# behzadnouri/firedancer

Hardware: AMD Instinct MI355X
Metric: ed25519 verified sigs/sec at 1/8 MI355X vs host AVX-512; p99 batch latency (higher is better)
Workload: dtype u32; 1 GPU; BASELINE configs[1]: 1M single-sig 1232-byte synthetic Solana txns, all valid; txns_per_gpu=1048576, sigs_per_gpu=1048576, parallelism=independent per-GPU shards x1, semantics=avx512, contexts_per_gpu=1

## Files before the change

### firedancer_amd/csrc/fd_ed25519_gpu.hip

```cpp

#include "fd_gpu_sha512.h"
#include "fd_gpu_curve.h"
#include "fd_gpu_txn.h"
#include "fd_gpu_lattice.h"
#include "fd_pin_list.h"
#include "../../include/fd_ed25519_gpu.h"

#include <hip/hip_runtime.h>
#include <atomic>
#include <mutex>
#include <string.h>
#include <stdio.h>
#include <time.h>
#include <stdlib.h>
#include <string>
#include <vector>
#include <deque>
#include <thread>
#include <pthread.h>
#include <sched.h>

#define FD_WG 256
#define FD_ATAB_ENTRIES 9
#define FD_ATAB_STORED  8
// ... 38 lines not shown


FD_DEV void fe_store_packed( uint4 * dst, fe const & a ) {
  u32 w[8]; fe_pack( w, a );
  dst[0] = make_uint4( w[0], w[1], w[2], w[3] );
  dst[1] = make_uint4( w[4], w[5], w[6], w[7] );
}
FD_DEV void fe_from_quads( fe & a, uint4 x, uint4 y ) {
  u32 w[8] = { x.x, x.y, x.z, x.w, y.x, y.y, y.z, y.w };
  fe_unpack( a, w );
}

__device__ __attribute__(( aligned( 16 ) )) unsigned const fd_atab_ident_w[ 32 ] = {
  1u,0u,0u,0u, 0u,0u,0u,0u,  1u,0u,0u,0u, 0u,0u,0u,0u,  1u,0u,0u,0u, 0u,0u,0u,0u,  0u,0u,0u,0u, 0u,0u,0u,0u };

FD_DEV uint4 const * atab_entry( uint4 const * tab, u32 s, int e ) {
  return e ? tab + ((size_t)s * FD_ATAB_STORED + (size_t)( e - 1 )) * 8 : (uint4 const *)fd_atab_ident_w;
}

FD_DEV void atab_store( uint4 * tab, u32 s, int e, ge_cached const & c ) {
  uint4 * b = tab + ((size_t)s * FD_ATAB_STORED + (size_t)( e - 1 )) * 8;
  fe_store_packed( b + 0, c.YpX );
  fe_store_packed( b + 2, c.YmX );
  fe_store_packed( b + 4, c.Z   );
  fe_store_packed( b + 6, c.T2d );
}

struct atab_raw { uint4 q[8]; };

FD_DEV void atab_fetch( atab_raw & r, uint4 const * tab, u32 s, int e ) {
  uint4 const * b = atab_entry( tab, s, e );
#pragma unroll
  for( int i=0; i<8; i++ ) r.q[i] = b[i];
}
FD_DEV void fe_load_planar( fe & r, u32 const * p, size_t n ) {
#pragma unroll
  for( int i=0; i<10; i++ ) r.v[i] = p[(size_t)i*n];
}
FD_DEV void fe_store_planar( u32 * p, size_t n, fe const & a ) {
#pragma unroll
  for( int i=0; i<10; i++ ) p[(size_t)i*n] = a.v[i];
}
FD_DEV void fe_shfl_up( fe & r, fe const & a, int d ) {
#pragma unroll
  for( int i=0; i<10; i++ ) r.v[i] = (u32)__shfl_up( (int)a.v[i], (unsigned)d, 64 );
}
FD_DEV void fe_shfl_down( fe & r, fe const & a, int d ) {
#pragma unroll
  for( int i=0; i<10; i++ ) r.v[i] = (u32)__shfl_down( (int)a.v[i], (unsigned)d, 64 );
}

FD_DEV void atab_unpack( ge_cached & c, atab_raw const & r ) {
  fe_from_quads( c.YpX, r.q[0], r.q[1] );
  fe_from_quads( c.YmX, r.q[2], r.q[3] );
  fe_from_quads( c.Z,   r.q[4], r.q[5] );
  fe_from_quads( c.T2d, r.q[6], r.q[7] );
}

FD_DEV int ks_pos( u32 b, u32 nsig, u32 nf, u32 nh, u32 & col, u32 & j, int & cls ) {
  u32 fb = ( nf + FD_WG - 1u ) / FD_WG, hb = ( nh + FD_WG - 1u ) / FD_WG;
  cls = b < fb ? 2 : b < fb + hb ? 1 : 0;
  j = ( cls==2 ? b : cls==1 ? b - fb : b - fb - hb ) * FD_WG + threadIdx.x;
  col = cls==2 ? j : cls==1 ? nf + j : nsig - 1u - j;
  return j < ( cls==2 ? nf : cls==1 ? nh : nsig - nf - nh );
}
FD_DEV u32 ks_sig( u32 const * __restrict__ order, u32 const * __restrict__ orderh, u32 col, u32 j, int cls ) {
  return ( orderh && cls==1 ) ? orderh[j] : order[col];
}
#define FD_KC_HOTK 0
#define FD_KC_HOT  1
#define FD_KC_COLD 2
#define FD_KC_FBK  3
#define FD_KC_FB   4
#define FD_KC_HIT   6
#define FD_KC_MISS  7
#define FD_KC_BUILD 8
#define FD_KC_HAND0 9
#define FD_KC_HAND  10
#define FD_KC_PTIX  11
#define FD_KC_FFK   12
#define FD_KC_FFS   13
#define FD_KC_PINK  14
#define FD_KC_PINS  15


__global__ void __launch_bounds__( FD_WG )
fd_expand_kernel( fdgpu_txn_desc_t const * __restrict__ desc, u32 txn_cnt, u32 * __restrict__ map, u32 nsig,
                  u32 * __restrict__ zero_word ) {
  u32 t = blockIdx.x * FD_WG + threadIdx.x;
  if( zero_word && t == 0u ) { zero_word[0] = 0u; zero_word[1] = 0u; }
  if( t >= txn_cnt ) return;
  fdgpu_txn_desc_t d = desc[t];
  for( u32 j=0; j<d.sig_cnt; j++ ) {
    u32 s = d.sig_base + j;
    if( s < nsig ) map[s] = t | (j << 24);
  }
}

template<int FM = FD_CARRY_FOLD>
FD_DEV void atab_build( uint4 * __restrict__ tab, u32 s, uint4 const * __restrict__ Axy ) {
  uint4 const * ap = Axy + (size_t)s*4;
  ge_p3 A;
  fe_from_quads( A.X, ap[0], ap[1] );
  fe_from_quads( A.Y, ap[2], ap[3] );
  A.Z = fe_one();
  fe_neg( A.X, A.X ); fe_wcarry( A.X, A.X );
  fe_mul<FM>( A.T, A.X, A.Y );
  ge_cached c1, c;
  ge_p3_to_cached<FM>( c1, A );
  atab_store( tab, s, 1, c1 );
  ge_precomp a1; a1.ypx = c1.YpX; a1.ymx = c1.YmX; a1.xy2d = c1.T2d;
  ge_p3 cur = A;
#pragma unroll 1
  for( int e=2; e<FD_ATAB_ENTRIES; e++ ) {
    ge_p1p1 tt;
    ge_add_precomp<FM>( tt, cur, a1 );
    ge_p1p1_to_p3<FM>( cur, tt );
    ge_p3_to_cached<FM>( c, cur );
    atab_store( tab, s, e, c );
  }
}

FD_DEV int txn_desc_ok( fdgpu_txn_desc_t const & d ) {
  u32 cnt = d.sig_cnt;
  return !( cnt==0u || cnt>16u
            || (u32)d.signature_off + 64u*cnt > (u32)d.payload_sz
            || (u32)d.acct_addr_off + 32u*cnt > (u32)d.payload_sz
            || (u32)d.message_off > (u32)d.payload_sz );
}

template<int FM = FD_CARRY_FOLD>
FD_DEV void decode_one( unsigned char const * __restrict__ payload, fdgpu_txn_desc_t const * __restrict__ desc,
                        u32 const * __restrict__ map, u32 s, u32 is_r, unsigned char * __restrict__ stat,
                        uint4 * __restrict__ Rxy, uint4 * __restrict__ Axy ) {
  u32 m = map[s];
  u32 t = m & 0xffffffu, j = m >> 24;
  fdgpu_txn_desc_t d = desc[t];
  if( !txn_desc_ok( d ) ) { *stat = 0xffu; return; }
  unsigned char const * base = payload + d.payload_off;
  u32 w[8];
  fd_load_words<8>( w, base + ( is_r ? (u32)d.signature_off + 64u*j : (u32)d.acct_addr_off + 32u*j ) );
  ge_p3 P; int rc;
  ge_decode1<FM>( P, rc, w );
  int so = ge_affine_is_small_order( P );
  *stat = (unsigned char)( rc | (so << 2) );
  u32 x[8], y[8];
  fe_pack( x, P.X ); fe_pack( y, P.Y );
  uint4 * o = ( is_r ? Rxy : Axy ) + (size_t)s*4;
  o[0] = make_uint4( x[0], x[1], x[2], x[3] ); o[1] = make_uint4( x[4], x[5], x[6], x[7] );
  o[2] = make_uint4( y[0], y[1], y[2], y[3] ); o[3] = make_uint4( y[4], y[5], y[6], y[7] );
}

__global__ void __launch_bounds__( FD_WG )
fd_decode_kernel( unsigned char const *    __restrict__ payload,
                  fdgpu_txn_desc_t const * __restrict__ desc,
                  u32 const *              __restrict__ map,
                  u32                                   nsig,
                  int                                   both,
                  unsigned char *          __restrict__ pstat,
                  uint4 *                  __restrict__ Rxy,
                  uint4 *                  __restrict__ Axy,
                  uint4 *                  __restrict__ tabA,
                  uint4 *                  __restrict__ tabR,
                  u32 const *              __restrict__ ulist,
                  u32 *                    __restrict__ ucnt,
                  unsigned char *          __restrict__ astat,
                  u32                                   ublk,
                  u32 const *              __restrict__ order,
                  u32 const *              __restrict__ orderh,
                  u32 const *              __restrict__ kscnt,
                  u32 const *              __restrict__ kcnt,
                  u32                                   fb_min,
                  u32 const *              __restrict__ fidx,
                  u32 const *              __restrict__ birth,
                  u32                                   batch,
                  u32 const *              __restrict__ full ) {
  u32 s, is_r;
  unsigned char * st;
  if( ulist ) {
    if( blockIdx.x < ublk ) {
      u32 i = blockIdx.x * FD_WG + threadIdx.x;
      u32 cnt = ucnt[0];
      if( !i ) {
        u32 samp = FD_KD_SBLK( ublk ) * FD_WG; samp = samp < nsig ? samp : nsig;
        ucnt[1] = ucnt[1] ? ucnt[2] > samp - ( samp >> 3 ) : cnt > nsig - ( nsig >> 3 );
        ucnt[2] = 0u;
      }
      if( i >= cnt ) return;
      s = ulist[i]; is_r = 0u; st = astat + s;
      if( fidx && kcnt[s] >= fb_min ) {
        u32 slot = fidx[s];
        if( slot != FD_FB_NONE && full[slot] ) atomicAdd( ucnt + 3 + FD_KC_FFK, 1u );
        if( slot != FD_FB_NONE && birth[slot] != batch ) return;
      }
    } else if( order ) {
      u32 col, j; int cls;
      if( !ks_pos( blockIdx.x - ublk, nsig, kscnt[FD_KC_FB], kscnt[FD_KC_HOT], col, j, cls ) || cls==2 ) return;
      s = ks_sig( order, orderh, col, j, cls ); is_r = 1u;
      st = pstat + 2u*s + 1u;
    } else {
      s = ( blockIdx.x - ublk ) * FD_WG + threadIdx.x; is_r = 1u;
      if( s >= nsig ) return;
      st = pstat + 2u*s + 1u;
    }
  } else {
    u32 p = blockIdx.x * FD_WG + threadIdx.x;
    if( p >= ( both ? 2u*nsig : nsig ) ) return;
    s = both ? p >> 1 : p; is_r = both ? p & 1u : 0u;
    st = pstat + 2u*s + is_r;
  }
  decode_one( payload, desc, map, s, is_r, st, Rxy, Axy );
  if( tabA && ( *st & 3u )==0u ) atab_build( is_r ? tabR : tabA, s, is_r ? Rxy : Axy );
}

template<class W>
FD_DEV int store_digits_B( u32 const Sw[ 8 ], u32 s, size_t n, short * __restrict__ digB, int top, W win ) {
  int carry = 0;
#pragma unroll
  for( int i=0; i<FD_BDIG; i++ ) {
    int bit = FD_BWIN*i;
    int v = (int)((Sw[bit>>5] >> (bit&31)) & ((1u<<FD_BWIN)-1u)) + carry;
    carry = (v + (1<<(FD_BWIN-1))) >> FD_BWIN;
    int db = v - (carry << FD_BWIN);
    digB[(size_t)i*n + s] = (short)db;
    int wb = win( i );
    top = ( db && wb > top ) ? wb : top;
  }
  return top;
}

FD_DEV void store_digits( u32 const k[ 8 ], u32 const Sw[ 8 ], u32 s, size_t n,
                          i8 * __restrict__ digA, short * __restrict__ digB ) {
  int carry = 0;
#pragma unroll
  for( int i=0; i<64; i++ ) {
    int v = (int)((k[i>>3] >> (4*(i&7))) & 15u) + carry;
    carry = (v + 8) >> 4;
    digA[(size_t)i*n + s] = (i8)(v - (carry << 4));
  }
  (void)store_digits_B( Sw, s, n, digB, 0, []( int ) { return 0; } );
}


FD_DEV void sc_mul_5x8( u32 out[ 16 ], u32 const a[ 5 ], u32 const b[ 8 ] ) {
  u32 r[ 16 ];
#pragma unroll
  for( int i=0; i<16; i++ ) r[i] = 0u;
#pragma unroll
  for( int i=0; i<5; i++ ) {
    u64 c = 0;
#pragma unroll
    for( int j=0; j<8; j++ ) { u64 t = (u64)a[i] * (u64)b[j] + (u64)r[i+j] + c; r[i+j] = (u32)t; c = t >> 32; }
    r[i+8] = (u32)c;
  }
#pragma unroll
  for( int i=0; i<16; i++ ) out[i] = r[i];
}

template<int HOT = 0>
FD_DEV int hs_prepare( u32 const k[ 8 ], u32 const Sw[ 8 ], u32 c0[ HOT ? 7 : 5 ], u32 c1m[ 5 ], int & c1neg, u32 sp[ 8 ] ) {
  constexpr int NC = HOT ? 7 : 5;
  int ng = 0, nwin = 0;
  if( HOT ) { if( !fd_lat_skew( c0, c1m, &ng, &nwin, k ) ) return 0; }
  else if( !fd_lat_halfsize( c0, c1m, &ng, k ) ) return 0;
  c1neg = ng;
  u32 c1lo = ng ? 0u - c1m[0] : c1m[0];
  if( ( c0[0] - c1lo * k[0] ) & 7u ) return 0;
  u32 const lw[8] = { 0x5cf5d3edu, 0x5812631au, 0xa2f79cd6u, 0x14def9deu, 0u, 0u, 0u, 0x10000000u };
  u32 prod[ 16 ], x[ 8 ];
  sc_mul_5x8( prod, c1m, k ); sc_reduce( x, prod );
  u32 diff = 0u;
  if( !ng ) {
#pragma unroll
    for( int i=0; i<8; i++ ) diff |= x[i] ^ ( i < NC ? c0[i] : 0u );
  } else {
// ... 241 lines not shown
  fd_load_words<8>( Aw, base + d.acct_addr_off + 32u*j );
  u32 h[16], k[8];
  if( khash ) {
    if( q ) return;
    khash_load( h, khash, s );
  } else {
    fd_sha512_RAM_quad( h, Rw, Aw, base + d.message_off, (u32)d.payload_sz - (u32)d.message_off, q, qbase );
    if( q ) return;
  }
  sc_reduce( k, h );
  u32 c0[5], c1m[5], sp[8]; int c1neg = 0;
  if( !( force_slow && s % force_slow == 0u ) && hs_prepare( k, Sw, c0, c1m, c1neg, sp ) ) {
    hs_store_digits( c0, c1m, c1neg, sp, s, n, digA, digR, digB, htop );
    code_out[s] = FD_ED25519_SUCCESS;
  } else {
    store_digits( k, Sw, s, n, digA, digB );
    code_out[s] = FD_PEND_SLOW;
    slow[ atomicAdd( slow_cnt, 1u ) ] = s;
  }
}

template<int FM = FD_CARRY_FOLD>
FD_DEV void htab_build( uint4 * __restrict__ htab, u32 hi, u32 part, uint4 const * __restrict__ Axy, u32 rep ) {
  uint4 const * ap = Axy + (size_t)rep*4;
  ge_p3 A;
  fe_from_quads( A.X, ap[0], ap[1] );
  fe_from_quads( A.Y, ap[2], ap[3] );
  A.Z = fe_one();
  fe_neg( A.X, A.X ); fe_wcarry( A.X, A.X );
  fe_mul<FM>( A.T, A.X, A.Y );
  int nd = 4*FD_KS_W*( (int)part + 1 );
#pragma unroll 1
  for( int i=0; i<nd; i++ ) ge_p3_dbl<FM>( A, A );
  u32 t = 2u*hi + part;
  ge_cached c1;
  ge_p3_to_cached<FM>( c1, A );
  atab_store( htab, t, 1, c1 );
#pragma unroll 1
  for( int e=2; e<FD_ATAB_ENTRIES; e++ ) {
    ge_p1p1 tt;
    ge_add_cached<FM>( tt, A, c1 );
    ge_p1p1_to_p3<FM>( A, tt );
    uint4 * b = htab + ((size_t)t * FD_ATAB_STORED + (size_t)( e - 1 )) * 8;
    fe u;
    fe_add( u, A.Y, A.X ); fe_store_packed( b + 0, u );
    fe_sub( u, A.Y, A.X ); fe_store_packed( b + 2, u );
    fe_store_packed( b + 4, A.Z );
    fe d2 = fe_d2(); fe_mul<FM>( u, A.T, d2 ); fe_store_packed( b + 6, u );
  }
}


FD_DEV void hashf_one( unsigned char const * __restrict__ payload, fdgpu_txn_desc_t const * __restrict__ desc,
                       u32 const * __restrict__ map, u32 s, size_t n, int semantics, u32 pa,
                       i8 * __restrict__ code_out, i8 * __restrict__ digA, short * __restrict__ digB,
                       uint4 * __restrict__ Rraw, uint4 const * __restrict__ khash, u32 col ) {
  fdgpu_txn_desc_t d; u32 j;
  if( !sig_desc( desc, map, s, d, j ) ) { code_out[s] = FD_ED25519_ERR_SIG; return; }
  unsigned char const * base = payload + d.payload_off;
  u32 Sw[8];
  fd_load_words<8>( Sw, base + d.signature_off + 64u*j + 32u );
  int code = sc_is_canonical( Sw ) ? FD_ED25519_SUCCESS : FD_ED25519_ERR_SIG;
  code = result_code( code, pa, 0u, semantics, 1 );
  code_out[s] = (i8)code;
  if( code != FD_ED25519_SUCCESS && code != FD_PEND_ASMALL ) return;
  u32 Rw[8], Aw[8];
  fd_load_words<8>( Rw, base + d.signature_off + 64u*j );
  Rraw[4*(size_t)s]   = make_uint4( Rw[0], Rw[1], Rw[2], Rw[3] );
  Rraw[4*(size_t)s+1] = make_uint4( Rw[4], Rw[5], Rw[6], Rw[7] );
  if( code != FD_ED25519_SUCCESS ) return;
  fd_load_words<8>( Aw, base + d.acct_addr_off + 32u*j );
  u32 h[16], k[8];
  if( khash ) khash_load( h, khash, s );
  else fd_sha512_RAM( h, Rw, Aw, base + d.message_off, (u32)d.payload_sz - (u32)d.message_off );
  sc_reduce( k, h );
  i8 dk[ 32 ];
  (void)fd_fb_recode( dk, k );
#pragma unroll
  for( int i=0; i<32; i++ ) digA[(size_t)i*n + col] = dk[i];
  (void)store_digits_B( Sw, col, n, digB, 0, []( int ) { return 0; } );
}

template<int FM = FD_CARRY_FOLD>
FD_DEV void fbase_chain( uint4 * __restrict__ fbase, u32 fi, u32 j, ge_p3 & A, int nd ) {
#pragma unroll 1
  for( int i=0; i<nd; i++ ) ge_p3_dbl<FM>( A, A );
  ge_cached c;
  ge_p3_to_cached<FM>( c, A );
  uint4 * b = fbase + ( (size_t)fi * FD_FB_NT + j ) * 8;
  fe_store_packed( b + 0, c.YpX );
  fe_store_packed( b + 2, c.YmX );
  fe_store_packed( b + 4, c.Z   );
  fe_store_packed( b + 6, c.T2d );
}
template<int FM = FD_CARRY_FOLD>
FD_DEV void fbase_build( uint4 * __restrict__ fbase, u32 fi, u32 j, uint4 const * __restrict__ Axy, u32 rep ) {
  uint4 const * ap = Axy + (size_t)rep*4;
  ge_p3 A;
  fe_from_quads( A.X, ap[0], ap[1] );
  fe_from_quads( A.Y, ap[2], ap[3] );
  A.Z = fe_one();
  fe_neg( A.X, A.X ); fe_wcarry( A.X, A.X );
  fe_mul<FM>( A.T, A.X, A.Y );
  fbase_chain<FM>( fbase, fi, j, A, 8*(int)j );
}

__device__ __attribute__(( aligned( 16 ) )) unsigned const fd_ptab_ident_w[ 24 ] = {
  1u,0u,0u,0u, 0u,0u,0u,0u,  1u,0u,0u,0u, 0u,0u,0u,0u,  0u,0u,0u,0u, 0u,0u,0u,0u };

FD_DEV size_t ftab_at( u32 fi, u32 j, u32 e ) {
  return ( ( (size_t)fi * FD_FB_NT + j ) * FD_FB_E + ( e - 1u ) ) * 6;
}

template<int I>
FD_DEV void ftab_pass1( ge_p3 & Q, ge_cached const & pc, uint4 * __restrict__ ent, fe (&pf)[ 8 ] ) {
  ge_p1p1 tt;
  ge_add_cached( tt, Q, pc ); ge_p1p1_to_p3( Q, tt );
  fe_store_packed( ent + 6*I + 0, Q.X );
  fe_store_packed( ent + 6*I + 2, Q.Y );
  fe_store_packed( ent + 6*I + 4, Q.Z );
  if constexpr( I > 0 ) fe_mul( pf[I], pf[I-1], Q.Z ); else pf[0] = Q.Z;
  if constexpr( I < 7 ) ftab_pass1<I+1>( Q, pc, ent, pf );
}
template<int I>
FD_DEV void ftab_pass2( fe & inv, uint4 * __restrict__ ent, fe const (&pf)[ 8 ] ) {
  fe X, Y, Z, zi, x, y, u;
  fe_from_quads( X, ent[6*I+0], ent[6*I+1] );
  fe_from_quads( Y, ent[6*I+2], ent[6*I+3] );
  if constexpr( I > 0 ) {
    fe_from_quads( Z, ent[6*I+4], ent[6*I+5] );
    fe_mul( zi, inv, pf[I-1] ); fe_mul( inv, inv, Z );
  } else zi = inv;
  fe_mul( x, X, zi ); fe_mul( y, Y, zi );
  fe_add( u, y, x ); fe_store_packed( ent + 6*I + 0, u );
  fe_sub( u, y, x ); fe_store_packed( ent + 6*I + 2, u );
  fe d2 = fe_d2();
  fe_mul( u, x, y ); fe_mul( u, u, d2 ); fe_store_packed( ent + 6*I + 4, u );
  if constexpr( I > 0 ) ftab_pass2<I-1>( inv, ent, pf );
}

__global__ void __launch_bounds__( FD_WG, 2 )
fd_ftab_kernel( u32 const * __restrict__ kscnt, u32 const * __restrict__ flist,
                unsigned char const * __restrict__ astat, uint4 const * __restrict__ fbase, uint4 * __restrict__ ftab,
                u32 cg, u32 const * __restrict__ plist, u32 pmax ) {
  u32 nk = kscnt[FD_KC_BUILD] * cg;
  u32 np = kscnt[FD_KC_PTIX]; np = np < pmax ? np : pmax;
  u32 bi = blockIdx.x * 2u + ( threadIdx.x >> 7 );
  if( blockIdx.x * 2u >= nk + 3u*np ) return;
  if( bi >= nk + 3u*np ) return;
  u32 fi, grp;
  if( bi < nk ) {
    if( astat[ flist[ 2u*( bi / cg ) + 1u ] ] & 7u ) return;
    fi = flist[ 2u*( bi / cg ) ]; grp = bi % cg;
  } else { fi = plist[ ( bi - nk ) / 3u ]; grp = ( bi - nk ) % 3u + 1u; }
  u32 t = 4u*( ( threadIdx.x >> 4 ) & 7u ) + grp, g = threadIdx.x & 15u;
  int lane = (int)( threadIdx.x & 63u );
  ge_cached pc;
  {
    atab_raw r; uint4 const * b = fbase + ( (size_t)fi * FD_FB_NT + t ) * 8;
#pragma unroll
    for( int i=0; i<8; i++ ) r.q[i] = b[i];
    atab_unpack( pc, r );
  }
  ge_p3 Q; ge_p3_identity( Q );
  ge_p1p1 tt;
#pragma unroll 1
  for( int b=3; b>=0; b-- ) {
    ge_p3_dbl( Q, Q );
    ge_add_cached( tt, Q, pc );
    ge_p3 Qa; ge_p1p1_to_p3( Qa, tt );
    int bit = (int)( ( g >> b ) & 1u );
    fe_sel( Q.X, bit, Qa.X, Q.X ); fe_sel( Q.Y, bit, Qa.Y, Q.Y ); fe_sel( Q.Z, bit, Qa.Z, Q.Z ); fe_sel( Q.T, bit, Qa.T, Q.T );
  }
#pragma unroll 1
  for( int b=0; b<3; b++ ) ge_p3_dbl( Q, Q );
  fe pf[ 8 ];
  uint4 * ent = ftab + ftab_at( fi, t, 8u*g + 1u );
  ftab_pass1<0>( Q, pc, ent, pf );
  fe one = fe_one(), pre = pf[7], suf = pf[7], u;
#pragma unroll 1
  for( int d=1; d<64; d<<=1 ) {
    fe_shfl_up( u, pre, d );   fe_sel( u, lane >= d, u, one );     fe_mul( pre, pre, u );
    fe_shfl_down( u, suf, d ); fe_sel( u, lane + d < 64, u, one ); fe_mul( suf, suf, u );
  }
  fe o, e, tot, inv;
  fe_shfl_up( o, pre, 1 );   fe_sel( o, lane > 0, o, one );
  fe_shfl_down( e, suf, 1 ); fe_sel( e, lane < 63, e, one );
  fe_mul( o, o, e );
#pragma unroll
  for( int i=0; i<10; i++ ) tot.v[i] = (u32)__shfl( (int)pre.v[i], 63, 64 );
  fe_invert( inv, tot );
  fe_mul( inv, inv, o );
  ftab_pass2<7>( inv, ent, pf );
}

template<int KS>
__global__ void __launch_bounds__( FD_WG )
fd_hashh_kernel( unsigned char const *    __restrict__ payload,
                 fdgpu_txn_desc_t const * __restrict__ desc,
                 u32 const *              __restrict__ map,
                 u32                                   nsig,
                 int                                   semantics,
                 unsigned char *          __restrict__ pstat,
                 i8 *                     __restrict__ code_out,
                 i8 *                     __restrict__ digA,
                 i8 *                     __restrict__ digR,
                 short *                  __restrict__ digB,
                 u32 *                    __restrict__ slow,
                 u32 *                    __restrict__ slow_cnt,
                 uint4 const *            __restrict__ khash,
                 u32                                   force_slow,
                 unsigned char *          __restrict__ htop,
                 u32 const *              __restrict__ arep,
                 unsigned char const *    __restrict__ astat,
                 u32 *                    __restrict__ order,
                 u32 const *              __restrict__ kscnt,
                 u32 const *              __restrict__ hlist,
                 uint4 const *            __restrict__ Axy,
                 uint4 *                  __restrict__ htab,
                 u32                                   hblk,
                 u32 const *              __restrict__ orderh,
                 u32 const *              __restrict__ flist,
                 uint4 *                  __restrict__ fbase,
                 u32                                   fblk,
                 unsigned char *          __restrict__ sstat,
                 uint4 *                  __restrict__ Rraw,
                 u32                                   lpk ) {
  if( KS ) {
    if( blockIdx.x < hblk ) {
      u32 i = blockIdx.x * FD_WG + threadIdx.x;
      if( ( i >> 1 ) >= kscnt[FD_KC_HOTK] ) return;
      u32 rep = hlist[ i >> 1 ];
      if( astat[rep] & 7u ) return;
      htab_build( htab, i >> 1, i & 1u, Axy, rep );
      return;
    }
    if( blockIdx.x < hblk + fblk ) {
      u32 i = ( blockIdx.x - hblk ) * FD_WG + threadIdx.x;
      u32 k = i / lpk, q = i % lpk;
      if( k >= kscnt[FD_KC_BUILD] ) return;
      u32 slot = flist[ 2u*k ], rep = flist[ 2u*k + 1u ];
      if( !q ) sstat[slot] = astat[rep];
      if( astat[rep] & 7u ) return;
      fbase_build( fbase, slot, q * ( (u32)FD_FB_NT / lpk ), Axy, rep );
      return;
    }
    u32 col, j; int cls;
    if( !ks_pos( blockIdx.x - hblk - fblk, nsig, orderh ? kscnt[FD_KC_FB] : 0u, kscnt[FD_KC_HOT], col, j, cls ) ) return;
    u32 s = ks_sig( order, orderh, col, j, cls );
    if( cls==2 ) {
      hashf_one( payload, desc, map, s, nsig, semantics, astat[ arep[s] ], code_out, digA, digB, Rraw, khash, col );
      return;
    }
    if( orderh && cls==1 ) order[col] = s;
    hashh_one<1>( payload, desc, map, s, nsig, semantics, 1, pstat, code_out, digA, digR, digB, slow, slow_cnt,
                  khash, force_slow, htop, arep, astat, col, cls==1 );
    return;
  }
  u32 s = blockIdx.x * FD_WG + threadIdx.x;
  if( s >= nsig ) return;
// ... 251 lines not shown
  uint4 ra[ 6 ], rb[ 6 ];
#pragma unroll 1
  for( int r=3; r>=0; r-- ) {
    int na = fd_fb_old_adds( r );
    int d = dA[ (size_t)fd_fb_old_digit( r, 0 )*n ];
    ptab_fetch( ra, d ? ftab + ftab_at( fi, (u32)fd_fb_old_table( 0 ), (u32)fd_fb_entry( d ) ) : (uint4 const *)fd_ptab_ident_w );
#pragma unroll 1
    for( int i=0; i<na; i++ ) {
      int dn = 0;
      if( i + 1 < na ) {
        int i1 = i + 1;
        if( !fd_fb_old_is_base( i1 ) ) {
          dn = dA[ (size_t)fd_fb_old_digit( r, i1 )*n ];
          ptab_fetch( rb, dn ? ftab + ftab_at( fi, (u32)fd_fb_old_table( i1 ), (u32)fd_fb_entry( dn ) ) : (uint4 const *)fd_ptab_ident_w );
        } else {
          dn = dB[ (size_t)fd_fb_old_digit( r, i1 )*n ];
          ptab_fetch( rb, btabf + ( (size_t)fd_fb_old_table( i1 ) * FD_BTAB_ENTRIES + (size_t)fd_fb_entry( dn ) ) * 6 );
        }
      }
      ge_precomp q;
      fe_from_quads( q.ypx,  ra[0], ra[1] );
      fe_from_quads( q.ymx,  ra[2], ra[3] );
      fe_from_quads( q.xy2d, ra[4], ra[5] );
      ge_precomp_cneg( q, d < 0 );
      ge_p1p1 t;
      ge_add_precomp<FM>( t, P, q ); ge_p1p1_to_p3<FM>( P, t );
#pragma unroll
      for( int v=0; v<6; v++ ) ra[v] = rb[v];
      d = dn;
    }
    if( r ) {
      ge_p2 P2; P2.X = P.X; P2.Y = P.Y; P2.Z = P.Z;
      ge_p1p1 t;
#pragma unroll 1
      for( int b=0; b<7; b++ ) { ge_dbl<FM>( t, P2 ); ge_p1p1_to_p2<FM>( P2, t ); }
      ge_dbl<FM>( t, P2 ); ge_p1p1_to_p3<FM>( P, t );
    }
  }
  fe_store_planar( Pbuf + col, n, P.X );
  fe_store_planar( Pbuf + 10*n + col, n, P.Y );
  fe_store_planar( Pbuf + 20*n + col, n, P.Z );
}

FD_DEV void full_fetch( uint4 r[ 6 ], int & d, int i, size_t n, u32 fi, uint4 const * __restrict__ ftab,
                        uint4 const * __restrict__ btabf, i8 const * __restrict__ dA, short const * __restrict__ dB ) {
  if( !fd_fb_full_is_base( i ) ) {
    d = dA[ (size_t)fd_fb_full_digit( i )*n ];
    ptab_fetch( r, d ? ftab + ftab_at( fi, (u32)fd_fb_full_table( i ), (u32)fd_fb_entry( d ) ) : (uint4 const *)fd_ptab_ident_w );
  } else {
    d = dB[ (size_t)fd_fb_full_digit( i )*n ];
    ptab_fetch( r, btabf + ( (size_t)fd_fb_full_table( i ) * FD_BTAB_ENTRIES + (size_t)fd_fb_entry( d ) ) * 6 );
  }
}
template<int FM>
FD_DEV void full_add( ge_p3 & P, uint4 const r[ 6 ], int d ) {
  ge_precomp q;
  fe_from_quads( q.ypx,  r[0], r[1] );
  fe_from_quads( q.ymx,  r[2], r[3] );
  fe_from_quads( q.xy2d, r[4], r[5] );
  ge_precomp_cneg( q, d < 0 );
  ge_p1p1 t;
  ge_add_precomp<FM>( t, P, q ); ge_p1p1_to_p3<FM>( P, t );
}
template<int FM>
FD_DEV void dsmf_full( u32 col, size_t n, u32 fi, uint4 const * __restrict__ ftab, uint4 const * __restrict__ btabf,
                       i8 const * __restrict__ digA, short const * __restrict__ digB, u32 * __restrict__ Pbuf ) {
  ge_p3 P; ge_p3_identity( P );
  i8 const * dA = digA + col; short const * dB = digB + col;
  uint4 ra[ 6 ], rb[ 6 ];
  int da, db;
  full_fetch( ra, da, 0, n, fi, ftab, btabf, dA, dB );
#pragma unroll 1
  for( int i=0; i<FD_FB_FULL_ADDS; i+=2 ) {
    full_fetch( rb, db, i + 1, n, fi, ftab, btabf, dA, dB );
    full_add<FM>( P, ra, da );
    if( i + 2 < FD_FB_FULL_ADDS ) full_fetch( ra, da, i + 2, n, fi, ftab, btabf, dA, dB );
    full_add<FM>( P, rb, db );
  }
  fe_store_planar( Pbuf + col, n, P.X );
  fe_store_planar( Pbuf + 10*n + col, n, P.Y );
  fe_store_planar( Pbuf + 20*n + col, n, P.Z );
}

template<int FM, int KS = 0>
__global__ void __launch_bounds__( FD_WG, FM ? FD_DSMH_MINW : 1 )
fd_dsmh_kernel( u32                      nsig,
                uint4 const * __restrict__ tabA,
                uint4 const * __restrict__ tabR,
                i8 const *    __restrict__ digA,
                i8 const *    __restrict__ digR,
                short const * __restrict__ digB,
                uint4 const * __restrict__ btab,
                uint4 const * __restrict__ btab2,
                i8 *          __restrict__ code,
                uint4 const * __restrict__ Rxy,
                u32 const *   __restrict__ slow,
                u32 const *   __restrict__ slow_cnt,
                u32                        nslowblk,
                unsigned char const * __restrict__ pstat,
                unsigned char const * __restrict__ htop,
                int                        rc,
                int                        semantics,
                u32 const *   __restrict__ arep,
                u32 const *   __restrict__ order,
                u32 const *   __restrict__ kscnt,
                u32 const *   __restrict__ hidx,
                uint4 const * __restrict__ htab,
                uint4 const * __restrict__ btabh,
                u32 const *   __restrict__ fidx,
                uint4 const * __restrict__ ftab,
                uint4 const * __restrict__ btabf,
                u32 *         __restrict__ Pbuf,
                u32 const *   __restrict__ full,
                u32 *         __restrict__ ffcnt ) {
  size_t n = nsig;
  if( blockIdx.x < nslowblk ) {
    u32 i = blockIdx.x * FD_WG + threadIdx.x;
    if( i < *slow_cnt ) {
      u32 cs = slow[i], ss = KS ? order[cs] : cs;
      dsm_one<FM>( ss, n, tabA, Rxy, digA, digB, btab, code, (u32 *)0, 0, arep ? arep[ss] : ss, cs );
    }
    return;
  }
  u32 s, col; int in, hot = 0;
  if( KS ) {
    u32 j; int cls;
    in = ks_pos( blockIdx.x - nslowblk, nsig, fidx ? kscnt[FD_KC_FB] : 0u, kscnt[FD_KC_HOT], col, j, cls );
    s = in ? order[col] : 0u;
    if( cls==2 ) {
      int walk = in && code[s] == FD_ED25519_SUCCESS;
      u32 fi = walk ? fidx[ arep[s] ] : 0u;
      unsigned long long wm = __ballot( walk );
      int allfull = __all( walk ? full[fi] != 0u : 1 );
      if( !walk ) return;
      if( allfull ) {
        if( (int)( threadIdx.x & 63u ) == __ffsll( (long long)wm ) - 1 ) atomicAdd( ffcnt, (u32)__popcll( wm ) );
        dsmf_full<FM>( col, n, fi, ftab, btabf, (i8 const *)digA, digB, Pbuf );
      }
      else dsmf_one<FM>( col, n, fi, ftab, btabf, (i8 const *)digA, digB, Pbuf );
      return;
    }
    hot = cls==1;
  }
  else { s = col = ( blockIdx.x - nslowblk ) * FD_WG + threadIdx.x; in = s < nsig; }
  int c = in ? (int)code[s] : FD_ED25519_ERR_SIG;
  if( rc && in ) c = result_code( c, pstat[2*s], pstat[2*s+1], semantics, 0 );
  int pend = c == FD_ED25519_SUCCESS && !( pstat[2*s] & FD_PSTAT_SLOW );
  int wtop = hs_wave_top( pend, htop, col );
  if( !pend ) { if( rc && in && c != FD_PEND_SLOW ) code[s] = (i8)c; return; }
  u32 sa = arep ? arep[s] : s;
  if( KS && hot ) {
    int ok = dsmh_hot<FM>( s, col, n, wtop, sa, hidx[sa], tabA, tabR, htab, digA, digR, digB, btab, btabh );
    code[s] = ok ? FD_ED25519_SUCCESS : FD_ED25519_ERR_MSG;
    return;
  }
  ge_p3 P; ge_p3_identity( P );
  ge_p2 P2;
  atab_raw ra, rr;
  int da = digA[ (size_t)wtop*n + col ], dr = digR[ (size_t)wtop*n + col ];
#pragma unroll 1
  for( int w=wtop; w>=0; w-- ) {
    atab_fetch( ra, tabA, sa, da < 0 ? -da : da );
    ge_p1p1 t;
    if( w != wtop ) {
#pragma unroll 1
      for( int r=0; r<3; r++ ) { ge_dbl<FM>( t, P2 ); ge_p1p1_to_p2<FM>( P2, t ); }
      ge_dbl<FM>( t, P2 ); ge_p1p1_to_p3<FM>( P, t );
    }
    atab_fetch( rr, tabR, s, dr < 0 ? -dr : dr );
    {
      ge_cached q; atab_unpack( q, ra ); ge_cached_cneg( q, da < 0 );
      ge_add_cached<FM>( t, P, q ); ge_p1p1_to_p3<FM>( P, t );
    }
    int bw = !(w & 1) && w < 32;
    int db = bw ? digB[ (size_t)( (w>>2) + ( (w & 2) ? 8 : 0 ) )*n + col ] : 0;
    {
      ge_cached q; atab_unpack( q, rr ); ge_cached_cneg( q, dr < 0 );
      ge_add_cached<FM>( t, P, q );
    }
    if( bw ) {
      uint4 braw[6];
      uint4 const * bp = ( (w & 2) ? btab2 : btab ) + (size_t)( db < 0 ? -db : db )*6;
#pragma unroll
      for( int i=0; i<6; i++ ) braw[i] = bp[i];
      ge_precomp bq;
      ge_p1p1_to_p3<FM>( P, t );
      fe_from_quads( bq.ypx,  braw[0], braw[1] );
      fe_from_quads( bq.ymx,  braw[2], braw[3] );
      fe_from_quads( bq.xy2d, braw[4], braw[5] );
      ge_precomp_cneg( bq, db < 0 );
      ge_add_precomp<FM>( t, P, bq );
    }
    ge_p1p1_to_p2<FM>( P2, t );
    if( w > 0 ) { da = digA[ (size_t)(w-1)*n + col ]; dr = digR[ (size_t)(w-1)*n + col ]; }
  }
  int ok = fe_is_zero( P2.X ) & fe_eq( P2.Y, P2.Z );
  code[s] = ok ? FD_ED25519_SUCCESS : FD_ED25519_ERR_MSG;
}

#define FD_DPP_MOV( d, a, PERM ) "v_mov_b32_dpp %" #d ", %" #a " " PERM " row_mask:0xf bank_mask:0xf\n\t"
#define FD_DEF_FE_DPP( name, PERM )                                                        \
FD_DEV void name( fe & r, fe const & a ) {                                                 \
  asm volatile( "s_nop 1\n\t"                                                              \
                FD_DPP_MOV( 0, 10, PERM ) FD_DPP_MOV( 1, 11, PERM ) FD_DPP_MOV( 2, 12, PERM ) \
                FD_DPP_MOV( 3, 13, PERM ) FD_DPP_MOV( 4, 14, PERM ) FD_DPP_MOV( 5, 15, PERM ) \
                FD_DPP_MOV( 6, 16, PERM ) FD_DPP_MOV( 7, 17, PERM ) FD_DPP_MOV( 8, 18, PERM ) \
                FD_DPP_MOV( 9, 19, PERM )                                                  \
                : "=&v"( r.v[0] ), "=&v"( r.v[1] ), "=&v"( r.v[2] ), "=&v"( r.v[3] ), "=&v"( r.v[4] ), \
                  "=&v"( r.v[5] ), "=&v"( r.v[6] ), "=&v"( r.v[7] ), "=&v"( r.v[8] ), "=&v"( r.v[9] ) \
                : "v"( a.v[0] ), "v"( a.v[1] ), "v"( a.v[2] ), "v"( a.v[3] ), "v"( a.v[4] ),  \
                  "v"( a.v[5] ), "v"( a.v[6] ), "v"( a.v[7] ), "v"( a.v[8] ), "v"( a.v[9] ) ); \
}
#define FD_DEF_U32_DPP( name, PERM )                                                       \
FD_DEV u32 name( u32 x ) {                                                                 \
  u32 r;                                                                                   \
  asm volatile( "s_nop 1\n\t" FD_DPP_MOV( 0, 1, PERM ) : "=&v"( r ) : "v"( x ) );          \
  return r;                                                                                \
}
FD_DEF_U32_DPP( fd_pair_xchg, "quad_perm:[1,0,3,2]" )
FD_DEF_FE_DPP( fe_xchg,   "quad_perm:[1,0,3,2]" )
// ... 715 lines not shown
FD_DEV u64 fd_xxh_round( u64 acc, u64 in ) { acc += in * FD_XXP2; acc = fd_rotl64( acc, 31 ); return acc * FD_XXP1; }
FD_DEV u64 fd_xxh64_64( u64 seed, unsigned char const * p ) {
  u32 w[16];
  fd_load_words<16>( w, p );
  u64 v[4] = { seed + FD_XXP1 + FD_XXP2, seed + FD_XXP2, seed, seed - FD_XXP1 };
#pragma unroll
  for( int blk=0; blk<2; blk++ )
#pragma unroll
    for( int i=0; i<4; i++ ) v[i] = fd_xxh_round( v[i], ((u64)w[8*blk + 2*i + 1] << 32) | (u64)w[8*blk + 2*i] );
  u64 h = fd_rotl64( v[0], 1 ) + fd_rotl64( v[1], 7 ) + fd_rotl64( v[2], 12 ) + fd_rotl64( v[3], 18 );
#pragma unroll
  for( int i=0; i<4; i++ ) { h ^= fd_xxh_round( 0UL, v[i] ); h = h * FD_XXP1 + FD_XXP4; }
  h += 64UL;
  h ^= h >> 33; h *= FD_XXP2; h ^= h >> 29; h *= FD_XXP3; h ^= h >> 32;
  return h;
}

#define FD_KD_PROBES 16u
FD_DEV u64 fd_key_hash( u32 const w[ 8 ], u32 seed32 ) {
  u64 seed = (u64)seed32 * FD_XXP3;
  u64 v0 = fd_xxh_round( seed + FD_XXP1 + FD_XXP2, ((u64)w[1] << 32) | (u64)w[0] );
  u64 v1 = fd_xxh_round( seed + FD_XXP2,           ((u64)w[3] << 32) | (u64)w[2] );
  u64 v2 = fd_xxh_round( seed,                     ((u64)w[5] << 32) | (u64)w[4] );
  u64 v3 = fd_xxh_round( seed - FD_XXP1,           ((u64)w[7] << 32) | (u64)w[6] );
  u64 h = fd_rotl64( v0, 1 ) + fd_rotl64( v1, 7 ) + fd_rotl64( v2, 12 ) + fd_rotl64( v3, 18 );
  h ^= h >> 33; h *= FD_XXP2; h ^= h >> 29; h *= FD_XXP3; h ^= h >> 32;
  return h;
}

struct fd_kcache {
  u32 *           key;
  u32 *           state;
  u32 *           birth;
  unsigned char * stat;
  u32 *           idx;
  u32             imask, iprobes;
  u32             fcap;
  u32             batch;
  u32 *           full;
  u32 *           plist;
  u32             pmax;
  u32             fnow;
  u32             npin;
};

template<int KS>
__global__ void __launch_bounds__( FD_WG )
fd_keydedup_kernel( unsigned char const *    __restrict__ payload,
                    fdgpu_txn_desc_t const * __restrict__ desc,
                    u32 const *              __restrict__ map,
                    u32                                   nsig,
                    u32 *                    __restrict__ ktab,
                    u32                                   kmask,
                    u32                                   seed32,
                    u32                                   probes,
                    u32 *                    __restrict__ arep,
                    u32 *                    __restrict__ ulist,
                    u32 *                    __restrict__ ucnt,
                    unsigned char *          __restrict__ pstat,
                    u32                                   sblk,
                    u32 *                    __restrict__ kcnt,
                    u32                                   hot_min,
                    u32                                   iblk,
                    fd_kcache                             kc ) {
  __shared__ u32 wcnt[ FD_WG / 64 + 1 ];
  if( KS && blockIdx.x < iblk ) {
    u32 slot = blockIdx.x * FD_WG + threadIdx.x;
    if( slot < kc.npin ) { kc.state[slot] = kc.batch; kc.birth[slot] = 0u; kc.full[slot] = 1u; }
    if( slot >= kc.fcap || !kc.state[slot] ) return;
    u32 w[8];
#pragma unroll
    for( int k=0; k<8; k++ ) w[k] = kc.key[ 8u*slot + k ];
    u32 h = (u32)( fd_key_hash( w, seed32 ) >> 32 );
    for( u32 i=0; i<kc.iprobes; i++ )
      if( !atomicCAS( kc.idx + ( ( h + i ) & kc.imask ), 0u, slot + 1u ) ) break;
    return;
  }
  u32 bx = KS ? blockIdx.x - iblk : blockIdx.x;
  u32 s = bx * FD_WG + threadIdx.x;
  if( KS && !s ) {
    u32 * c = ucnt + 3;
    for( int k=0; k<5; k++ ) c[k] = 0u;
    for( int k=FD_KC_HIT; k<=FD_KC_BUILD; k++ ) c[k] = 0u;
    for( int k=FD_KC_PTIX; k<=FD_KC_PINS; k++ ) c[k] = 0u;
    if( iblk ) { u32 h = c[FD_KC_HAND] % kc.fcap; c[FD_KC_HAND] = h; c[FD_KC_HAND0] = h; }
  }
  int bypass = ucnt[1] != 0u;
  int peek = !bypass;
  int own = s < nsig;
  u32 rep = s;
  if( s < nsig ) {
    pstat[2u*s] = 0u;
    u32 m = map[s];
    fdgpu_txn_desc_t d = desc[m & 0xffffffu];
    if( ( !bypass || bx < sblk ) && txn_desc_ok( d ) ) {
      u32 w[8];
      fd_load_words<8>( w, payload + d.payload_off + (u32)d.acct_addr_off + 32u*( m >> 24 ) );
      u64 h = fd_key_hash( w, seed32 );
      for( u32 i=0; i<probes; i++ ) {
        u32 * slot = ktab + ( ( (u32)h + i ) & kmask );
        u32 v = peek ? __hip_atomic_load( slot, __ATOMIC_RELAXED, __HIP_MEMORY_SCOPE_WORKGROUP ) : 0u;
        if( !v ) {
          v = atomicCAS( slot, 0u, s + 1u );
          if( !v ) break;
        }
        u32 c = v - 1u;
        if( c >= nsig ) continue;
        u32 mc = map[c];
        fdgpu_txn_desc_t dc = desc[mc & 0xffffffu];
        u32 wc[8];
        fd_load_words<8>( wc, payload + dc.payload_off + (u32)dc.acct_addr_off + 32u*( mc >> 24 ) );
        u32 diff = 0u;
#pragma unroll
        for( int k=0; k<8; k++ ) diff |= w[k] ^ wc[k];
        if( !diff ) { rep = c; own = 0; break; }
      }
      if( KS && !bypass ) {
        u32 * kc = kcnt + rep;
        if( __hip_atomic_load( kc, __ATOMIC_RELAXED, __HIP_MEMORY_SCOPE_WORKGROUP ) < hot_min ) atomicAdd( kc, 1u );
      }
    }
    arep[s] = rep;
  }
  unsigned long long mk = __ballot( own );
  u32 lane = threadIdx.x & 63u, wv = threadIdx.x >> 6;
  if( !lane ) wcnt[wv] = (u32)__popcll( mk );
  __syncthreads();
  u32 nsamp = sblk * FD_WG < nsig ? sblk * FD_WG : nsig;
  if( !threadIdx.x ) {
    u32 tot = 0u;
    for( u32 k=0; k<FD_WG/64; k++ ) { u32 c = wcnt[k]; wcnt[k] = tot; tot += c; }
    u32 base = 0u;
    if( !bypass ) {
      if( tot ) base = atomicAdd( ucnt, tot );
      if( tot && bx < sblk ) atomicAdd( ucnt + 2, tot );
    } else if( bx < sblk ) {
      if( tot ) { base = ( nsig - nsamp ) + atomicAdd( ucnt + 2, tot ); atomicAdd( ucnt, tot ); }
      if( !bx && nsig > nsamp ) atomicAdd( ucnt, nsig - nsamp );
    }
    wcnt[ FD_WG/64 ] = base;
  }
  __syncthreads();
  if( own ) {
    if( bypass && bx >= sblk ) ulist[ s - nsamp ] = s;
    else ulist[ wcnt[ FD_WG/64 ] + wcnt[wv] + (u32)__popcll( mk & ( ( 1ULL << lane ) - 1ULL ) ) ] = s;
  }
}

__global__ void __launch_bounds__( FD_WG )
fd_keysplit_kernel( u32 nsig, u32 const * __restrict__ arep, u32 const * __restrict__ kcnt, u32 hot_min,
                    u32 * __restrict__ hidx, u32 * __restrict__ hlist, u32 * __restrict__ order, u32 * __restrict__ cnt,
                    u32 hcap, u32 const * __restrict__ fidx, u32 * __restrict__ orderh, u32 fb_min,
                    u32 npin ) {
  __shared__ u32 wc[ 5 ][ FD_WG / 64 ], base[ 5 ];
  u32 s = blockIdx.x * FD_WG + threadIdx.x;
  int in = s < nsig;
  u32 rep = in ? arep[s] : 0u;
  u32 kc = in ? kcnt[rep] : 0u;
  u32 fi = in && fidx && kc >= fb_min ? fidx[rep] : FD_FB_NONE;
  int fb  = fi != FD_FB_NONE;
  int hot = !fb && kc >= hot_min;
  int f[ 5 ] = { hot && rep == s, hot, in && !hot && !fb, fb, fb && fi < npin };
  u32 lane = threadIdx.x & 63u, wv = threadIdx.x >> 6, rank[ 4 ];
#pragma unroll
  for( int k=0; k<5; k++ ) {
    unsigned long long mk = __ballot( f[k] );
    if( !lane ) wc[k][wv] = (u32)__popcll( mk );
    if( k < 4 ) rank[k] = (u32)__popcll( mk & ( ( 1ULL << lane ) - 1ULL ) );
  }
  __syncthreads();
  if( threadIdx.x < 5u ) {
    u32 k = threadIdx.x, tot = 0u;
    for( u32 w=0; w<FD_WG/64; w++ ) { u32 c = wc[k][w]; wc[k][w] = tot; tot += c; }
    base[k] = tot ? atomicAdd( cnt + ( k < 3u ? k : k == 3u ? (u32)FD_KC_FB : (u32)FD_KC_PINS ), tot ) : 0u;
  }
  __syncthreads();
  if( f[0] ) { u32 i = base[0] + wc[0][wv] + rank[0]; if( i < hcap ) { hidx[s] = i; hlist[i] = s; } }
  if( f[1] ) ( fidx ? orderh : order )[ base[1] + wc[1][wv] + rank[1] ] = s;
  if( f[2] ) order[ nsig - 1u - ( base[2] + wc[2][wv] + rank[2] ) ] = s;
  if( f[3] ) order[ base[3] + wc[3][wv] + rank[3] ] = s;
}

__global__ void __launch_bounds__( FD_WG )
fd_keyclass_kernel( u32 const * __restrict__ ulist, u32 const * __restrict__ ucnt, u32 const * __restrict__ kcnt,
                    u32 fb_min, u32 * __restrict__ fidx, u32 * __restrict__ mlist, u32 * __restrict__ cnt,
                    unsigned char const * __restrict__ payload, fdgpu_txn_desc_t const * __restrict__ desc,
                    u32 const * __restrict__ map, u32 seed32, unsigned char * __restrict__ astat, fd_kcache kc ) {
  u32 i = blockIdx.x * FD_WG + threadIdx.x;
  int sampled = ucnt[1] != 0u;
  if( ( sampled && !kc.npin ) || i >= ucnt[0] ) return;
  u32 s = ulist[i];
  int bound = !sampled && kcnt[s] >= fb_min;
  if( !bound && !kc.npin ) return;
  u32 m = map[s];
  fdgpu_txn_desc_t d = desc[m & 0xffffffu];
  if( kc.npin && !txn_desc_ok( d ) ) { fidx[s] = FD_FB_NONE; return; }
  u32 w[8];
  fd_load_words<8>( w, payload + d.payload_off + (u32)d.acct_addr_off + 32u*( m >> 24 ) );
  u32 h = (u32)( fd_key_hash( w, seed32 ) >> 32 );
  u32 slot = FD_FB_NONE;
  for( u32 p=0; p<kc.iprobes; p++ ) {
    u32 v = kc.idx[ ( h + p ) & kc.imask ];
    if( !v ) break;
    u32 sl = v - 1u;
    if( sl >= kc.fcap ) continue;
    u32 diff = 0u;
#pragma unroll
    for( int k=0; k<8; k++ ) diff |= w[k] ^ kc.key[ 8u*sl + k ];
    if( diff ) continue;
    if( sl < kc.npin ) {
      fidx[s] = sl;
      astat[s] = kc.stat[sl];
      atomicAdd( cnt + FD_KC_FBK, 1u ); atomicAdd( cnt + FD_KC_PINK, 1u );
      return;
    }
    slot = sl;
    if( !kc.npin ) break;
  }
  if( bound && slot != FD_FB_NONE ) {
    kc.state[slot] = kc.batch;
    fidx[s] = slot;
    u32 stt = kc.stat[slot];
    astat[s] = (unsigned char)stt;
    atomicAdd( cnt + FD_KC_FBK, 1u ); atomicAdd( cnt + FD_KC_HIT, 1u );
    if( kc.pmax && !( stt & 7u ) && !kc.full[slot] && !atomicCAS( kc.full + slot, 0u, kc.batch ) ) {
      u32 tk = atomicAdd( cnt + FD_KC_PTIX, 1u );
      if( tk < kc.pmax ) kc.plist[tk] = slot; else kc.full[slot] = 0u;
    }
    return;
  }
  fidx[s] = FD_FB_NONE;
  if( bound ) mlist[ atomicAdd( cnt + FD_KC_MISS, 1u ) ] = s;
}

__global__ void __launch_bounds__( FD_WG )
fd_keyclaim_kernel( u32 const * __restrict__ mlist, u32 * __restrict__ cnt, u32 * __restrict__ fidx,
                    u32 * __restrict__ flist, unsigned char const * __restrict__ payload,
                    fdgpu_txn_desc_t const * __restrict__ desc, u32 const * __restrict__ map, fd_kcache kc,
                    u32 cblk, uint4 * __restrict__ fbase ) {
  if( blockIdx.x >= cblk ) {
    u32 i = ( blockIdx.x - cblk ) * FD_WG + threadIdx.x;
    u32 np = cnt[FD_KC_PTIX]; np = np < kc.pmax ? np : kc.pmax;
    u32 p = i / 24u, q = i % 24u;
    if( p >= np ) return;
    u32 slot = kc.plist[p], t = q / 3u, r = q % 3u + 1u;
    uint4 const * e = fbase + ( (size_t)slot * FD_FB_NT + 4u*t ) * 8;
    fe ypx, ymx; ge_p3 A;
    fe_from_quads( ypx, e[0], e[1] ); fe_from_quads( ymx, e[2], e[3] ); fe_from_quads( A.Z, e[4], e[5] );
    fe_sub( A.X, ypx, ymx ); fe_wcarry( A.X, A.X );
    fe_add( A.Y, ypx, ymx ); fe_wcarry( A.Y, A.Y );
    fe_add( A.Z, A.Z, A.Z ); fe_wcarry( A.Z, A.Z ); A.T = fe_zero();
    fbase_chain( fbase, slot, 4u*t + r, A, 8*(int)r );
    return;
  }
  u32 i = blockIdx.x * FD_WG + threadIdx.x;
  if( i >= cnt[FD_KC_MISS] || i >= kc.fcap ) return;
  u32 s = mlist[i], hand0 = cnt[FD_KC_HAND0];
  for(;;) {
    u32 hv = atomicAdd( cnt + FD_KC_HAND, 1u );
    if( hv - hand0 >= kc.fcap ) return;
    u32 slot = hv % kc.fcap;
    if( kc.state[slot] == kc.batch ) continue;
    u32 m = map[s];
    fdgpu_txn_desc_t d = desc[m & 0xffffffu];
    u32 w[8];
    fd_load_words<8>( w, payload + d.payload_off + (u32)d.acct_addr_off + 32u*( m >> 24 ) );
#pragma unroll
    for( int k=0; k<8; k++ ) kc.key[ 8u*slot + k ] = w[k];
    kc.state[slot] = kc.batch; kc.birth[slot] = kc.batch;
    kc.full[slot] = kc.fnow ? kc.batch : 0u;
    fidx[s] = slot;
    u32 b = atomicAdd( cnt + FD_KC_BUILD, 1u );
    flist[2u*b] = slot; flist[2u*b+1u] = s;
    atomicAdd( cnt + FD_KC_FBK, 1u );
    return;
  }
}

__global__ void __launch_bounds__( FD_WG )
fd_keypin_kernel( u32 m, u32 const * __restrict__ key, unsigned char * __restrict__ sstat, uint4 * __restrict__ fbase,
                  u32 * __restrict__ flist, u32 * __restrict__ pcnt ) {
  u32 i = blockIdx.x * FD_WG + threadIdx.x;
  if( !i ) { pcnt[FD_KC_BUILD] = m; pcnt[FD_KC_PTIX] = 0u; }
  u32 slot = i / (u32)FD_FB_NT, j = i % (u32)FD_FB_NT;
  if( slot >= m ) return;
  u32 w[8];
#pragma unroll
  for( int k=0; k<8; k++ ) w[k] = key[ 8u*slot + k ];
  ge_p3 P; int rc;
  ge_decode1( P, rc, w );
  u32 st = (u32)rc | ( (u32)ge_affine_is_small_order( P ) << 2 );
  if( !j ) { sstat[slot] = (unsigned char)st; flist[2u*slot] = slot; flist[2u*slot+1u] = slot; }
  if( st & 7u ) return;
  u32 x[8], y[8];
  fe_pack( x, P.X ); fe_pack( y, P.Y );
  ge_p3 A;
  fe_unpack( A.X, x ); fe_unpack( A.Y, y );
  A.Z = fe_one();
  fe_neg( A.X, A.X ); fe_wcarry( A.X, A.X );
  fe_mul( A.T, A.X, A.Y );
  fbase_chain( fbase, slot, j, A, 8*(int)j );
}

struct fd_seeds { u64 seed[ 16 ]; u32 nseed; };

__global__ void __launch_bounds__( FD_WG )
fd_parse_kernel( unsigned char const *    __restrict__ payload,
                 fdgpu_txn_raw_t const *  __restrict__ raw,
                 u32                                    txn_cnt,
                 fdgpu_txn_desc_t *       __restrict__ desc_out,
                 unsigned char *          __restrict__ pflag,
                 unsigned char *          __restrict__ img,
                 u32                                    img_stride,
                 unsigned short *         __restrict__ fp_out,
                 fd_seeds                               dseeds,
                 u64 *                    __restrict__ dtag_out,
                 unsigned char const *    __restrict__ ovr,
                 u32 *                    __restrict__ map,
                 u32                                    nsig,
                 u32 *                    __restrict__ zero_word,
                 unsigned long *          __restrict__ stamp ) {
  u32 t = blockIdx.x * FD_WG + threadIdx.x;
  if( t == 0u ) {
    if( stamp ) __hip_atomic_store( stamp, __builtin_amdgcn_s_memrealtime(), __ATOMIC_RELAXED, __HIP_MEMORY_SCOPE_SYSTEM );
    if( zero_word ) { zero_word[0] = 0u; zero_word[1] = 0u; }
  }
  if( t >= txn_cnt ) return;
  fdgpu_txn_raw_t r = raw[t];
  if( ovr && ovr[t] ) {
    if( fp_out ) fp_out[t] = 0;
    if( dtag_out ) dtag_out[t] = 0UL;
    if( !desc_out ) return;
    fdgpu_txn_desc_t d;
    d.payload_off = r.payload_off; d.sig_base = r.sig_base; d.payload_sz = 0; d.message_off = 0; d.acct_addr_off = 0;
    d.signature_off = 0; d.sig_cnt = r.sig_lanes;
    desc_out[t] = d;
    pflag[t] = 2u;
    if( map ) for( u32 j=0; j<d.sig_cnt; j++ ) { u32 s = d.sig_base + j; if( s < nsig ) map[s] = t | (j << 24); }
    return;
  }
  fd_txn_hdr h;
  u32 fp = fd_txn_parse_dev( payload + r.payload_off, (u32)r.payload_sz,
                             img ? img + (size_t)t*img_stride : (unsigned char *)0, h );
  if( fp_out ) fp_out[t] = (unsigned short)fp;
  if( dtag_out ) {
    u64 seed = dseeds.nseed ? dseeds.seed[ r._pad[1] & 15u ] : dseeds.seed[0];
    dtag_out[t] = fp ? fd_xxh64_64( seed, payload + r.payload_off + h.sig_off ) : 0UL;
  }
  if( !desc_out ) return;
  fdgpu_txn_desc_t d;
  d.payload_off = r.payload_off; d.sig_base = r.sig_base;
  u32 lanes = h.sig_cnt <= 16u ? h.sig_cnt : 0u;
  int ok = fp != 0u && lanes == (u32)r.sig_lanes;
  if( ok ) {
    d.payload_sz = r.payload_sz; d.message_off = (unsigned short)h.msg_off; d.acct_addr_off = (unsigned short)h.acct_off;
    d.signature_off = (unsigned char)h.sig_off; d.sig_cnt = (unsigned char)lanes;
  } else {
    d.payload_sz = 0; d.message_off = 0; d.acct_addr_off = 0; d.signature_off = 0; d.sig_cnt = r.sig_lanes;
  }
  desc_out[t] = d;
  pflag[t] = ok ? 0u : 1u;
  if( map ) for( u32 j=0; j<d.sig_cnt; j++ ) { u32 s = d.sig_base + j; if( s < nsig ) map[s] = t | (j << 24); }
}

__global__ void __launch_bounds__( FD_WG )
fd_sha512_batch_kernel( unsigned char const * __restrict__ data, unsigned long const * __restrict__ off,
                        unsigned int const * __restrict__ sz, u32 cnt, uint4 * __restrict__ hash ) {
  u32 t = blockIdx.x * FD_WG + threadIdx.x;
  if( t >= cnt ) return;
  u32 h[16];
  fd_sha512_bytes( h, data + off[t], sz[t] );
  uint4 * o = hash + (size_t)t*4;
#pragma unroll
  for( int i=0; i<4; i++ ) o[i] = make_uint4( h[4*i], h[4*i+1], h[4*i+2], h[4*i+3] );
}

__global__ void __launch_bounds__( 256 ) fd_btab_kernel( uint4 * out, int dbl ) {
  int e = blockIdx.x * blockDim.x + threadIdx.x;
  if( e >= FD_BTAB_ENTRIES ) return;
  ge_p3 B; B.X = fe_Bx(); B.Y = fe_By(); B.Z = fe_one(); fe_mul( B.T, B.X, B.Y );
#pragma unroll 1
  for( int i=0; i<dbl; i++ ) ge_p3_dbl( B, B );
  ge_p3 acc; ge_p3_identity( acc );
#pragma unroll 1
// ... 142 lines not shown
#define FD_NGT   64

struct fdgpu_ed25519_ctx {
  int device, semantics, timing;
  std::vector<void *> dev_mem, pin_mem;
  unsigned long max_txn, max_sig, max_payload;
  hipStream_t stream;
  hipStream_t cstream;
  hipEvent_t  pipe_ev[ FD_PIPE_MAX ];
  u32 *   d_map;
  i8 *    d_code;
  unsigned char * d_pstat;
  uint4 * d_tab;
  uint4 * d_Rxy;
  uint4 * d_Axy;
  i8 *    d_digA;
  short * d_digB;
  uint4 * d_btab;
  fdgpu_txn_desc_t * d_rdesc;
  unsigned char *    d_pflag;
  int dsm_lanes;
  int poll_pf;
  int gather_rpb;
  int gather_cu_spread;
  int gather_nowb;
  unsigned long small_max;
  int last_path;
  int           excl_mode;
  unsigned long lat_cus;
  int           quad_sha;
  unsigned      excl_lds[ 8 ];
  unsigned long nofold_max;
  u32 *   d_P;
  u32 *   d_O;
  u32 *   d_blk;
  u32 *   d_slow;
  int     half;
  u32     half_force_slow;
  uint4 * d_tabR;
  i8 *    d_digR;
  unsigned char * d_htop;
  uint4 * d_btab2;
  uint4 * d_khash;
  int     key_dedup;
  u32 *   d_ktab;
  u32     kd_slots, kd_probes;
  int     kd_tiny;
  u32     kd_seed;
  u32 *   d_arep;
  u32 *   d_ulist;
  unsigned char * d_astat;
  int     key_split;
  u32     hot_min;
  u32     hot_cap;
  u32 *   d_kcnt;
  u32 *   d_hidx;
  u32 *   d_hlist;
  u32 *   d_order;
  uint4 * d_htab;
  uint4 * d_btabh;
  int     key_fixed;
  u32     fb_min;
  u32     fb_cap;
  u32 *   d_fidx;
  u32 *   d_flist;
  int     kc_mode;
  int     kc_dirty;
  u32     kc_batch;
  u32     kc_iwords, kc_iprobes;
  u32 *   d_kidx;
  u32 *   d_skey;
  u32 *   d_sstate;
  u32 *   d_sbirth;
  u32 *   d_sfull;
  int     kfull_mode;
  u32     pmax;
  u32 *   d_plist;
  u32     npin;
  unsigned char * d_sstat;
  u32 *   d_mlist;
  u32 *   d_orderh;
  uint4 * d_fbase;
  uint4 * d_ftab;
  uint4 * d_btabf;
  u32 *   d_fslow;
  hipEvent_t ev[5];
  hipEvent_t ring[ FD_NRING ][ 5 ];
  unsigned long ring_cnt;
  fd_slot slot[ FD_NSLOT ];
  int cur;
  int fault;
  int dbg_fail_issue;
  int dedup;
  unsigned long dedup_seed;
  unsigned long dedup_seeds[ 16 ];
  int           dedup_nseed;
  int rec_fp_off;
  hipStream_t gstream;
  hipEvent_t  gev;
  unsigned long * d_gcnt;
  unsigned long   g_launched;
  unsigned        gather_cus;
  unsigned long * h_gtime;
  unsigned long * d_gtime;
  struct { unsigned long target, t_launch, t_issue; } gt[ FD_NGT ];
  unsigned long   gt_head, gt_tail;
  double          gclk_off_ns;
  int             gclk_ok;
  unsigned long   gs_n, gs_start_sum, gs_start_max, gs_run_sum, gs_run_max;
  unsigned long   gs_issue_sum, gs_issue_max, gs_issue_slow;
  long            last_gt;
  unsigned long * h_stamp;
  unsigned long * d_stamp;
  unsigned long   ph[ 9 ];
  unsigned long n_batches, n_txns;
  unsigned long launch_ns;
  unsigned long volatile * h_flag;
  unsigned long sync_token;
  unsigned long * d_flag;
  unsigned long lat_hist[ FDGPU_LAT_BUCKETS ];
  std::deque<int> inflight;
  struct fdgpu_launcher * launcher;
  char lerr[ 192 ];
};

template< class T > static hipError_t
ctx_dev_alloc( fdgpu_ed25519_ctx_t * ctx, T ** p, size_t sz ) {
  hipError_t e = hipMalloc( (void **)p, sz );
  if( e == hipSuccess ) ctx->dev_mem.push_back( (void *)*p );
  return e;
}
template< class T, class U = T > static hipError_t
ctx_pin_alloc( fdgpu_ed25519_ctx_t * ctx, T ** p, size_t sz, U ** dev = NULL ) {
  hipError_t e = hipHostMalloc( (void **)p, sz, hipHostMallocDefault );
  if( e != hipSuccess ) return e;
  ctx->pin_mem.push_back( (void *)*p );
  return dev ? hipHostGetDevicePointer( (void **)dev, (void *)*p, 0 ) : hipSuccess;
}

#define FD_SYNC_SPIN_NS 20000000UL
static int stream_wait( fdgpu_ed25519_ctx_t * ctx, hipStream_t st, int pageable ) {
  if( !pageable ) {
    unsigned long tok = ++ctx->sync_token;
    hipLaunchKernelGGL( fd_done_kernel, dim3(1), dim3(1), 0, st, ctx->d_flag + FD_NSLOT, tok, (unsigned long *)NULL );
    if( hipGetLastError() == hipSuccess ) {
      unsigned long t0 = fd_now_ns();
      while( fd_now_ns() - t0 < FD_SYNC_SPIN_NS ) {
        if( ctx->h_flag[ FD_NSLOT ] == tok ) {
          std::atomic_thread_fence( std::memory_order_acquire );
          return 0;
        }
#if defined(__x86_64__)
        __builtin_ia32_pause();
#endif
      }
    }
  }
  hipError_t e = hipStreamSynchronize( st );
  if( e != hipSuccess ) { set_err( "hipStreamSynchronize", e ); return -2; }
  return 0;
}

extern "C" unsigned long
fdgpu_ed25519_set_small_batch_max( fdgpu_ed25519_ctx_t * ctx, unsigned long small_max ) {
  if( !ctx ) return 0UL;
  unsigned long old = ctx->small_max;
// ... 7 lines not shown
fdgpu_ed25519_set_cu_exclusive( fdgpu_ed25519_ctx_t * ctx, int on ) {
  if( !ctx || on < 0 || on > 4 ) return -1;
  void const * f[ 8 ] = { (void const *)fd_prep_kernel<0,1>, (void const *)fd_prep_kernel<0,0>, (void const *)fd_dsm8_kernel<0>,
                          (void const *)fd_dsm4_kernel<0,1>, (void const *)fd_dsm4_kernel<0,0>,
                          (void const *)fd_dsm2_kernel<0,1>, (void const *)fd_dsm2_kernel<0,0>,
                          (void const *)fd_prep_kernel<0,1,1> };
  unsigned v[ 8 ] = { 0u, 0u, 0u, 0u, 0u, 0u, 0u, 0u };
  if( on ) {
    HIPCHK( hipSetDevice( ctx->device ), -2 );
    int lds = 0;
    HIPCHK( hipDeviceGetAttribute( &lds, hipDeviceAttributeMaxSharedMemoryPerMultiprocessor, ctx->device ), -2 );
    if( lds < 3 * 1024 ) { fd_err = "fdgpu_ed25519_set_cu_exclusive: no LDS size"; return -1; }
    unsigned half = ( (unsigned)lds / 2u + 4096u ) & ~1023u;
    unsigned third = ( (unsigned)lds / 3u + 2048u ) & ~1023u;
    unsigned want = on == 2 ? third : half;
    std::lock_guard<std::mutex> lk( g_excl_mu );
    for( int i=0; i<8; i++ ) {
      hipFuncAttributes a;
      HIPCHK( hipFuncGetAttributes( &a, f[i] ), -2 );
      unsigned st = (unsigned)a.sharedSizeBytes;
      int walk = i >= 2 && i <= 6;
      if( ( on == 3 && !walk ) || ( on == 4 && walk ) ) continue;
      v[i] = st < want ? want - st : 0u;
      unsigned top = st < half ? half - st : 0u;
      if( v[i] && g_excl_max[i] < top ) {
        HIPCHK( hipFuncSetAttribute( f[i], hipFuncAttributeMaxDynamicSharedMemorySize, (int)top ), -2 );
        g_excl_max[i] = top;
      }
    }
  }
  for( int i=0; i<8; i++ ) ctx->excl_lds[i] = v[i];
  ctx->excl_mode = on;
  return 0;
}

extern "C" int
fdgpu_ed25519_get_cu_exclusive( fdgpu_ed25519_ctx_t const * ctx ) { return ctx ? ctx->excl_mode : 0; }

extern "C" int
fdgpu_ed25519_set_lat_share( fdgpu_ed25519_ctx_t * ctx, unsigned parts ) {
  if( !ctx ) return -1;
  if( !parts ) { ctx->lat_cus = 0UL; return 0; }
  int ncu = 0;
  HIPCHK( hipSetDevice( ctx->device ), -2 );
  HIPCHK( hipDeviceGetAttribute( &ncu, hipDeviceAttributeMultiprocessorCount, ctx->device ), -2 );
  unsigned long free_cus = (unsigned long)ncu > ctx->gather_cus ? (unsigned long)ncu - ctx->gather_cus : 1UL;
  ctx->lat_cus = free_cus / parts ? free_cus / parts : 1UL;
  return 0;
}

extern "C" char const * fdgpu_last_error( void ) { return fd_err.c_str(); }

static int async_busy( fdgpu_ed25519_ctx_t const * ctx ) {
  if( !ctx->inflight.empty() ) return 1;
  for( int i=0; i<FD_NSLOT; i++ ) if( ctx->slot[i].txn_cnt ) return 1;
  return 0;
}

static int pick_path( fdgpu_ed25519_ctx_t const * ctx, unsigned long nsig ) {
  if( !nsig ) return FDGPU_PATH_NONE;
  if( nsig <= ctx->small_max ) {
    int lanes = ctx->dsm_lanes ? ctx->dsm_lanes : ( nsig <= FD_DSM8_MAX && ctx->half ? 8 : nsig <= FD_DSM4_MAX ? 4 :
                                                    nsig <= FD_DSM2_MAX ? 2 : 1 );
    if( lanes == 8 && !ctx->half ) lanes = 4;
    int excl_walk = ctx->excl_mode == 1 || ctx->excl_mode == 2 || ctx->excl_mode == 3;
    if( !ctx->dsm_lanes && ctx->lat_cus && excl_walk ) {
      unsigned long budget = ctx->lat_cus * ( ctx->excl_mode == 2 ? 2UL : 1UL );
      unsigned long wg = ( nsig + FD_WG - 1UL ) / FD_WG;
      while( lanes > 1 && (unsigned long)lanes * wg > budget ) lanes >>= 1;
    }
    return lanes;
  }
  return ctx->half ? FDGPU_PATH_THROUGHPUT : FDGPU_PATH_THROUGHPUT_FULL;
}

enum {
  FD_SW_SLOW     = 0,
  FD_SW_KEYS     = 1,
  FD_SW_DISTINCT = 2,
  FD_SW_SAMPLE   = 3,
  FD_SW_HOT      = 4,
  FD_SW_FBSLOW   = 9,
  FD_SW_KCACHE   = 10,
  FD_SW_CNT      = 20 };
static u32 * slow_word( fdgpu_ed25519_ctx_t const * ctx, int w ) { return ctx->d_slow + ctx->max_sig + w; }

struct fd_batch {
  unsigned char const *    d_payload;
  fdgpu_txn_desc_t const * d_desc;
  u32                      nsig;
  unsigned                 sg;
  i8 *                     code;
  hipStream_t              st;
  hipEvent_t *             ev;
};

static int launch_latency( fdgpu_ed25519_ctx_t * ctx, fd_batch const & b, int lanes ) {
  u32 nsig = b.nsig; unsigned sg = b.sg; i8 * code = b.code; hipStream_t st = b.st;
  int hs = ctx->half;
  int qs = hs && ctx->quad_sha >= 0 && nsig <= FD_QSHA_MAX;
  int d2 = lanes > 1;
  u32 * slow_cnt = slow_word( ctx, FD_SW_SLOW );
  hipLaunchKernelGGL( ( qs ? fd_prep_kernel<0,1,1> : hs ? fd_prep_kernel<0,1> : fd_prep_kernel<0,0> ),
                      dim3( ( qs ? 6 : 3 )*sg ), dim3(FD_WG), ctx->excl_lds[ qs ? 7 : hs ? 0 : 1 ], st, b.d_payload, b.d_desc,
                      ctx->d_map, nsig, (u32)sg, ctx->semantics, ctx->d_pstat, ctx->d_Rxy, ctx->d_Axy, code, ctx->d_digA,
                      ctx->d_digB, hs || d2 ? ctx->d_tab : (uint4 *)NULL, (uint4 const *)ctx->d_khash,
                      hs ? ctx->d_tabR : (uint4 *)NULL, hs ? ctx->d_digR : (i8 *)NULL, hs ? ctx->d_slow : (u32 *)NULL,
                      hs ? slow_cnt : (u32 *)NULL, hs ? ctx->half_force_slow : 0u, hs ? ctx->d_htop : (unsigned char *)NULL );
  if( !hs && !d2 )
    hipLaunchKernelGGL( fd_table_kernel, dim3(sg), dim3(FD_WG), 0, st, nsig, ctx->semantics, ctx->d_pstat, code,
                        ctx->d_Axy, ctx->d_tab );
  if( ctx->timing ) hipEventRecord( b.ev[1], st );
  if( lanes==8 )
    hipLaunchKernelGGL( fd_dsm8_kernel<0>, dim3(8*sg), dim3(FD_WG), ctx->excl_lds[2], st, nsig, ctx->d_tab, ctx->d_tabR,
                        ctx->d_digA, ctx->d_digR, ctx->d_digB, ctx->d_btab, ctx->d_btab2, code, ctx->semantics, ctx->d_pstat,
                        ctx->d_htop, ctx->d_Rxy, ctx->d_slow, slow_cnt );
  else if( lanes==4 || lanes==2 )
    hipLaunchKernelGGL( ( lanes==4 ? ( hs ? fd_dsm4_kernel<0,1> : fd_dsm4_kernel<0,0> )
                                   : ( hs ? fd_dsm2_kernel<0,1> : fd_dsm2_kernel<0,0> ) ),
                        dim3(lanes*sg), dim3(FD_WG), ctx->excl_lds[ ( lanes==4 ? 3 : 5 ) + !hs ], st, nsig, ctx->d_tab,
                        ctx->d_Rxy, ctx->d_digA, ctx->d_digB, ctx->d_btab, code, ctx->semantics, ctx->d_pstat,
                        ctx->d_tabR, ctx->d_digR, ctx->d_btab2, ctx->d_htop, ctx->d_slow, slow_cnt );
  else if( hs )
    hipLaunchKernelGGL( fd_dsmh_kernel<0>, dim3(sg), dim3(FD_WG), 0, st, nsig, ctx->d_tab, ctx->d_tabR, ctx->d_digA,
                        ctx->d_digR, ctx->d_digB, ctx->d_btab, ctx->d_btab2, code, ctx->d_Rxy, ctx->d_slow, slow_cnt, 0u,
                        ctx->d_pstat, ctx->d_htop, 1, ctx->semantics, (u32 const *)NULL, (u32 const *)NULL,
                        (u32 const *)NULL, (u32 const *)NULL, (uint4 const *)NULL, (uint4 const *)NULL,
                        (u32 const *)NULL, (uint4 const *)NULL, (uint4 const *)NULL, (u32 *)NULL, (u32 const *)NULL,
                        (u32 *)NULL );
  else
    hipLaunchKernelGGL( ( nsig <= ctx->nofold_max ? fd_dsm_kernel<0> : fd_dsm_kernel<1> ), dim3(sg), dim3(FD_WG), 0, st,
                        nsig, ctx->d_tab, ctx->d_Rxy, ctx->d_digA, ctx->d_digB, ctx->d_btab, code, ctx->d_P, 0 );
  if( ctx->timing ) hipEventRecord( b.ev[2], st );
  if( hs && lanes <= 1 )
    hipLaunchKernelGGL( fd_dsm_slowl_kernel<0>, dim3(sg), dim3(FD_WG), 0, st, nsig, ctx->d_tab, ctx->d_Rxy, ctx->d_digA,
                        ctx->d_digB, ctx->d_btab, code, ctx->d_slow, slow_cnt, ctx->semantics, ctx->d_pstat );
  return 0;
}

static int launch_half( fdgpu_ed25519_ctx_t * ctx, fd_batch const & b ) {
  u32 nsig = b.nsig; unsigned sg = b.sg; i8 * code = b.code; hipStream_t st = b.st;
  int kd = ctx->key_dedup, ks = ctx->key_split, kf = ctx->key_fixed;
  u32 * slow_cnt = slow_word( ctx, FD_SW_SLOW ), * ucnt = slow_word( ctx, FD_SW_KEYS );
  u32 const * arep = kd ? ctx->d_arep : NULL, * order = ks ? ctx->d_order : NULL, * hidx = ks ? ctx->d_hidx : NULL;
  u32 const * kscnt = ks ? slow_word( ctx, FD_SW_HOT ) : NULL;
  unsigned long fkeys = kf ? nsig / ctx->fb_min : 0UL; if( fkeys > ctx->fb_cap ) fkeys = ctx->fb_cap;
  fd_kcache kc = {}; unsigned iblk = 0u;
  u32 npin = kf ? ctx->npin : 0u, fbm = npin ? 0u : ctx->fb_min;
  if( kd ) {
    u32 slots = 64u;
    if( !ctx->kd_tiny ) while( slots < ctx->kd_slots && slots < 2u*nsig ) slots <<= 1;
    if( kf ) {
      kc.key = ctx->d_skey; kc.state = ctx->d_sstate; kc.birth = ctx->d_sbirth; kc.stat = ctx->d_sstat; kc.idx = ctx->d_kidx;
      kc.imask = ctx->kc_iwords - 1u; kc.iprobes = ctx->kc_iprobes; kc.fcap = ctx->fb_cap;
      if( !++ctx->kc_batch ) { ctx->kc_batch = 1u; ctx->kc_dirty = 1; }
      kc.batch = ctx->kc_batch;
      kc.full = ctx->d_sfull; kc.plist = ctx->d_plist; kc.pmax = ctx->pmax; kc.fnow = ctx->kfull_mode == 2;
      kc.npin = ctx->npin;
      int clear = ctx->kc_mode == 1 || ctx->kc_dirty;
      ctx->kc_dirty = 2;
      if( clear ) HIPCHK( hipMemsetAsync( ctx->d_sstate, 0, ( ctx->fb_cap ? ctx->fb_cap : 1UL ) * 3 * sizeof(u32), st ), -3 );
      iblk = ( ctx->fb_cap + FD_WG - 1u ) / FD_WG;
    }
    HIPCHK( hipMemsetAsync( kf ? ctx->d_kidx : ctx->d_ktab, 0, ( (size_t)slots + ( kf ? ctx->kc_iwords : 0u ) ) * sizeof(u32), st ), -3 );
    if( ks ) HIPCHK( hipMemsetAsync( ctx->d_kcnt, 0, (size_t)nsig * sizeof(u32), st ), -3 );
    u32 seed = ++ctx->kd_seed;
    hipLaunchKernelGGL( ( ks ? fd_keydedup_kernel<1> : fd_keydedup_kernel<0> ), dim3(iblk + sg), dim3(FD_WG), 0, st, b.d_payload,
                        b.d_desc, ctx->d_map, nsig, ctx->d_ktab, slots - 1u, seed, ctx->kd_probes, ctx->d_arep,
                        ctx->d_ulist, ucnt, ctx->d_pstat, FD_KD_SBLK( sg ), ks ? ctx->d_kcnt : (u32 *)NULL,
                        kf && ctx->fb_min > ctx->hot_min ? ctx->fb_min : ks ? ctx->hot_min : 0u, (u32)iblk, kc );
    if( kf ) {
      hipLaunchKernelGGL( fd_keyclass_kernel, dim3(sg), dim3(FD_WG), 0, st, (u32 const *)ctx->d_ulist, (u32 const *)ucnt,
                          (u32 const *)ctx->d_kcnt, ctx->fb_min, ctx->d_fidx, ctx->d_mlist, slow_word( ctx, FD_SW_HOT ),
                          b.d_payload, b.d_desc, (u32 const *)ctx->d_map, seed, ctx->d_astat, kc );
      if( fkeys ) {
        unsigned cblk = (unsigned)( ( fkeys + FD_WG - 1UL ) / FD_WG ), pbk = (unsigned)( ( 24UL * ctx->pmax + FD_WG - 1 ) / FD_WG );
        hipLaunchKernelGGL( fd_keyclaim_kernel, dim3( cblk + pbk ), dim3(FD_WG), 0, st,
                            (u32 const *)ctx->d_mlist, slow_word( ctx, FD_SW_HOT ), ctx->d_fidx, ctx->d_flist, b.d_payload,
                            b.d_desc, (u32 const *)ctx->d_map, kc, (u32)cblk, ctx->d_fbase );
      }
    }
    if( ks )
      hipLaunchKernelGGL( fd_keysplit_kernel, dim3(sg), dim3(FD_WG), 0, st, nsig, (u32 const *)ctx->d_arep,
                          (u32 const *)ctx->d_kcnt, ctx->hot_min, ctx->d_hidx, ctx->d_hlist, ctx->d_order,
                          slow_word( ctx, FD_SW_HOT ), ctx->hot_cap, (u32 const *)( kf ? ctx->d_fidx : NULL ),
                          kf ? ctx->d_orderh : (u32 *)NULL, kf ? fbm : 0u, npin );
  }
  hipLaunchKernelGGL( fd_decode_kernel, dim3( kf ? 2*sg + 2 : kd ? 2*sg : (unsigned)( ( 2UL*nsig + FD_WG - 1 ) / FD_WG ) ),
                      dim3(FD_WG), 0, st,
                      b.d_payload, b.d_desc, ctx->d_map, nsig, 1, ctx->d_pstat, ctx->d_Rxy, ctx->d_Axy, ctx->d_tab, ctx->d_tabR,
                      kd ? (u32 const *)ctx->d_ulist : NULL, kd ? ucnt : (u32 *)NULL,
                      kd ? ctx->d_astat : (unsigned char *)NULL, kd ? (u32)sg : 0u, kf ? order : (u32 const *)NULL,
                      (u32 const *)( kf ? ctx->d_orderh : NULL ), kf ? kscnt : (u32 const *)NULL,
                      (u32 const *)( kf ? ctx->d_kcnt : NULL ), kf ? fbm : 0u, (u32 const *)( kf ? ctx->d_fidx : NULL ),
                      (u32 const *)( kf ? ctx->d_sbirth : NULL ), kc.batch, (u32 const *)( kf ? ctx->d_sfull : NULL ) );
  if( ctx->timing ) hipEventRecord( b.ev[4], st );
  unsigned hb = ks ? (unsigned)( ( 2UL * ( nsig / ctx->hot_min ) + FD_WG - 1 ) / FD_WG ) : 0u;
  unsigned lpk = kf && ctx->kfull_mode == 2 ? 32u : 8u, cg = lpk / 8u;
  unsigned long pkeys = fkeys ? ctx->pmax : 0UL;
  unsigned fbk = (unsigned)( ( lpk * fkeys + FD_WG - 1 ) / FD_WG );
  hipLaunchKernelGGL( ( ks ? fd_hashh_kernel<1> : fd_hashh_kernel<0> ), dim3( ks ? hb + fbk + sg + ( kf ? 2 : 1 ) : sg ),
                      dim3(FD_WG), 0, st,
                      b.d_payload, b.d_desc, ctx->d_map, nsig, ctx->semantics, ctx->d_pstat, code, ctx->d_digA, ctx->d_digR,
                      ctx->d_digB, ctx->d_slow, slow_cnt, (uint4 const *)ctx->d_khash, ctx->half_force_slow, ctx->d_htop,
                      arep, (unsigned char const *)( kd ? ctx->d_astat : NULL ), ks ? ctx->d_order : (u32 *)NULL, kscnt,
                      (u32 const *)( ks ? ctx->d_hlist : NULL ), (uint4 const *)( ks ? ctx->d_Axy : NULL ),
                      ks ? ctx->d_htab : (uint4 *)NULL, (u32)hb, (u32 const *)( kf ? ctx->d_orderh : NULL ),
                      (u32 const *)( kf ? ctx->d_flist : NULL ), kf ? ctx->d_fbase : (uint4 *)NULL, (u32)fbk,
                      kf ? ctx->d_sstat : (unsigned char *)NULL, kf ? ctx->d_Rxy : (uint4 *)NULL, (u32)lpk );
  if( fkeys )
    hipLaunchKernelGGL( fd_ftab_kernel, dim3( (unsigned)( ( cg * fkeys + 3UL * pkeys + 1UL ) / 2UL ) ), dim3(FD_WG), 0, st, kscnt,
                        (u32 const *)ctx->d_flist, (unsigned char const *)ctx->d_astat, (uint4 const *)ctx->d_fbase,
                        ctx->d_ftab, (u32)cg, (u32 const *)ctx->d_plist, ctx->pmax );
  if( ctx->timing ) hipEventRecord( b.ev[1], st );
  unsigned nsb = ( sg + 63u ) / 64u;
  int fold = nsig > ctx->nofold_max;
  hipLaunchKernelGGL( ( fold ? ( ks ? fd_dsmh_kernel<1,1> : fd_dsmh_kernel<1,0> )
                             : ( ks ? fd_dsmh_kernel<0,1> : fd_dsmh_kernel<0,0> ) ),
                      dim3( nsb + sg + ( kf ? 2u : ks ? 1u : 0u ) ), dim3(FD_WG), 0, st, nsig, ctx->d_tab, ctx->d_tabR, ctx->d_digA,
                      ctx->d_digR, ctx->d_digB, ctx->d_btab, ctx->d_btab2, code, ctx->d_Rxy, ctx->d_slow, slow_cnt, nsb,
                      ctx->d_pstat, ctx->d_htop, 0, ctx->semantics, arep, order, kscnt, hidx,
                      (uint4 const *)( ks ? ctx->d_htab : NULL ), (uint4 const *)( ks ? ctx->d_btabh : NULL ),
                      (u32 const *)( kf ? ctx->d_fidx : NULL ), (uint4 const *)( kf ? ctx->d_ftab : NULL ),
                      (uint4 const *)( kf ? ctx->d_btabf : NULL ), kf ? ctx->d_P : (u32 *)NULL,
                      (u32 const *)( kf ? ctx->d_sfull : NULL ), kf ? slow_word( ctx, FD_SW_HOT ) + FD_KC_FFS : (u32 *)NULL );
  if( ctx->timing ) hipEventRecord( b.ev[2], st );
  if( fkeys || npin ) {
    u32 const * fcnt = kscnt + FD_KC_FB; u32 * fslow_cnt = slow_word( ctx, FD_SW_FBSLOW );
    hipLaunchKernelGGL( fd_rprod_kernel, dim3(sg), dim3(FD_WG), 0, st, nsig, code, ctx->d_P, ctx->d_O, ctx->d_blk, fslow_cnt,
                        order, fcnt );
    hipLaunchKernelGGL( fd_rinv_kernel, dim3((sg + FD_WG - 1)/FD_WG), dim3(FD_WG), 0, st, sg, ctx->d_blk, fcnt );
    hipLaunchKernelGGL( fd_rcheck_kernel, dim3(sg), dim3(FD_WG), 0, st, nsig, code, ctx->d_Rxy, ctx->d_P, ctx->d_O, ctx->d_blk,
                        ctx->d_fslow, fslow_cnt, order, fcnt, 4u, FD_PEND_FBREQ );
    hipLaunchKernelGGL( fd_rslow_kernel, dim3(sg), dim3(FD_WG), 0, st, nsig, ctx->semantics, code, ctx->d_Rxy, ctx->d_P,
                        ctx->d_fslow, fslow_cnt, order, 4u );
  }
  hipLaunchKernelGGL( ( fold ? fd_dsm_slow_kernel<1> : fd_dsm_slow_kernel<0> ), dim3(sg), dim3(FD_WG), 0, st, nsig,
                      ctx->d_tab, ctx->d_Rxy, ctx->d_digA, ctx->d_digB, ctx->d_btab, code, ctx->d_slow, slow_cnt,
                      nsb * FD_WG, arep, order );
  return 0;
}

static int launch_full( fdgpu_ed25519_ctx_t * ctx, fd_batch const & b ) {
  u32 nsig = b.nsig; unsigned sg = b.sg; i8 * code = b.code; hipStream_t st = b.st;
  u32 * slow_cnt = slow_word( ctx, FD_SW_SLOW );
  hipLaunchKernelGGL( fd_decode_kernel, dim3(sg), dim3(FD_WG), 0, st, b.d_payload, b.d_desc, ctx->d_map, nsig, 0,
                      ctx->d_pstat, ctx->d_Rxy, ctx->d_Axy, (uint4 *)NULL, (uint4 *)NULL, (u32 const *)NULL,
                      (u32 *)NULL, (unsigned char *)NULL, 0u, (u32 const *)NULL, (u32 const *)NULL, (u32 const *)NULL,
                      (u32 const *)NULL, 0u, (u32 const *)NULL, (u32 const *)NULL, 0u, (u32 const *)NULL );
  hipLaunchKernelGGL( fd_hash_kernel, dim3(sg), dim3(FD_WG), 0, st, b.d_payload, b.d_desc, ctx->d_map, nsig,
                      ctx->semantics, 1, ctx->d_pstat, code, ctx->d_digA, ctx->d_digB, ctx->d_Rxy,
                      (uint4 const *)ctx->d_khash );
  hipLaunchKernelGGL( fd_table_kernel, dim3(sg), dim3(FD_WG), 0, st, nsig, ctx->semantics,
                      (unsigned char const *)NULL, code, ctx->d_Axy, ctx->d_tab );
  if( ctx->timing ) hipEventRecord( b.ev[1], st );
  hipLaunchKernelGGL( ( nsig <= ctx->nofold_max ? fd_dsm_kernel<0> : fd_dsm_kernel<1> ), dim3(sg), dim3(FD_WG), 0, st,
                      nsig, ctx->d_tab, ctx->d_Rxy, ctx->d_digA, ctx->d_digB, ctx->d_btab, code, ctx->d_P, 1 );
  if( ctx->timing ) hipEventRecord( b.ev[2], st );
  hipLaunchKernelGGL( fd_rprod_kernel, dim3(sg), dim3(FD_WG), 0, st, nsig, code, ctx->d_P, ctx->d_O, ctx->d_blk, slow_cnt,
                      (u32 const *)NULL, (u32 const *)NULL );
  hipLaunchKernelGGL( fd_rinv_kernel, dim3((sg + FD_WG - 1)/FD_WG), dim3(FD_WG), 0, st, sg, ctx->d_blk, (u32 const *)NULL );
  hipLaunchKernelGGL( fd_rcheck_kernel, dim3(sg), dim3(FD_WG), 0, st, nsig, code, ctx->d_Rxy, ctx->d_P, ctx->d_O, ctx->d_blk,
                      ctx->d_slow, slow_cnt, (u32 const *)NULL, (u32 const *)NULL, 2u, FD_PEND_REQ );
  hipLaunchKernelGGL( fd_rslow_kernel, dim3(sg), dim3(FD_WG), 0, st, nsig, ctx->semantics, code, ctx->d_Rxy, ctx->d_P,
                      ctx->d_slow, slow_cnt, (u32 const *)NULL, 2u );
  return 0;
}

static int launch_batch( fdgpu_ed25519_ctx_t * ctx, unsigned char const * d_payload, fdgpu_txn_desc_t const * d_desc,
                         unsigned long txn_cnt, unsigned long sig_cnt, i8 * d_txn_out, i8 * d_sig_out, hipStream_t st,
                         unsigned char const * d_pflag = NULL, int flags = 0 ) {
  if( !txn_cnt ) return 0;
  fd_batch b = { d_payload, d_desc, (u32)sig_cnt, (unsigned)( (sig_cnt + FD_WG - 1) / FD_WG ),
                 d_sig_out ? d_sig_out : ctx->d_code, st, ctx->ev };
  if( ctx->timing ) { b.ev = ctx->ring[ ctx->ring_cnt % FD_NRING ]; ctx->ring_cnt++; }
  unsigned tg = (unsigned)( (txn_cnt + FD_WG - 1) / FD_WG );
  ctx->last_path = pick_path( ctx, b.nsig );
  if( b.nsig ) {
    if( !( flags & 1 ) )
      hipLaunchKernelGGL( fd_expand_kernel, dim3(tg), dim3(FD_WG), 0, st, d_desc, (u32)txn_cnt, ctx->d_map, b.nsig,
                          slow_word( ctx, FD_SW_SLOW ) );
    if( ctx->timing ) hipEventRecord( b.ev[0], st );
    int err = b.nsig <= ctx->small_max ? launch_latency( ctx, b, ctx->last_path )
            : ctx->half                ? launch_half( ctx, b ) : launch_full( ctx, b );
    if( err ) return err;
  }
  if( !( flags & 2 ) )
    hipLaunchKernelGGL( fd_reduce_kernel, dim3(tg), dim3(FD_WG), 0, st, d_desc, (u32)txn_cnt, b.nsig, b.code, d_pflag, d_txn_out );
  if( ctx->timing ) hipEventRecord( b.ev[3], st );
  HIPCHK( hipGetLastError(), -3 );
  if( ctx->kc_dirty == 2 ) ctx->kc_dirty = 0;
  return 0;
}

static std::mutex g_dbg_mu;
static fdgpu_debug_opts_t g_dbg = { -1, 0u, -1L, 0, -1L, 0, 0, 0, 0, 0, 0, 0, 0, 0, 0, 0 };
static void debug_opts_get( fdgpu_debug_opts_t * o ) { std::lock_guard<std::mutex> lk( g_dbg_mu ); *o = g_dbg; }

extern "C" void
fdgpu_debug_set_opts( fdgpu_debug_opts_t const * opts ) {
  std::lock_guard<std::mutex> lk( g_dbg_mu );
  if( opts ) g_dbg = *opts;
  else       g_dbg = fdgpu_debug_opts_t{ -1, 0u, -1L, 0, -1L, 0, 0, 0, 0, 0, 0, 0, 0, 0, 0, 0 };
}

static int
slot_bufs( fdgpu_ed25519_ctx_t * ctx, int i ) {
  fd_slot & sl = ctx->slot[i];
  if( sl.h_payload ) return 0;
  unsigned long mp = ctx->max_payload, mt = ctx->max_txn;
  HIPCHK( hipSetDevice( ctx->device ), -1 );
  HIPCHK( ctx_pin_alloc( ctx, &sl.h_payload, mp + FD_ARENA_SLACK ), -1 );
  HIPCHK( ctx_pin_alloc( ctx, &sl.h_desc, mt * sizeof(fdgpu_txn_desc_t), &sl.hd_desc ), -1 );
  HIPCHK( ctx_pin_alloc( ctx, &sl.h_txn_out, mt, &sl.hd_txn_out ), -1 );
  HIPCHK( ctx_pin_alloc( ctx, &sl.h_tags, mt * sizeof(unsigned long) ), -1 );
  HIPCHK( ctx_dev_alloc( ctx, &sl.d_payload, mp + FD_ARENA_SLACK + FD_IMG_TAIL ), -1 );
  HIPCHK( ctx_dev_alloc( ctx, &sl.d_desc, mt * sizeof(fdgpu_txn_desc_t) ), -1 );
  HIPCHK( ctx_dev_alloc( ctx, &sl.d_txn_out, mt ), -1 );
  memset( sl.h_payload, 0, FD_ARENA_SLACK );
  return 0;
}

__global__ void fd_clock_kernel( unsigned long * out ) {
  __hip_atomic_store( out, __builtin_amdgcn_s_memrealtime(), __ATOMIC_RELAXED, __HIP_MEMORY_SCOPE_SYSTEM );
}

static void gclk_calibrate( fdgpu_ed25519_ctx_t * ctx ) {
  unsigned long volatile * w = (unsigned long volatile *)( ctx->h_stamp + 2*FD_NSLOT );
  double best = 1e30;
  for( int k=0; k<3; k++ ) {
    w[0] = 0UL;
    unsigned long t0 = fd_now_ns();
    hipLaunchKernelGGL( fd_clock_kernel, dim3(1), dim3(1), 0, ctx->stream, ctx->d_stamp + 2*FD_NSLOT );
    if( hipStreamSynchronize( ctx->stream ) != hipSuccess || !w[0] ) return;
    unsigned long t1 = fd_now_ns();
    if( (double)( t1 - t0 ) < best ) { best = (double)( t1 - t0 ); ctx->gclk_off_ns = (double)w[0] * 10.0 - 0.5 * ( (double)t0 + (double)t1 ); }
  }
  ctx->gclk_ok = 1;
}

static int
ctx_init( fdgpu_ed25519_ctx_t * ctx, int device, unsigned long max_txn, unsigned long max_sig,
          unsigned long max_payload_bytes, int semantics ) {
  ctx->device = device; ctx->semantics = semantics; ctx->timing = 0;
  ctx->max_txn = max_txn; ctx->max_sig = max_sig; ctx->max_payload = max_payload_bytes;
  size_t ns = max_sig;
  HIPCHK( hipStreamCreateWithFlags( &ctx->stream, hipStreamNonBlocking ), -1 );

  HIPCHK( ctx_dev_alloc( ctx, &ctx->d_map,  ns * sizeof(u32) ), -1 );
  HIPCHK( ctx_dev_alloc( ctx, &ctx->d_code, ns ), -1 );
  HIPCHK( ctx_dev_alloc( ctx, &ctx->d_pstat, 2*ns ), -1 );
  HIPCHK( ctx_dev_alloc( ctx, &ctx->d_tab,  ns * FD_ATAB_STORED * 8 * sizeof(uint4) ), -1 );
  HIPCHK( ctx_dev_alloc( ctx, &ctx->d_Rxy,  ns * 4 * sizeof(uint4) ), -1 );
  HIPCHK( ctx_dev_alloc( ctx, &ctx->d_Axy,  ns * 4 * sizeof(uint4) ), -1 );
  HIPCHK( ctx_dev_alloc( ctx, &ctx->d_digA, ns * 64 ), -1 );
  HIPCHK( ctx_dev_alloc( ctx, &ctx->d_digB, ns * FD_BDIG * sizeof(short) ), -1 );
  HIPCHK( ctx_dev_alloc( ctx, &ctx->d_btab, FD_BTAB_ENTRIES * 6 * sizeof(uint4) ), -1 );
  HIPCHK( ctx_dev_alloc( ctx, &ctx->d_rdesc, max_txn * sizeof(fdgpu_txn_desc_t) ), -1 );
  HIPCHK( ctx_dev_alloc( ctx, &ctx->d_pflag, max_txn ), -1 );
  HIPCHK( ctx_dev_alloc( ctx, &ctx->d_P, ns * 30 * sizeof(u32) ), -1 );
  HIPCHK( ctx_dev_alloc( ctx, &ctx->d_O, ns * 10 * sizeof(u32) ), -1 );
  HIPCHK( ctx_dev_alloc( ctx, &ctx->d_blk, ( ( ns + FD_WG - 1 ) / FD_WG ) * 10 * sizeof(u32) ), -1 );
  HIPCHK( ctx_dev_alloc( ctx, &ctx->d_slow, ( ns + FD_SW_CNT ) * sizeof(u32) ), -1 );
  HIPCHK( hipMemsetAsync( slow_word( ctx, 0 ), 0, FD_SW_CNT * sizeof(u32), ctx->stream ), -1 );
  fdgpu_debug_opts_t dbg; debug_opts_get( &dbg );
  ctx->half = dbg.half >= 0 ? dbg.half : FD_HALF;
  ctx->half_force_slow = dbg.half_force_slow;
  if( ctx->half ) {
    HIPCHK( ctx_dev_alloc( ctx, &ctx->d_tabR, ns * FD_ATAB_STORED * 8 * sizeof(uint4) ), -1 );
    HIPCHK( ctx_dev_alloc( ctx, &ctx->d_digR, ns * FD_HDIG ), -1 );
    HIPCHK( ctx_dev_alloc( ctx, &ctx->d_htop, ns ), -1 );
    HIPCHK( ctx_dev_alloc( ctx, &ctx->d_btab2, FD_BTAB_ENTRIES * 6 * sizeof(uint4) ), -1 );
    ctx->key_dedup = dbg.key_dedup != 1;
    if( ctx->key_dedup ) {
      unsigned long slots = 64UL;
      if( dbg.key_dedup != 2 ) while( slots < 2UL*ns && slots < ( 1UL << 31 ) ) slots <<= 1;
      ctx->kd_slots = (u32)slots; ctx->kd_tiny = dbg.key_dedup == 2; ctx->kd_probes = ctx->kd_tiny ? 2u : FD_KD_PROBES;
      ctx->kd_seed = 0u;
      ctx->key_fixed = dbg.key_split != 1 && dbg.key_fixed != 1 && !ctx->half_force_slow;
      if( ctx->key_fixed ) {
        ctx->fb_min = dbg.key_fixed == 2 ? 4u : FD_FB_MIN;
        unsigned long fc = ns / ctx->fb_min;
        ctx->fb_cap = (u32)( fc < FD_FB_CAP ? fc : FD_FB_CAP );
        ctx->kc_mode = dbg.key_cache; ctx->kc_dirty = 0; ctx->kc_batch = 0u;
        if( ctx->kc_mode == 2 && ctx->fb_cap > 8u ) ctx->fb_cap = 8u;
        u32 iw = 8u;
        if( ctx->kc_mode != 2 ) while( iw < 4u * ctx->fb_cap ) iw <<= 1;
        ctx->kc_iwords = iw; ctx->kc_iprobes = ctx->kc_mode == 2 ? 2u : FD_KD_PROBES;
        ctx->kfull_mode = dbg.key_full;
        ctx->pmax = ctx->kfull_mode == 1 ? 0u : ctx->fb_cap / 4u > 1u ? ctx->fb_cap / 4u : 1u;
      }
      HIPCHK( ctx_dev_alloc( ctx, &ctx->d_kidx, ( (size_t)ctx->kc_iwords + slots ) * sizeof(u32) ), -1 );
      ctx->d_ktab = ctx->d_kidx + ctx->kc_iwords;
      HIPCHK( ctx_dev_alloc( ctx, &ctx->d_arep, ns * sizeof(u32) ), -1 );
      HIPCHK( ctx_dev_alloc( ctx, &ctx->d_ulist, ns * sizeof(u32) ), -1 );
      HIPCHK( ctx_dev_alloc( ctx, &ctx->d_astat, ns ), -1 );
      ctx->key_split = dbg.key_split != 1;
      if( ctx->key_split ) {
        ctx->hot_min = dbg.key_split == 2 ? 2u : FD_HOT_MIN;
        ctx->hot_cap = (u32)( ns / ctx->hot_min );
        size_t hc = ctx->hot_cap ? ctx->hot_cap : 1UL;
        HIPCHK( ctx_dev_alloc( ctx, &ctx->d_kcnt, ns * sizeof(u32) ), -1 );
        HIPCHK( ctx_dev_alloc( ctx, &ctx->d_hidx, ns * sizeof(u32) ), -1 );
        HIPCHK( ctx_dev_alloc( ctx, &ctx->d_hlist, hc * sizeof(u32) ), -1 );
        HIPCHK( ctx_dev_alloc( ctx, &ctx->d_order, ns * sizeof(u32) ), -1 );
        HIPCHK( ctx_dev_alloc( ctx, &ctx->d_htab, hc * 2 * FD_ATAB_STORED * 8 * sizeof(uint4) ), -1 );
        HIPCHK( ctx_dev_alloc( ctx, &ctx->d_btabh, (size_t)3 * FD_BTAB_ENTRIES * 6 * sizeof(uint4) ), -1 );
        if( ctx->key_fixed ) {
          size_t fcn = ctx->fb_cap ? ctx->fb_cap : 1UL;
          HIPCHK( ctx_dev_alloc( ctx, &ctx->d_fidx, ns * sizeof(u32) ), -1 );
          HIPCHK( ctx_dev_alloc( ctx, &ctx->d_flist, fcn * 2 * sizeof(u32) ), -1 );
          HIPCHK( ctx_dev_alloc( ctx, &ctx->d_skey, fcn * 8 * sizeof(u32) ), -1 );
          HIPCHK( ctx_dev_alloc( ctx, &ctx->d_sstate, fcn * 3 * sizeof(u32) ), -1 );
          ctx->d_sbirth = ctx->d_sstate + fcn; ctx->d_sfull = ctx->d_sbirth + fcn;
          HIPCHK( ctx_dev_alloc( ctx, &ctx->d_plist, ( ctx->pmax ? ctx->pmax : 1UL ) * sizeof(u32) ), -1 );
          HIPCHK( ctx_dev_alloc( ctx, &ctx->d_sstat, fcn ), -1 );
          HIPCHK( ctx_dev_alloc( ctx, &ctx->d_mlist, ( ns / ctx->fb_min + 1UL ) * sizeof(u32) ), -1 );
          HIPCHK( hipMemsetAsync( ctx->d_sstate, 0, fcn * 3 * sizeof(u32), ctx->stream ), -1 );
          HIPCHK( ctx_dev_alloc( ctx, &ctx->d_orderh, ns * sizeof(u32) ), -1 );
          HIPCHK( ctx_dev_alloc( ctx, &ctx->d_fbase, fcn * FD_FB_NT * 8 * sizeof(uint4) ), -1 );
          HIPCHK( ctx_dev_alloc( ctx, &ctx->d_ftab, fcn * FD_FB_NT * FD_FB_E * 6 * sizeof(uint4) ), -1 );
          HIPCHK( ctx_dev_alloc( ctx, &ctx->d_btabf, (size_t)FD_FB_NB * FD_BTAB_ENTRIES * 6 * sizeof(uint4) ), -1 );
          HIPCHK( ctx_dev_alloc( ctx, &ctx->d_fslow, ns * sizeof(u32) ), -1 );
        }
      }
    }
  }
  ctx->small_max  = dbg.small_batch_max >= 0 ? (unsigned long)dbg.small_batch_max : FD_SMALL_BATCH_MAX;
  ctx->dsm_lanes  = dbg.dsm_lanes;
  ctx->nofold_max = dbg.nofold_max >= 0 ? (unsigned long)dbg.nofold_max : FD_NOFOLD_MAX;
  ctx->gather_nowb = dbg.gather_no_writeback;
  ctx->poll_pf = dbg.poll_prefetch > 0 ? dbg.poll_prefetch : 0;
  ctx->gather_rpb = dbg.gather_rpb == 1 ? 1 : 4;
  ctx->gather_cu_spread = dbg.gather_cu_spread;
  ctx->quad_sha = dbg.quad_sha;
  for( int i=0; i<5; i++ ) HIPCHK( hipEventCreate( &ctx->ev[i] ), -1 );
  for( int r=0; r<FD_NRING; r++ ) for( int i=0; i<5; i++ ) HIPCHK( hipEventCreate( &ctx->ring[r][i] ), -1 );
  ctx->ring_cnt = 0;
  hipLaunchKernelGGL( fd_btab_kernel, dim3((FD_BTAB_ENTRIES + 255)/256), dim3(256), 0, ctx->stream, ctx->d_btab, 0 );
  if( ctx->half )
    hipLaunchKernelGGL( fd_btab_kernel, dim3((FD_BTAB_ENTRIES + 255)/256), dim3(256), 0, ctx->stream, ctx->d_btab2, 120 );
  if( ctx->key_split ) {
    int const e[ 3 ] = { 72, 140, 196 };
    for( int t=0; t<3; t++ )
      hipLaunchKernelGGL( fd_btab_kernel, dim3((FD_BTAB_ENTRIES + 255)/256), dim3(256), 0, ctx->stream,
                          ctx->d_btabh + (size_t)t * FD_BTAB_ENTRIES * 6, e[t] );
  }
  if( ctx->key_fixed )
    for( int u=0; u<FD_FB_NB; u++ )
      hipLaunchKernelGGL( fd_btab_kernel, dim3((FD_BTAB_ENTRIES + 255)/256), dim3(256), 0, ctx->stream,
                          ctx->d_btabf + (size_t)u * FD_BTAB_ENTRIES * 6, 16*u );
  HIPCHK( hipGetLastError(), -1 );
  for( int i=0; i<FD_NSLOT; i++ ) HIPCHK( hipEventCreateWithFlags( &ctx->slot[i].done, hipEventDisableTiming ), -1 );
  HIPCHK( ctx_pin_alloc( ctx, &ctx->h_flag, ( FD_NSLOT + 2 ) * sizeof(unsigned long), &ctx->d_flag ), -1 );
  for( int i=0; i<=FD_NSLOT+1; i++ ) ctx->h_flag[i] = 0UL;
  HIPCHK( ctx_dev_alloc( ctx, &ctx->d_gcnt, sizeof(unsigned long) ), -1 );
  HIPCHK( hipMemsetAsync( ctx->d_gcnt, 0, sizeof(unsigned long), ctx->stream ), -1 );
  HIPCHK( ctx_pin_alloc( ctx, &ctx->h_stamp, ( 2*FD_NSLOT + 1 ) * sizeof(unsigned long), &ctx->d_stamp ), -1 );
  memset( ctx->h_stamp, 0, ( 2*FD_NSLOT + 1 ) * sizeof(unsigned long) );
  ctx->last_gt = -1;
  if( dbg.cu_exclusive > 0 && fdgpu_ed25519_set_cu_exclusive( ctx, dbg.cu_exclusive ) ) return -1;
  if( dbg.cu_exclusive < 0 ) ctx->excl_mode = -1;
  if( max_payload_bytes && slot_bufs( ctx, 0 ) ) return -1;
  ctx->cur = 0; ctx->rec_fp_off = -1;
  HIPCHK( hipStreamSynchronize( ctx->stream ), -1 );
  gclk_calibrate( ctx );
  return 0;
}

extern "C" void fdgpu_ed25519_set_timing( fdgpu_ed25519_ctx_t * ctx, int enable ) { ctx->timing = enable; ctx->ring_cnt = 0; }

extern "C" float
fdgpu_ed25519_kernel_ms( fdgpu_ed25519_ctx_t * ctx, int idx ) {
  if( idx<0 || idx>4 || !ctx->ring_cnt ) return -1.f;
  unsigned long n = ctx->ring_cnt < (unsigned long)FD_NRING ? ctx->ring_cnt : (unsigned long)FD_NRING;
  static int const from[5] = { 0, 1, 2, 0, 4 }, to[5] = { 1, 2, 3, 4, 1 };
  double sum = 0.;
  for( unsigned long r=0; r<n; r++ ) {
    float ms = 0.f;
    if( hipEventElapsedTime( &ms, ctx->ring[r][ from[idx] ], ctx->ring[r][ to[idx] ] ) != hipSuccess ) return -1.f;
    sum += ms;
  }
  return (float)( sum / (double)n );
}

__global__ void __launch_bounds__( 256 )
fd_mad_probe_kernel( u32 iters, u32 seed, u64 * out ) {
  u64 acc[16]; u32 a = seed + threadIdx.x, b = seed ^ (blockIdx.x * 2654435761u);
#pragma unroll
  for( int i=0; i<16; i++ ) acc[i] = (u64)(a + i) << 7;
  for( u32 it=0; it<iters; it++ ) {
#pragma unroll
    for( int i=0; i<16; i++ ) {
      asm volatile( "v_mad_u64_u32 %0, vcc, %1, %2, %0" : "+v"(acc[i]) : "v"(a), "v"(b) : "vcc" );
    }
  }
  u64 x = 0;
#pragma unroll
  for( int i=0; i<16; i++ ) x ^= acc[i];
  if( x == 0x1234567ull ) out[0] = x;
}

extern "C" double
fdgpu_mad_peak_per_s( int device ) {
// ... 1221 lines not shown
  __atomic_store_n( &ctx->dbg_fail_issue, on ? 1 : 0, __ATOMIC_RELEASE );
}

extern "C" void
fdgpu_ed25519_debug_fault( fdgpu_ed25519_ctx_t * ctx ) {
  if( !ctx ) return;
  ctx->fault = 1;
  fd_err = "fdgpu_ed25519_poll: batch failed: injected by fdgpu_ed25519_debug_fault";
}

extern "C" unsigned long
fdgpu_ed25519_slow_count( fdgpu_ed25519_ctx_t * ctx ) {
  if( !ctx || !ctx->half ) return 0UL;
  if( hipSetDevice( ctx->device ) != hipSuccess || hipStreamSynchronize( ctx->stream ) != hipSuccess ) return ~0UL;
  u32 cnt = 0u;
  if( hipMemcpy( &cnt, slow_word( ctx, FD_SW_SLOW ), sizeof(u32), hipMemcpyDeviceToHost ) != hipSuccess ) return ~0UL;
  return (unsigned long)cnt;
}

extern "C" unsigned long
fdgpu_ed25519_key_count( fdgpu_ed25519_ctx_t * ctx ) {
  if( !ctx || !ctx->half || !ctx->key_dedup || ctx->last_path != FDGPU_PATH_THROUGHPUT ) return 0UL;
  if( hipSetDevice( ctx->device ) != hipSuccess || hipStreamSynchronize( ctx->stream ) != hipSuccess ) return ~0UL;
  u32 cnt = 0u;
  if( hipMemcpy( &cnt, slow_word( ctx, FD_SW_KEYS ), sizeof(u32), hipMemcpyDeviceToHost ) != hipSuccess ) return ~0UL;
  return (unsigned long)cnt;
}

extern "C" int
fdgpu_ed25519_hot_count( fdgpu_ed25519_ctx_t * ctx, unsigned long * hot_keys, unsigned long * hot_sigs ) {
  if( hot_keys ) *hot_keys = 0UL;
  if( hot_sigs ) *hot_sigs = 0UL;
  if( !ctx || !ctx->half || !ctx->key_split || ctx->last_path != FDGPU_PATH_THROUGHPUT ) return 0;
  if( hipSetDevice( ctx->device ) != hipSuccess || hipStreamSynchronize( ctx->stream ) != hipSuccess ) return -1;
  u32 cnt[ 5 ] = { 0u, 0u, 0u, 0u, 0u };
  if( hipMemcpy( cnt, slow_word( ctx, FD_SW_HOT ), sizeof(cnt), hipMemcpyDeviceToHost ) != hipSuccess ) return -1;
  if( ctx->key_fixed ) { cnt[0] += cnt[FD_KC_FBK] < ctx->fb_cap ? cnt[FD_KC_FBK] : ctx->fb_cap; cnt[1] += cnt[FD_KC_FB]; }
  if( hot_keys ) *hot_keys = (unsigned long)cnt[0];
  if( hot_sigs ) *hot_sigs = (unsigned long)cnt[1];
  return 0;
}

extern "C" int
fdgpu_ed25519_fixed_count( fdgpu_ed25519_ctx_t * ctx, unsigned long * fixed_keys, unsigned long * fixed_sigs ) {
  if( fixed_keys ) *fixed_keys = 0UL;
  if( fixed_sigs ) *fixed_sigs = 0UL;
  if( !ctx || !ctx->half || !ctx->key_fixed || ctx->last_path != FDGPU_PATH_THROUGHPUT ) return 0;
  if( hipSetDevice( ctx->device ) != hipSuccess || hipStreamSynchronize( ctx->stream ) != hipSuccess ) return -1;
  u32 cnt[ 2 ] = { 0u, 0u };
  if( hipMemcpy( cnt, slow_word( ctx, FD_SW_HOT ) + FD_KC_FBK, sizeof(cnt), hipMemcpyDeviceToHost ) != hipSuccess ) return -1;
  if( cnt[0] > ctx->fb_cap ) cnt[0] = ctx->fb_cap;
  if( fixed_keys ) *fixed_keys = (unsigned long)cnt[0];
  if( fixed_sigs ) *fixed_sigs = (unsigned long)cnt[1];
  return 0;
}

extern "C" int
fdgpu_ed25519_fcache_count( fdgpu_ed25519_ctx_t * ctx, unsigned long * hits, unsigned long * builds ) {
  if( hits ) *hits = 0UL;
  if( builds ) *builds = 0UL;
  if( !ctx || !ctx->half || !ctx->key_fixed || ctx->last_path != FDGPU_PATH_THROUGHPUT ) return 0;
  if( hipSetDevice( ctx->device ) != hipSuccess || hipStreamSynchronize( ctx->stream ) != hipSuccess ) return -1;
  u32 cnt[ 3 ] = { 0u, 0u, 0u };
  if( hipMemcpy( cnt, slow_word( ctx, FD_SW_HOT ) + FD_KC_HIT, sizeof(cnt), hipMemcpyDeviceToHost ) != hipSuccess ) return -1;
  if( hits ) *hits = (unsigned long)cnt[0];
  if( builds ) *builds = (unsigned long)cnt[2];
  return 0;
}

extern "C" int
fdgpu_ed25519_ffull_count( fdgpu_ed25519_ctx_t * ctx, unsigned long * keys, unsigned long * sigs ) {
  if( keys ) *keys = 0UL;
  if( sigs ) *sigs = 0UL;
  if( !ctx || !ctx->half || !ctx->key_fixed || ctx->last_path != FDGPU_PATH_THROUGHPUT ) return 0;
  if( hipSetDevice( ctx->device ) != hipSuccess || hipStreamSynchronize( ctx->stream ) != hipSuccess ) return -1;
  u32 cnt[ 2 ] = { 0u, 0u };
  if( hipMemcpy( cnt, slow_word( ctx, FD_SW_HOT ) + FD_KC_FFK, sizeof(cnt), hipMemcpyDeviceToHost ) != hipSuccess ) return -1;
  if( keys ) *keys = (unsigned long)cnt[0];
  if( sigs ) *sigs = (unsigned long)cnt[1];
  return 0;
}

extern "C" int
fdgpu_ed25519_pinned_count( fdgpu_ed25519_ctx_t * ctx, unsigned long * keys, unsigned long * sigs ) {
  if( keys ) *keys = 0UL;
  if( sigs ) *sigs = 0UL;
  if( !ctx || !ctx->half || !ctx->key_fixed || ctx->last_path != FDGPU_PATH_THROUGHPUT ) return 0;
  if( hipSetDevice( ctx->device ) != hipSuccess || hipStreamSynchronize( ctx->stream ) != hipSuccess ) return -1;
  u32 cnt[ 2 ] = { 0u, 0u };
  if( hipMemcpy( cnt, slow_word( ctx, FD_SW_HOT ) + FD_KC_PINK, sizeof(cnt), hipMemcpyDeviceToHost ) != hipSuccess ) return -1;
  if( keys ) *keys = (unsigned long)cnt[0];
  if( sigs ) *sigs = (unsigned long)cnt[1];
  return 0;
}

extern "C" unsigned long
fdgpu_ed25519_pin_cap( fdgpu_ed25519_ctx_t * ctx ) {
  if( !ctx || !ctx->half || !ctx->key_fixed ) return 0UL;
  return fd_pin_list_cap( ctx->fb_cap );
}

extern "C" int
fdgpu_ed25519_set_pinned_keys( fdgpu_ed25519_ctx_t * ctx, unsigned char const * keys, unsigned long n,
                               unsigned char * status_out ) {
  if( !ctx || ( n && !keys ) ) { fd_err = "fdgpu_ed25519_set_pinned_keys: bad arguments"; return -1; }
  if( n > fdgpu_ed25519_pin_cap( ctx ) ) { fd_err = "fdgpu_ed25519_set_pinned_keys: more keys than fdgpu_ed25519_pin_cap"; return -1; }
  if( async_busy( ctx ) ) { fd_err = "fdgpu_ed25519_set_pinned_keys: the async pipeline holds a batch"; return -2; }
  if( ctx->fault ) { fd_err = "fdgpu_ed25519_set_pinned_keys: the context is faulted"; return -3; }
  if( !ctx->key_fixed ) return 0;
  std::vector<unsigned int> slot_of( n ? n : 1UL ), first_of( n ? n : 1UL ), work( fd_pin_list_work( n ) );
  unsigned long m = fd_pin_list_dedup( keys, n, slot_of.data(), first_of.data(), work.data() );
  std::vector<unsigned char> uniq( 32UL * ( m ? m : 1UL ) ), st( m ? m : 1UL );
  for( unsigned long j=0UL; j<m; j++ ) memcpy( uniq.data() + 32UL*j, keys + 32UL*first_of[j], 32UL );
  HIPCHK( hipSetDevice( ctx->device ), -3 );
  HIPCHK( hipStreamSynchronize( ctx->stream ), -3 );
  ctx->npin = 0u; ctx->kc_dirty = 1;
  if( m ) {
    hipStream_t s = ctx->stream;
    u32 * pcnt = (u32 *)ctx->d_Rxy;
    HIPCHK( hipMemcpy( ctx->d_skey, uniq.data(), 32UL*m, hipMemcpyHostToDevice ), -3 );
    hipLaunchKernelGGL( fd_keypin_kernel, dim3( (unsigned)( ( (unsigned long)FD_FB_NT * m + FD_WG - 1UL ) / FD_WG ) ), dim3(FD_WG), 0, s,
                        (u32)m, (u32 const *)ctx->d_skey, ctx->d_sstat, ctx->d_fbase, ctx->d_flist, pcnt );
    hipLaunchKernelGGL( fd_ftab_kernel, dim3( (unsigned)( ( 4UL * m + 1UL ) / 2UL ) ), dim3(FD_WG), 0, s, (u32 const *)pcnt,
                        (u32 const *)ctx->d_flist, (unsigned char const *)ctx->d_sstat, (uint4 const *)ctx->d_fbase,
                        ctx->d_ftab, 4u, (u32 const *)ctx->d_plist, 0u );
    HIPCHK( hipGetLastError(), -3 );
    HIPCHK( hipStreamSynchronize( s ), -3 );
    HIPCHK( hipMemcpy( st.data(), ctx->d_sstat, m, hipMemcpyDeviceToHost ), -3 );
  }
  if( status_out ) for( unsigned long i=0UL; i<n; i++ ) status_out[i] = st[ slot_of[i] ];
  ctx->npin = (u32)m;
  return 0;
}

extern "C" unsigned long
fdgpu_ed25519_front_remaining( fdgpu_ed25519_ctx_t const * ctx ) {
  if( ctx->inflight.empty() ) return 0UL;
  fd_slot const & sl = ctx->slot[ ctx->inflight.front() ];
  return sl.txn_cnt - sl.cursor;
}

extern "C" int
fdgpu_ed25519_front_batch( fdgpu_ed25519_ctx_t const * ctx, unsigned long * txn_cnt, unsigned long * cursor, int * path ) {
  if( ctx->inflight.empty() ) { *txn_cnt = 0UL; *cursor = 0UL; *path = FDGPU_PATH_NONE; return 0; }
  fd_slot const & sl = ctx->slot[ ctx->inflight.front() ];
  *txn_cnt = sl.txn_cnt; *cursor = sl.cursor; *path = sl.path;
  return 1;
}

extern "C" void
fdgpu_ed25519_pipeline_state( fdgpu_ed25519_ctx_t const * ctx, unsigned long * filling, unsigned long * inflight ) {
  *filling  = ctx->slot[ ctx->cur ].state==0 ? ctx->slot[ ctx->cur ].txn_cnt : 0UL;
  *inflight = (unsigned long)ctx->inflight.size();
}

extern "C" unsigned long
fdgpu_ed25519_poll( fdgpu_ed25519_ctx_t * ctx, unsigned long * out_tags, signed char * out_codes,
                    unsigned long max, int blocking ) {
  return poll_any( ctx, out_tags, out_codes, NULL, NULL, NULL, max, blocking );
}

extern "C" unsigned long
fdgpu_ed25519_poll_raw( fdgpu_ed25519_ctx_t * ctx, unsigned long * out_tags, signed char * out_codes,
                        unsigned char * out_img, unsigned short * out_fp, unsigned long * out_dedup, unsigned long max,
                        int blocking ) {
  return poll_any( ctx, out_tags, out_codes, out_img, out_fp, out_dedup, max, blocking );
}

extern "C" void
fdgpu_ed25519_set_dedup( fdgpu_ed25519_ctx_t * ctx, int enable, unsigned long seed ) {
  ctx->dedup = enable ? 1 : 0; ctx->dedup_seed = seed;
}

extern "C" int
fdgpu_ed25519_set_dedup_seeds( fdgpu_ed25519_ctx_t * ctx, unsigned long const * seeds, int n ) {
  if( n < 0 || n > 16 || ( n && !seeds ) ) { fd_err = "fdgpu_ed25519_set_dedup_seeds: 0..16 seeds"; return -1; }
  for( int i=0; i<16; i++ ) __atomic_store_n( &ctx->dedup_seeds[i], i < n ? seeds[i] : 0UL, __ATOMIC_RELAXED );
  __atomic_store_n( &ctx->dedup_nseed, n, __ATOMIC_RELEASE );
  ctx->dedup = 1;
  return 0;
}

extern "C" int
fdgpu_ed25519_set_record_fp_off( fdgpu_ed25519_ctx_t * ctx, int off ) {
  if( off < -1 || off > 253 ) { fd_err = "bad record footprint offset"; return -1; }
  ctx->rec_fp_off = off;
  return 0;
}


static std::mutex g_mu;
static fdgpu_ed25519_ctx_t * g_ctx = NULL;

static int g_dropin_device = 0, g_dropin_semantics = FDGPU_SEMANTICS_AVX512;

static fdgpu_ed25519_ctx_t * global_ctx( void ) {
  if( g_ctx ) return g_ctx;
  g_ctx = fdgpu_ed25519_ctx_new( g_dropin_device, 64, 64, 1UL<<17, g_dropin_semantics );
  return g_ctx;
}

extern "C" int
fdgpu_ed25519_dropin_init( int device, int semantics ) {
  if( semantics!=FDGPU_SEMANTICS_AVX512 && semantics!=FDGPU_SEMANTICS_REF ) { fd_err = "bad semantics"; return -1; }
  std::lock_guard<std::mutex> lk( g_mu );
  if( g_ctx && ( g_ctx->device != device || g_ctx->semantics != semantics ) ) { fdgpu_ed25519_ctx_delete( g_ctx ); g_ctx = NULL; }
  g_dropin_device = device; g_dropin_semantics = semantics;
  return global_ctx() ? 0 : -2;
// ... 82 lines not shown
```

### firedancer_amd/csrc/fd_gpu_lattice.h

```cpp
#pragma once

#include <stdint.h>

#ifndef FD_LAT_FN
#if defined(__HIPCC__)
#define FD_LAT_FN __device__ __forceinline__
#else
#define FD_LAT_FN static inline
#endif
#endif

#define FD_LAT_MAXIT  10
#define FD_LAT_MAXIN  64
#define FD_LAT_BITS   159

#define FD_LAT_N8L { 0xe7ae9f68u, 0xc09318d2u, 0x17bce6b2u, 0xa6f7cef5u, 0u, 0u, 0u, 0x80000000u }

FD_LAT_FN int fd_lat_bitlen8( uint32_t const x[ 8 ] ) {
  int b = 0;
#pragma unroll
  for( int i=0; i<8; i++ ) b = x[i] ? 32*i + 32 - __builtin_clz( x[i] ) : b;
  return b;
}

// ... 212 lines not shown
      if( bs > a ) { s--; bs >>= 1; }
      uint64_t n00 = (uint64_t)m00 + ( (uint64_t)m10 << s ), n01 = (uint64_t)m01 + ( (uint64_t)m11 << s );
      if( ( n00 | n01 ) >> 31 ) break;
      a -= bs; m00 = (uint32_t)n00; m01 = (uint32_t)n01; steps++;
      if( a < b ) {
        uint64_t ta = a; a = b; b = ta;
        uint32_t t0 = m00; m00 = m10; m10 = t0;
        uint32_t t1 = m01; m01 = m11; m11 = t1;
      }
    }
    if( !steps ) {
      int s = L - fd_lat_bitlen8( R1 ) - 1;
      s = s < 0 ? 0 : ( s > 30 ? 30 : s );
      m00 = 1u; m01 = 1u << s; m10 = 0u; m11 = 1u;
    }
    uint32_t nR0[ 8 ], nR1[ 8 ], nT0[ 5 ], nT1[ 5 ];
    int n0 = fd_lat_comb8( nR0, m00, R0, m01, R1, &ovf );
    int n1 = fd_lat_comb8( nR1, m11, R1, m10, R0, &ovf );
    fd_lat_combT( nT0, m00, T0, m01, T1, n0 );
    fd_lat_combT( nT1, m11, T1, m10, T0, n1 );
    int sw = fd_lat_lt8( nR0, nR1 );
#pragma unroll
    for( int i=0; i<8; i++ ) { R0[i] = sw ? nR1[i] : nR0[i]; R1[i] = sw ? nR0[i] : nR1[i]; }
#pragma unroll
    for( int i=0; i<5; i++ ) { T0[i] = sw ? nT1[i] : nT0[i]; T1[i] = sw ? nT0[i] : nT1[i]; }
  }
  if( ovf | ( fd_lat_bitlen8( R1 ) > FD_LAT_SKEW_T ) ) return 0;

  uint32_t cr[ 8 ] = { 0u, 0u, 0u, 0u, 0u, 0u, 0u, 0u }, ct[ 5 ] = { 0u, 0u, 0u, 0u, 0u };
  int best = 1 << 20;
#pragma unroll 1
  for( int c=0; c<4; c++ ) {
    uint32_t dr[ 8 ], dt[ 5 ], da[ 5 ];
    int o2 = 0;
    if( c < 3 ) {
      uint32_t x = c != 0, y = c != 1;
      int ng = fd_lat_comb8( dr, x, R0, y, R1, &o2 );
      fd_lat_combT( dt, x, T0, y, T1, ng );
    } else {
      fd_lat_sum8( dr, R0, R1, &o2 );
      fd_lat_sum5( dt, T0, T1 );
    }
    fd_lat_abs5( da, dt );
    uint32_t da8[ 8 ] = { da[0], da[1], da[2], da[3], da[4], 0u, 0u, 0u };
    int nw = fd_lat_skew_windows( fd_lat_bitlen8( dr ), fd_lat_bitlen8( da8 ) );
    if( ( da[0] & 1u ) && !o2 && nw < best ) {
      best = nw;
#pragma unroll
      for( int i=0; i<8; i++ ) cr[i] = dr[i];
#pragma unroll
      for( int i=0; i<5; i++ ) ct[i] = dt[i];
    }
  }
  if( best > FD_LAT_SKEW_NW ) return 0;
  *c1neg = fd_lat_abs5( c1m, ct );
#pragma unroll
  for( int i=0; i<7; i++ ) c0[i] = cr[i];
  *nwin = best;
  return (int)( c1m[0] & 1u ) & ( cr[7] == 0u );
}

FD_LAT_FN int fd_fb_recode( signed char d[ 32 ], uint32_t const k[ 8 ] ) {
  int carry = 0;
#pragma unroll
  for( int j=0; j<32; j++ ) {
    int v = (int)( ( k[ j >> 2 ] >> ( 8*( j & 3 ) ) ) & 255u ) + carry;
    carry = ( v + 128 ) >> 8;
    d[j] = (signed char)( v - ( carry << 8 ) );
  }
  return carry;
}

#define FD_FB_NT        32
#define FD_FB_NB        16
#define FD_FB_FULL_ADDS 48
FD_LAT_FN int fd_fb_entry( int d ) { return d < 0 ? -d : d; }
FD_LAT_FN int fd_fb_old_adds( int r ) { return ( r & 1 ) ? 8 : 16; }
FD_LAT_FN int fd_fb_old_is_base( int i ) { return i >= 8; }
FD_LAT_FN int fd_fb_old_digit( int r, int i ) { return i < 8 ? 4*i + r : 2*( i - 8 ) + ( r >> 1 ); }
FD_LAT_FN int fd_fb_old_table( int i ) { return i < 8 ? 4*i : 2*( i - 8 ); }
FD_LAT_FN int fd_fb_full_is_base( int i ) { return ( i % 3 ) == 2; }
FD_LAT_FN int fd_fb_full_digit( int i ) { return ( i % 3 ) == 2 ? i / 3 : 2*( i / 3 ) + ( i % 3 ); }
FD_LAT_FN int fd_fb_full_table( int i ) { return fd_fb_full_digit( i ); }
```

### firedancer_amd/csrc/fd_lat_host.c

```c
#include "fd_gpu_lattice.h"

int
fd_lat_halfsize_host( uint32_t c0[ 5 ], uint32_t c1m[ 5 ], int * c1neg, uint32_t const k[ 8 ] ) {
  return fd_lat_halfsize( c0, c1m, c1neg, k );
}

int
fd_lat_skew_host( uint32_t c0[ 7 ], uint32_t c1m[ 5 ], int * c1neg, int * nwin, uint32_t const k[ 8 ] ) {
  return fd_lat_skew( c0, c1m, c1neg, nwin, k );
}

void
fd_lat_skew_host_many( unsigned long n, uint32_t const * k, uint32_t * c0, uint32_t * c1m, int * neg, int * nwin,
                       int * ok ) {
  for( unsigned long i=0UL; i<n; i++ ) {
    neg[i] = 0; nwin[i] = 0;
    ok[i] = fd_lat_skew( c0 + 7UL*i, c1m + 5UL*i, neg + i, nwin + i, k + 8UL*i );
  }
}

int
fd_fb_recode_host( signed char d[ 32 ], uint32_t const k[ 8 ] ) {
  return fd_fb_recode( d, k );
}

int
fd_fb_old_sched_host( int r, int * out ) {
  int na = fd_fb_old_adds( r );
  for( int i=0; i<na; i++ ) { out[3*i] = fd_fb_old_is_base( i ); out[3*i+1] = fd_fb_old_digit( r, i ); out[3*i+2] = fd_fb_old_table( i ); }
  return na;
}

int
fd_fb_full_sched_host( int * out ) {
  for( int i=0; i<FD_FB_FULL_ADDS; i++ ) { out[3*i] = fd_fb_full_is_base( i ); out[3*i+1] = fd_fb_full_digit( i ); out[3*i+2] = fd_fb_full_table( i ); }
  return FD_FB_FULL_ADDS;
}

int
fd_fb_entry_host( int d ) { return fd_fb_entry( d ); }

int
fd_fb_tables_host( int * nt, int * nb ) { *nt = FD_FB_NT; *nb = FD_FB_NB; return 0; }
```

### firedancer_amd/engine.py

```python
from __future__ import annotations

import ctypes
import os
import threading

import numpy as np

PKG_DIR = os.path.dirname(os.path.abspath(__file__))
LIB_PATH = os.environ.get("FDGPU_LIB") or os.path.join(PKG_DIR, "libfdgpu_ed25519.so")

FD_ED25519_SUCCESS = 0
FD_ED25519_ERR_SIG = -1
FD_ED25519_ERR_PUBKEY = -2
FD_ED25519_ERR_MSG = -3
SEMANTICS_AVX512 = 0
SEMANTICS_REF = 1

DESC_DTYPE = np.dtype([("payload_off", "<u4"), ("sig_base", "<u4"), ("payload_sz", "<u2"),
                       ("message_off", "<u2"), ("acct_addr_off", "<u2"), ("signature_off", "u1"),
                       ("sig_cnt", "u1")])
assert DESC_DTYPE.itemsize == 16
RAW_DTYPE = np.dtype([("payload_off", "<u4"), ("sig_base", "<u4"), ("payload_sz", "<u2"), ("sig_lanes", "u1"),
                      ("_pad", "u1", (5,))])
assert RAW_DTYPE.itemsize == 16
FDGPU_ERR_PARSE = -16
FDGPU_ERR_OVERRUN = -17
TXN_IMG_STRIDE = 864

EXPORTS = ("fd_ed25519_verify", "fd_ed25519_verify_batch_single_msg", "fd_ed25519_strerror",
           "fdgpu_ed25519_ctx_new", "fdgpu_ed25519_ctx_delete", "fdgpu_ed25519_verify_txns_device",
           "fdgpu_ed25519_verify_txns_host", "fdgpu_txn_parse_device", "fdgpu_ed25519_verify_raw_device",
           "fdgpu_ed25519_verify_raw_host", "fdgpu_ed25519_submit", "fdgpu_ed25519_flush",
           "fdgpu_ed25519_poll", "fdgpu_ed25519_submit_raw", "fdgpu_ed25519_poll_raw", "fdgpu_ed25519_submit_raw_ref",
           "fdgpu_host_alloc", "fdgpu_host_free", "fdgpu_host_register", "fdgpu_host_unregister", "fdgpu_device_numa_node",
           "fdgpu_ed25519_submit_raw_gather", "fdgpu_ed25519_submit_raw_gather_chk", "fdgpu_ed25519_gather",
           "fdgpu_ed25519_gathered", "fdgpu_ed25519_gather_launched", "fdgpu_ed25519_gather_wait", "fdgpu_host_dev_ptr", "fdgpu_host_register_shared",
           "fdgpu_ed25519_reserve_gather_cus", "fdgpu_ed25519_reserve_cus", "fdgpu_ed25519_set_cu_exclusive", "fdgpu_ed25519_get_cu_exclusive", "fdgpu_ed25519_set_lat_share", "fdgpu_ed25519_gather_stats", "fdgpu_ed25519_phase_stats", "fdgpu_ed25519_prepare", "fdgpu_ed25519_submit_raw_gather_dev", "fdgpu_host_region",
           "fdgpu_ed25519_dropin_init", "fdgpu_debug_set_opts", "fdgpu_debug_gather_pauses",
           "fdgpu_ed25519_pipeline_state", "fdgpu_ed25519_verify_many_host", "fdgpu_sha512_batch_device", "fdgpu_sha512_batch_host", "fdgpu_ed25519_set_timing", "fdgpu_ed25519_set_small_batch_max", "fdgpu_ed25519_kernel_ms", "fdgpu_mad_peak_per_s",
           "fdgpu_ed25519_faulted", "fdgpu_ed25519_debug_fault", "fdgpu_ed25519_slow_count", "fdgpu_ed25519_key_count", "fdgpu_ed25519_hot_count", "fdgpu_ed25519_fixed_count", "fdgpu_ed25519_fcache_count", "fdgpu_ed25519_ffull_count", "fdgpu_ed25519_set_pinned_keys", "fdgpu_ed25519_pin_cap", "fdgpu_ed25519_pinned_count", "fdgpu_ed25519_set_dedup",
           "fdgpu_ed25519_set_record_fp_off", "fdgpu_ed25519_batch_stats", "fdgpu_ed25519_launch_stats", "fdgpu_ed25519_front_remaining", "fdgpu_ed25519_front_batch", "fdgpu_ed25519_verify_txn_ptrs",
           "fdgpu_ed25519_submit_raw_gather_dev_f", "fdgpu_launcher_new", "fdgpu_launcher_delete", "fdgpu_launcher_stats", "fdgpu_ed25519_set_launcher",
           "fdgpu_ed25519_submit_raw_gather_to", "fdgpu_ed25519_set_dedup_seeds", "fdgpu_ed25519_debug_fail_launch",
           "fdgpu_last_error")

_lib = None
_lock = threading.Lock()
_u8p = ctypes.POINTER(ctypes.c_uint8)


def load_library():
    global _lib
    with _lock:
        if _lib is not None:
            return _lib
        if not os.path.exists(LIB_PATH):
            raise RuntimeError(f"{LIB_PATH} not built: run `python -c 'import __graft_entry__ as g; g.build()'`")
        try:
            import torch
            if getattr(torch.version, "hip", None):
                torch.cuda.device_count()
        except ImportError:
            pass
        L = ctypes.CDLL(LIB_PATH)
        L.fd_ed25519_verify.restype = ctypes.c_int
        L.fd_ed25519_verify.argtypes = [_u8p, ctypes.c_ulong, _u8p, _u8p, ctypes.c_void_p]
        L.fd_ed25519_verify_batch_single_msg.restype = ctypes.c_int
        L.fd_ed25519_verify_batch_single_msg.argtypes = [_u8p, ctypes.c_ulong, _u8p, _u8p, ctypes.c_void_p, ctypes.c_uint8]
        L.fd_ed25519_strerror.restype = ctypes.c_char_p
        L.fd_ed25519_strerror.argtypes = [ctypes.c_int]
        L.fdgpu_ed25519_ctx_new.restype = ctypes.c_void_p
        L.fdgpu_ed25519_ctx_new.argtypes = [ctypes.c_int, ctypes.c_ulong, ctypes.c_ulong, ctypes.c_ulong, ctypes.c_int]
        L.fdgpu_ed25519_ctx_delete.argtypes = [ctypes.c_void_p]
        L.fdgpu_ed25519_verify_txns_device.restype = ctypes.c_int
        L.fdgpu_ed25519_verify_txns_device.argtypes = [ctypes.c_void_p, ctypes.c_void_p, ctypes.c_void_p, ctypes.c_ulong,
                                                      ctypes.c_ulong, ctypes.c_void_p, ctypes.c_void_p, ctypes.c_void_p]
        L.fdgpu_ed25519_verify_txns_host.restype = ctypes.c_int
        L.fdgpu_ed25519_verify_txns_host.argtypes = [ctypes.c_void_p, ctypes.c_void_p, ctypes.c_ulong, ctypes.c_void_p,
                                                    ctypes.c_ulong, ctypes.c_void_p, ctypes.c_void_p]
        L.fdgpu_txn_parse_device.restype = ctypes.c_int
        L.fdgpu_txn_parse_device.argtypes = [ctypes.c_void_p, ctypes.c_void_p, ctypes.c_ulong, ctypes.c_void_p,
                                             ctypes.c_ulong, ctypes.c_void_p, ctypes.c_void_p]
        L.fdgpu_ed25519_verify_raw_device.restype = ctypes.c_int
        L.fdgpu_ed25519_verify_raw_device.argtypes = [ctypes.c_void_p, ctypes.c_void_p, ctypes.c_void_p, ctypes.c_ulong,
                                                      ctypes.c_ulong, ctypes.c_void_p, ctypes.c_void_p, ctypes.c_ulong,
                                                      ctypes.c_void_p, ctypes.c_void_p]
        L.fdgpu_ed25519_verify_raw_host.restype = ctypes.c_int
        L.fdgpu_ed25519_verify_raw_host.argtypes = [ctypes.c_void_p, ctypes.c_void_p, ctypes.c_ulong, ctypes.c_void_p,
                                                    ctypes.c_ulong, ctypes.c_void_p, ctypes.c_void_p, ctypes.c_ulong,
                                                    ctypes.c_void_p]
        L.fdgpu_ed25519_verify_many_host.restype = ctypes.c_int
        L.fdgpu_ed25519_verify_many_host.argtypes = [ctypes.c_void_p] * 5 + [ctypes.c_ulong, ctypes.c_void_p]
        L.fdgpu_sha512_batch_device.restype = ctypes.c_int
        L.fdgpu_sha512_batch_device.argtypes = [ctypes.c_void_p] * 3 + [ctypes.c_ulong, ctypes.c_void_p, ctypes.c_void_p]
        L.fdgpu_sha512_batch_host.restype = ctypes.c_int
        L.fdgpu_sha512_batch_host.argtypes = [ctypes.c_int, ctypes.c_void_p, ctypes.c_ulong, ctypes.c_void_p,
                                              ctypes.c_void_p, ctypes.c_ulong, ctypes.c_void_p]
        L.fdgpu_ed25519_submit.restype = ctypes.c_int
        L.fdgpu_ed25519_submit.argtypes = [ctypes.c_void_p, ctypes.c_void_p, ctypes.c_ushort, ctypes.c_ubyte,
                                           ctypes.c_ushort, ctypes.c_ushort, ctypes.c_ubyte, ctypes.c_ulong]
        L.fdgpu_ed25519_flush.restype = ctypes.c_int
        L.fdgpu_ed25519_flush.argtypes = [ctypes.c_void_p]
        L.fdgpu_ed25519_poll.restype = ctypes.c_ulong
        L.fdgpu_ed25519_poll.argtypes = [ctypes.c_void_p, ctypes.c_void_p, ctypes.c_void_p, ctypes.c_ulong, ctypes.c_int]
        L.fdgpu_ed25519_submit_raw.restype = ctypes.c_int
        L.fdgpu_ed25519_submit_raw.argtypes = [ctypes.c_void_p, ctypes.c_void_p, ctypes.c_ushort, ctypes.c_ulong]
        L.fdgpu_ed25519_poll_raw.restype = ctypes.c_ulong
        L.fdgpu_ed25519_poll_raw.argtypes = [ctypes.c_void_p, ctypes.c_void_p, ctypes.c_void_p, ctypes.c_void_p,
                                             ctypes.c_void_p, ctypes.c_void_p, ctypes.c_ulong, ctypes.c_int]
        L.fdgpu_ed25519_set_dedup.argtypes = [ctypes.c_void_p, ctypes.c_int, ctypes.c_ulong]
        L.fdgpu_ed25519_set_record_fp_off.restype = ctypes.c_int
        L.fdgpu_ed25519_set_record_fp_off.argtypes = [ctypes.c_void_p, ctypes.c_int]
        L.fdgpu_ed25519_set_timing.argtypes = [ctypes.c_void_p, ctypes.c_int]
        L.fdgpu_ed25519_set_cu_exclusive.restype = ctypes.c_int
        L.fdgpu_ed25519_set_cu_exclusive.argtypes = [ctypes.c_void_p, ctypes.c_int]
        L.fdgpu_ed25519_set_lat_share.restype = ctypes.c_int
        L.fdgpu_ed25519_set_lat_share.argtypes = [ctypes.c_void_p, ctypes.c_uint]
        L.fdgpu_ed25519_front_batch.restype = ctypes.c_int
        L.fdgpu_ed25519_front_batch.argtypes = [ctypes.c_void_p, ctypes.POINTER(ctypes.c_ulong),
                                                ctypes.POINTER(ctypes.c_ulong), ctypes.POINTER(ctypes.c_int)]
        L.fdgpu_ed25519_set_small_batch_max.restype = ctypes.c_ulong
        L.fdgpu_ed25519_set_small_batch_max.argtypes = [ctypes.c_void_p, ctypes.c_ulong]
        L.fdgpu_ed25519_kernel_ms.restype = ctypes.c_float
        L.fdgpu_ed25519_kernel_ms.argtypes = [ctypes.c_void_p, ctypes.c_int]
        L.fdgpu_ed25519_pipeline_state.argtypes = [ctypes.c_void_p, ctypes.c_void_p, ctypes.c_void_p]
        L.fdgpu_ed25519_verify_txn_ptrs.restype = ctypes.c_int
        L.fdgpu_ed25519_verify_txn_ptrs.argtypes = [ctypes.c_void_p] * 3 + [ctypes.c_ulong, ctypes.c_void_p]
        L.fdgpu_ed25519_faulted.restype = ctypes.c_int
        L.fdgpu_ed25519_faulted.argtypes = [ctypes.c_void_p]
        L.fdgpu_ed25519_debug_fault.argtypes = [ctypes.c_void_p]
        L.fdgpu_ed25519_slow_count.restype = ctypes.c_ulong
        L.fdgpu_ed25519_slow_count.argtypes = [ctypes.c_void_p]
        L.fdgpu_ed25519_key_count.restype = ctypes.c_ulong
        L.fdgpu_ed25519_key_count.argtypes = [ctypes.c_void_p]
        L.fdgpu_ed25519_hot_count.restype = ctypes.c_int
        L.fdgpu_ed25519_hot_count.argtypes = [ctypes.c_void_p, ctypes.c_void_p, ctypes.c_void_p]
        L.fdgpu_ed25519_fixed_count.restype = ctypes.c_int
        L.fdgpu_ed25519_fixed_count.argtypes = [ctypes.c_void_p, ctypes.c_void_p, ctypes.c_void_p]
        L.fdgpu_ed25519_fcache_count.restype = ctypes.c_int
        L.fdgpu_ed25519_fcache_count.argtypes = [ctypes.c_void_p, ctypes.c_void_p, ctypes.c_void_p]
        L.fdgpu_ed25519_ffull_count.restype = ctypes.c_int
        L.fdgpu_ed25519_ffull_count.argtypes = [ctypes.c_void_p, ctypes.c_void_p, ctypes.c_void_p]
        L.fdgpu_ed25519_set_pinned_keys.restype = ctypes.c_int
        L.fdgpu_ed25519_set_pinned_keys.argtypes = [ctypes.c_void_p, ctypes.c_void_p, ctypes.c_ulong, ctypes.c_void_p]
        L.fdgpu_ed25519_pin_cap.restype = ctypes.c_ulong
        L.fdgpu_ed25519_pin_cap.argtypes = [ctypes.c_void_p]
        L.fdgpu_ed25519_pinned_count.restype = ctypes.c_int
        L.fdgpu_ed25519_pinned_count.argtypes = [ctypes.c_void_p, ctypes.c_void_p, ctypes.c_void_p]
        L.fdgpu_ed25519_submit_raw_ref.restype = ctypes.c_int
        L.fdgpu_ed25519_submit_raw_ref.argtypes = [ctypes.c_void_p, ctypes.c_void_p, ctypes.c_void_p, ctypes.c_ushort,
                                                   ctypes.c_ulong]
        L.fdgpu_ed25519_submit_raw_gather.restype = ctypes.c_int
        L.fdgpu_ed25519_submit_raw_gather.argtypes = [ctypes.c_void_p, ctypes.c_void_p, ctypes.c_void_p, ctypes.c_void_p,
                                                      ctypes.c_ushort, ctypes.c_ushort, ctypes.c_ushort, ctypes.c_ulong]
        L.fdgpu_ed25519_submit_raw_gather_chk.restype = ctypes.c_int
        L.fdgpu_ed25519_submit_raw_gather_chk.argtypes = [ctypes.c_void_p, ctypes.c_void_p, ctypes.c_void_p,
                                                          ctypes.c_void_p, ctypes.c_ushort, ctypes.c_ushort,
                                                          ctypes.c_ushort, ctypes.c_ulong, ctypes.c_void_p, ctypes.c_ulong]
        L.fdgpu_ed25519_gather.restype = ctypes.c_long
        L.fdgpu_ed25519_gather.argtypes = [ctypes.c_void_p]
        L.fdgpu_ed25519_gathered.restype = ctypes.c_ulong
        L.fdgpu_ed25519_gathered.argtypes = [ctypes.c_void_p]
        L.fdgpu_ed25519_gather_launched.restype = ctypes.c_ulong
        L.fdgpu_ed25519_gather_launched.argtypes = [ctypes.c_void_p]
        L.fdgpu_ed25519_gather_wait.restype = ctypes.c_int
        L.fdgpu_ed25519_gather_wait.argtypes = [ctypes.c_void_p]
        L.fdgpu_host_dev_ptr.restype = ctypes.c_void_p
        L.fdgpu_host_dev_ptr.argtypes = [ctypes.c_void_p, ctypes.c_ulong]
        L.fdgpu_ed25519_dropin_init.restype = ctypes.c_int
        L.fdgpu_ed25519_dropin_init.argtypes = [ctypes.c_int, ctypes.c_int]
        L.fdgpu_debug_set_opts.argtypes = [ctypes.c_void_p]
        L.fdgpu_host_alloc.restype = ctypes.c_void_p
        L.fdgpu_host_alloc.argtypes = [ctypes.c_ulong]
        L.fdgpu_host_free.argtypes = [ctypes.c_void_p]
        L.fdgpu_last_error.restype = ctypes.c_char_p
        _lib = L
        return L


def last_error() -> str:
    return load_library().fdgpu_last_error().decode()


class DebugOpts(ctypes.Structure):
    _fields_ = [("half", ctypes.c_int), ("half_force_slow", ctypes.c_uint), ("small_batch_max", ctypes.c_long),
                ("dsm_lanes", ctypes.c_int), ("nofold_max", ctypes.c_long), ("gather_no_writeback", ctypes.c_int),
                ("poll_prefetch", ctypes.c_int), ("gather_rpb", ctypes.c_int), ("gather_cu_spread", ctypes.c_int),
                ("cu_exclusive", ctypes.c_int), ("quad_sha", ctypes.c_int), ("key_dedup", ctypes.c_int),
                ("key_split", ctypes.c_int), ("key_fixed", ctypes.c_int), ("key_cache", ctypes.c_int),
                ("key_full", ctypes.c_int)]


def debug_set_opts(half: int = -1, half_force_slow: int = 0, small_batch_max: int = -1, dsm_lanes: int = 0,
                   nofold_max: int = -1, gather_no_writeback: int = 0, poll_prefetch: int = 0,
                   gather_rpb: int = 0, gather_cu_spread: int = 0, cu_exclusive: int = 0, quad_sha: int = 0,
                   key_dedup: int = 0, key_split: int = 0, key_fixed: int = 0, key_cache: int = 0,
                   key_full: int = 0) -> None:
    o = DebugOpts(half=half, half_force_slow=half_force_slow,
                  small_batch_max=min(small_batch_max, 2**63 - 1), dsm_lanes=dsm_lanes, nofold_max=nofold_max,
                  gather_no_writeback=gather_no_writeback, poll_prefetch=poll_prefetch, gather_rpb=gather_rpb,
                  gather_cu_spread=gather_cu_spread, cu_exclusive=cu_exclusive, quad_sha=quad_sha, key_dedup=key_dedup,
                  key_split=key_split, key_fixed=key_fixed, key_cache=key_cache, key_full=key_full)
    load_library().fdgpu_debug_set_opts(ctypes.byref(o))


def gather_pauses(reset: bool = True, n: int = 512) -> tuple[int, list]:
    L = load_library()
    L.fdgpu_debug_gather_pauses.restype = ctypes.c_ulong
    L.fdgpu_debug_gather_pauses.argtypes = [ctypes.c_void_p, ctypes.c_ulong, ctypes.c_int]
    buf = np.zeros(2 * n, np.uint64)
    tot = int(L.fdgpu_debug_gather_pauses(buf.ctypes.data, n, 1 if reset else 0))
    m = min(tot, n)
    return tot, [(int(buf[2 * i]), int(buf[2 * i + 1])) for i in range(m)]


def debug_reset_opts() -> None:
    load_library().fdgpu_debug_set_opts(None)


def dropin_init(device: int = 0, semantics: int = SEMANTICS_AVX512) -> None:
    rc = load_library().fdgpu_ed25519_dropin_init(device, semantics)
    if rc:
        raise RuntimeError(f"fdgpu_ed25519_dropin_init: {rc} {last_error()}")


def _buf(b: bytes):
    a = np.frombuffer(bytes(b) + b"\0", np.uint8)
    return a, a.ctypes.data_as(_u8p)


def fd_ed25519_verify(msg: bytes, sig: bytes, public_key: bytes) -> int:
    L = load_library()
    m, mp = _buf(msg); s, sp = _buf(sig); p, pp = _buf(public_key)
    return L.fd_ed25519_verify(mp, len(msg), sp, pp, None)


def fd_ed25519_verify_batch_single_msg(msg: bytes, signatures: bytes, pubkeys: bytes, batch_sz: int) -> int:
    L = load_library()
    m, mp = _buf(msg); s, sp = _buf(signatures); p, pp = _buf(pubkeys)
    return L.fd_ed25519_verify_batch_single_msg(mp, len(msg), sp, pp, None, batch_sz & 0xff)


def txn_parse_device(d_payload: int, d_raw: int, txn_cnt: int, d_img: int | None, d_fp: int,
                     stream: int | None = None, img_stride: int = TXN_IMG_STRIDE) -> None:
    rc = load_library().fdgpu_txn_parse_device(d_payload, d_raw, txn_cnt, d_img, img_stride, d_fp, stream)
    if rc:
        raise RuntimeError(f"fdgpu_txn_parse_device: {rc} {last_error()}")


def sha512_batch(msgs, device: int = 0) -> list[bytes]:
    L = load_library()
    off = np.zeros(len(msgs), np.uint64)
    sz = np.zeros(len(msgs), np.uint32)
    pos = 0
    for i, m in enumerate(msgs):
        off[i], sz[i] = pos, len(m)
        pos += len(m)
    data = np.frombuffer(b"".join(bytes(m) for m in msgs) + b"\0", np.uint8)
    out = np.zeros((len(msgs), 64), np.uint8)
    rc = L.fdgpu_sha512_batch_host(device, data.ctypes.data, pos, off.ctypes.data, sz.ctypes.data, len(msgs),
                                   out.ctypes.data)
    if rc:
        raise RuntimeError(f"fdgpu_sha512_batch_host: {rc} {last_error()}")
    return [out[i].tobytes() for i in range(len(msgs))]


def raw_records(payload: np.ndarray, off: np.ndarray, sz: np.ndarray):
    raw = np.zeros(len(off), RAW_DTYPE)
    raw["payload_off"] = off
    raw["payload_sz"] = sz
    b0 = np.where(np.asarray(sz) > 0, payload[np.minimum(off, len(payload) - 1)], 0)
    lanes = np.where((b0 >= 1) & (b0 <= 16), b0, 0).astype(np.uint32)
    raw["sig_lanes"] = lanes
    raw["sig_base"] = np.concatenate([[0], np.cumsum(lanes)[:-1]]).astype(np.uint32) if len(off) else []
    return raw, int(lanes.sum())


def host_register(buf: np.ndarray) -> None:
    L = load_library()
    if L.fdgpu_host_register(ctypes.c_void_p(buf.ctypes.data), ctypes.c_ulong(buf.nbytes)):
        raise RuntimeError("fdgpu_host_register failed: " + last_error())


def host_unregister(buf: np.ndarray) -> None:
    load_library().fdgpu_host_unregister(ctypes.c_void_p(buf.ctypes.data))
# ... 109 lines not shown
        if rc:
            raise RuntimeError(f"fdgpu_ed25519_verify_raw_host: {rc} {last_error()}")
        return codes, fp, img

    def verify_raw_device(self, d_payload: int, d_raw: int, txn_cnt: int, sig_cnt: int, d_txn_out: int,
                          d_img: int | None = None, d_fp: int | None = None, stream: int | None = None):
        rc = self.L.fdgpu_ed25519_verify_raw_device(self.ctx, d_payload, d_raw, txn_cnt, sig_cnt, d_txn_out, d_img,
                                                    TXN_IMG_STRIDE, d_fp, stream)
        if rc:
            raise RuntimeError(f"fdgpu_ed25519_verify_raw_device: {rc} {last_error()}")

    def submit(self, payload: bytes, signature_off: int, acct_addr_off: int, message_off: int,
               sig_cnt: int, tag: int) -> int:
        b = np.frombuffer(payload, np.uint8)
        rc = self.L.fdgpu_ed25519_submit(self.ctx, b.ctypes.data, len(payload), signature_off, acct_addr_off,
                                         message_off, sig_cnt, tag)
        if rc <= -3:
            raise RuntimeError(f"fdgpu_ed25519_submit: {rc} {last_error()}")
        return rc

    def flush(self):
        rc = self.L.fdgpu_ed25519_flush(self.ctx)
        if rc:
            raise RuntimeError(f"fdgpu_ed25519_flush: {rc} {last_error()}")

    def submit_raw(self, payload: bytes, tag: int) -> int:
        b = np.frombuffer(payload, np.uint8) if len(payload) else np.zeros(1, np.uint8)
        rc = self.L.fdgpu_ed25519_submit_raw(self.ctx, b.ctypes.data, len(payload), tag)
        if rc <= -3:
            raise RuntimeError(f"fdgpu_ed25519_submit_raw: {rc} {last_error()}")
        return rc

    def set_dedup(self, enable: bool, seed: int = 0):
        self.L.fdgpu_ed25519_set_dedup(self.ctx, 1 if enable else 0, seed)

    def poll_raw(self, max_n: int = 4096, blocking: bool = False, dedup: bool = False):
        tags = np.zeros(max_n, np.uint64)
        codes = np.zeros(max_n, np.int8)
        fp = np.zeros(max_n, np.uint16)
        img = np.zeros((max_n, TXN_IMG_STRIDE), np.uint8)
        dt = np.zeros(max_n, np.uint64)
        n = self.L.fdgpu_ed25519_poll_raw(self.ctx, tags.ctypes.data, codes.ctypes.data, img.ctypes.data,
                                          fp.ctypes.data, dt.ctypes.data, max_n, 1 if blocking else 0)
        if dedup:
            return tags[:n], codes[:n], fp[:n], img[:n], dt[:n]
        return tags[:n], codes[:n], fp[:n], img[:n]

    def faulted(self) -> bool:
        return bool(self.L.fdgpu_ed25519_faulted(self.ctx))

    def debug_fault(self):
        self.L.fdgpu_ed25519_debug_fault(self.ctx)

    def slow_count(self) -> int:
        return int(self.L.fdgpu_ed25519_slow_count(self.ctx))

    def key_count(self) -> int:
        return int(self.L.fdgpu_ed25519_key_count(self.ctx))

    def hot_count(self) -> tuple[int, int]:
        k, s = ctypes.c_ulong(), ctypes.c_ulong()
        if self.L.fdgpu_ed25519_hot_count(self.ctx, ctypes.byref(k), ctypes.byref(s)):
            raise RuntimeError("fdgpu_ed25519_hot_count: " + last_error())
        return int(k.value), int(s.value)

    def fixed_count(self) -> tuple[int, int]:
        k, s = ctypes.c_ulong(), ctypes.c_ulong()
        if self.L.fdgpu_ed25519_fixed_count(self.ctx, ctypes.byref(k), ctypes.byref(s)):
            raise RuntimeError("fdgpu_ed25519_fixed_count: " + last_error())
        return int(k.value), int(s.value)

    def fcache_count(self) -> tuple[int, int]:
        h, b = ctypes.c_ulong(), ctypes.c_ulong()
        if self.L.fdgpu_ed25519_fcache_count(self.ctx, ctypes.byref(h), ctypes.byref(b)):
            raise RuntimeError("fdgpu_ed25519_fcache_count: " + last_error())
        return int(h.value), int(b.value)

    def ffull_count(self) -> tuple[int, int]:
        k, s = ctypes.c_ulong(), ctypes.c_ulong()
        if self.L.fdgpu_ed25519_ffull_count(self.ctx, ctypes.byref(k), ctypes.byref(s)):
            raise RuntimeError("fdgpu_ed25519_ffull_count: " + last_error())
        return int(k.value), int(s.value)

    def set_pinned_keys(self, keys) -> np.ndarray:
        keys = [bytes(k) for k in keys]
        if any(len(k) != 32 for k in keys):
            raise ValueError("a public key has 32 bytes")
        buf = np.frombuffer(b"".join(keys) + b"\0", np.uint8)
        status = np.zeros(max(len(keys), 1), np.uint8)
        rc = self.L.fdgpu_ed25519_set_pinned_keys(self.ctx, buf.ctypes.data, len(keys), status.ctypes.data)
        if rc:
            raise RuntimeError(f"fdgpu_ed25519_set_pinned_keys: {rc} {last_error()}", rc)
        return status[:len(keys)]

    def pin_cap(self) -> int:
        return int(self.L.fdgpu_ed25519_pin_cap(self.ctx))

    def pinned_count(self) -> tuple[int, int]:
        k, s = ctypes.c_ulong(), ctypes.c_ulong()
        if self.L.fdgpu_ed25519_pinned_count(self.ctx, ctypes.byref(k), ctypes.byref(s)):
            raise RuntimeError("fdgpu_ed25519_pinned_count: " + last_error())
        return int(k.value), int(s.value)

    def poll(self, max_n: int = 4096, blocking: bool = False):
        tags = np.zeros(max_n, np.uint64)
        codes = np.zeros(max_n, np.int8)
        n = self.L.fdgpu_ed25519_poll(self.ctx, tags.ctypes.data, codes.ctypes.data, max_n, 1 if blocking else 0)
        return tags[:n], codes[:n]
```

### include/fd_ed25519_gpu.h

```cpp
#ifndef HEADER_fd_ed25519_gpu_h
#define HEADER_fd_ed25519_gpu_h


#ifdef __cplusplus
extern "C" {
#endif

#ifndef FD_ED25519_SUCCESS
#define FD_ED25519_SUCCESS    ( 0)
#define FD_ED25519_ERR_SIG    (-1)
#define FD_ED25519_ERR_PUBKEY (-2)
#define FD_ED25519_ERR_MSG    (-3)
#endif

#ifndef HEADER_fd_src_ballet_sha512_fd_sha512_h
typedef struct fd_sha512_private fd_sha512_t;
#endif


int
fd_ed25519_verify( unsigned char const   msg[],
                   unsigned long         msg_sz,
                   unsigned char const   sig[ 64 ],
                   unsigned char const   public_key[ 32 ],
// ... 117 lines not shown
fdgpu_ed25519_verify_txn_ptrs( fdgpu_ed25519_ctx_t *         ctx,
                               unsigned char const * const * payloads,
                               fdgpu_txn_desc_t const *      desc,
                               unsigned long                 cnt,
                               signed char *                 out );

int
fdgpu_sha512_batch_device( unsigned char const * d_data,
                           unsigned long const * d_off,
                           unsigned int const *  d_sz,
                           unsigned long         cnt,
                           unsigned char *       d_hash,
                           void *                stream );

int
fdgpu_sha512_batch_host( int                   device,
                         unsigned char const * data,
                         unsigned long         data_sz,
                         unsigned long const * off,
                         unsigned int const *  sz,
                         unsigned long         cnt,
                         unsigned char *       hash );

int
fdgpu_ed25519_submit( fdgpu_ed25519_ctx_t * ctx,
                      unsigned char const * payload,
                      unsigned short        payload_sz,
                      unsigned char         signature_off,
                      unsigned short        acct_addr_off,
                      unsigned short        message_off,
                      unsigned char         sig_cnt,
                      unsigned long         tag );

int
fdgpu_ed25519_flush( fdgpu_ed25519_ctx_t * ctx );

#define FDGPU_LAT_BUCKETS (40)
static inline int fdgpu_lat_bucket( unsigned long ns ) {
  if( ns < 32000UL ) return 0;
  int oct = 63 - __builtin_clzl( ns / 32000UL );
  unsigned long base = 32000UL << oct;
  int quarter = ( ns*10000UL >= base*11892UL ) + ( ns*10000UL >= base*14142UL ) + ( ns*10000UL >= base*16818UL );
  int b = 1 + 4*oct + quarter;
  return b < FDGPU_LAT_BUCKETS - 1 ? b : FDGPU_LAT_BUCKETS - 1;
}
void
fdgpu_ed25519_batch_stats( fdgpu_ed25519_ctx_t const * ctx, unsigned long * batches, unsigned long * txns,
                           unsigned long hist[ FDGPU_LAT_BUCKETS ] );

void
fdgpu_ed25519_launch_stats( fdgpu_ed25519_ctx_t const * ctx, unsigned long * launch_ns, unsigned long * launches );

typedef struct fdgpu_launcher fdgpu_launcher_t;
fdgpu_launcher_t * fdgpu_launcher_new( int device, int cpu );
void               fdgpu_launcher_delete( fdgpu_launcher_t * launcher );
void               fdgpu_launcher_stats( fdgpu_launcher_t const * launcher, unsigned long out[ 6 ] );
int                fdgpu_ed25519_set_launcher( fdgpu_ed25519_ctx_t * ctx, fdgpu_launcher_t * launcher );

int
fdgpu_ed25519_faulted( fdgpu_ed25519_ctx_t const * ctx );

void
fdgpu_ed25519_debug_fault( fdgpu_ed25519_ctx_t * ctx );
void
fdgpu_ed25519_debug_fail_launch( fdgpu_ed25519_ctx_t * ctx, int on );

unsigned long
fdgpu_ed25519_slow_count( fdgpu_ed25519_ctx_t * ctx );

unsigned long
fdgpu_ed25519_key_count( fdgpu_ed25519_ctx_t * ctx );

int
fdgpu_ed25519_hot_count( fdgpu_ed25519_ctx_t * ctx, unsigned long * hot_keys, unsigned long * hot_sigs );

int
fdgpu_ed25519_fixed_count( fdgpu_ed25519_ctx_t * ctx, unsigned long * fixed_keys, unsigned long * fixed_sigs );

int
fdgpu_ed25519_fcache_count( fdgpu_ed25519_ctx_t * ctx, unsigned long * hits, unsigned long * builds );

int
fdgpu_ed25519_ffull_count( fdgpu_ed25519_ctx_t * ctx, unsigned long * keys, unsigned long * sigs );

int
fdgpu_ed25519_set_pinned_keys( fdgpu_ed25519_ctx_t * ctx, unsigned char const * keys, unsigned long n,
                               unsigned char * status_out );

unsigned long
fdgpu_ed25519_pin_cap( fdgpu_ed25519_ctx_t * ctx );

int
fdgpu_ed25519_pinned_count( fdgpu_ed25519_ctx_t * ctx, unsigned long * keys, unsigned long * sigs );

unsigned long
fdgpu_ed25519_poll( fdgpu_ed25519_ctx_t * ctx,
                    unsigned long *       out_tags,
                    signed char *         out_codes,
                    unsigned long         max,
                    int                   blocking );

unsigned long
fdgpu_ed25519_front_remaining( fdgpu_ed25519_ctx_t const * ctx );

#define FDGPU_PATH_THROUGHPUT       (0)
#define FDGPU_PATH_THROUGHPUT_FULL  (-1)
#define FDGPU_PATH_NONE             (-2)
int
fdgpu_ed25519_front_batch( fdgpu_ed25519_ctx_t const * ctx, unsigned long * txn_cnt, unsigned long * cursor,
                           int * path );

void
fdgpu_ed25519_pipeline_state( fdgpu_ed25519_ctx_t const * ctx,
                              unsigned long *             filling,
                              unsigned long *             inflight );

int
fdgpu_ed25519_submit_raw( fdgpu_ed25519_ctx_t * ctx,
                          unsigned char const * payload,
                          unsigned short        payload_sz,
                          unsigned long         tag );

int
fdgpu_ed25519_submit_raw_ref( fdgpu_ed25519_ctx_t * ctx,
                              unsigned char const * base,
                              unsigned char const * payload,
                              unsigned short        payload_sz,
                              unsigned long         tag );

void * fdgpu_host_alloc( unsigned long sz );
void   fdgpu_host_free ( void * p );

int    fdgpu_host_register       ( void * p, unsigned long sz );
int    fdgpu_host_register_shared( void * p, unsigned long sz );
void   fdgpu_host_unregister     ( void * p );

int    fdgpu_device_numa_node( int device );

int
fdgpu_ed25519_submit_raw_gather( fdgpu_ed25519_ctx_t * ctx,
                                 unsigned char const * src,
                                 unsigned char *       dst_base,
                                 unsigned char *       dst,
                                 unsigned short        copy_sz,
                                 unsigned short        payload_off,
                                 unsigned short        payload_sz,
                                 unsigned long         tag );

int
fdgpu_ed25519_submit_raw_gather_chk( fdgpu_ed25519_ctx_t * ctx,
                                     unsigned char const * src,
                                     unsigned char *       dst_base,
                                     unsigned char *       dst,
                                     unsigned short        copy_sz,
                                     unsigned short        payload_off,
                                     unsigned short        payload_sz,
                                     unsigned long         tag,
                                     unsigned long const * seq_addr,
                                     unsigned long         seq );

long          fdgpu_ed25519_gather( fdgpu_ed25519_ctx_t * ctx );
unsigned long fdgpu_ed25519_gathered( fdgpu_ed25519_ctx_t const * ctx );
unsigned long fdgpu_ed25519_gather_launched( fdgpu_ed25519_ctx_t const * ctx );
int           fdgpu_ed25519_reserve_gather_cus( fdgpu_ed25519_ctx_t * ctx, unsigned n );
int           fdgpu_ed25519_reserve_cus( fdgpu_ed25519_ctx_t * ctx, unsigned n, unsigned part, unsigned parts );
void          fdgpu_ed25519_gather_stats( fdgpu_ed25519_ctx_t * ctx, unsigned long out[ 8 ] );
void          fdgpu_ed25519_phase_stats( fdgpu_ed25519_ctx_t const * ctx, unsigned long out[ 9 ] );
int           fdgpu_ed25519_prepare( fdgpu_ed25519_ctx_t * ctx, int raw );
int           fdgpu_ed25519_submit_raw_gather_dev( fdgpu_ed25519_ctx_t * ctx, unsigned char const * src,
                                                   unsigned char const * src_dev, unsigned char * dst_base,
                                                   unsigned char * dst, unsigned short copy_sz, unsigned short payload_off,
                                                   unsigned short payload_sz, unsigned long tag,
                                                   unsigned long const * seq_dev, unsigned long seq );
#define FDGPU_GATHER_NO_WRITEBACK (1U)
int           fdgpu_ed25519_submit_raw_gather_dev_f( fdgpu_ed25519_ctx_t * ctx, unsigned char const * src,
                                                     unsigned char const * src_dev, unsigned char * dst_base,
                                                     unsigned char * dst, unsigned short copy_sz,
                                                     unsigned short payload_off, unsigned short payload_sz,
                                                     unsigned long tag, unsigned long const * seq_dev,
                                                     unsigned long seq, unsigned flags );
#define FDGPU_GATHER_SEED( i ) ( ( (unsigned)(i) & 15u ) << 8 )
int           fdgpu_ed25519_set_dedup_seeds( fdgpu_ed25519_ctx_t * ctx, unsigned long const * seeds, int n );
int           fdgpu_ed25519_submit_raw_gather_to( fdgpu_ed25519_ctx_t * ctx, unsigned char const * src,
                                                  unsigned char const * src_dev, unsigned char * dst_dev,
                                                  unsigned short copy_sz, unsigned short payload_off,
                                                  unsigned short payload_sz, unsigned long tag,
                                                  unsigned long const * seq_dev, unsigned long seq, unsigned flags );
int           fdgpu_host_region( void const * p, void ** base, unsigned long * sz, void ** dev_base );
int           fdgpu_ed25519_gather_wait( fdgpu_ed25519_ctx_t * ctx );

void * fdgpu_host_dev_ptr( void const * p, unsigned long sz );

unsigned long
fdgpu_ed25519_poll_raw( fdgpu_ed25519_ctx_t * ctx,
                        unsigned long *       out_tags,
                        signed char *         out_codes,
                        unsigned char *       out_img,
                        unsigned short *      out_fp,
                        unsigned long *       out_dedup,
                        unsigned long         max,
                        int                   blocking );

void
fdgpu_ed25519_set_dedup( fdgpu_ed25519_ctx_t * ctx, int enable, unsigned long seed );

int
fdgpu_ed25519_set_record_fp_off( fdgpu_ed25519_ctx_t * ctx, int off );

unsigned long
fdgpu_ed25519_set_small_batch_max( fdgpu_ed25519_ctx_t * ctx, unsigned long small_max );

int
fdgpu_ed25519_set_cu_exclusive( fdgpu_ed25519_ctx_t * ctx, int on );
int
fdgpu_ed25519_get_cu_exclusive( fdgpu_ed25519_ctx_t const * ctx );

int
fdgpu_ed25519_set_lat_share( fdgpu_ed25519_ctx_t * ctx, unsigned parts );

void
fdgpu_ed25519_set_timing( fdgpu_ed25519_ctx_t * ctx, int enable );

float
fdgpu_ed25519_kernel_ms( fdgpu_ed25519_ctx_t * ctx, int idx );

double
fdgpu_mad_peak_per_s( int device );

int
fdgpu_ed25519_dropin_init( int device, int semantics );

typedef struct fdgpu_debug_opts {
  int           half;
  unsigned int  half_force_slow;
  long          small_batch_max;
  int           dsm_lanes;
  long          nofold_max;
  int           gather_no_writeback;
  int           poll_prefetch;
  int           gather_rpb;
  int           gather_cu_spread;
  int           cu_exclusive;
  int           quad_sha;
  int           key_dedup;
  int           key_split;
  int           key_fixed;
  int           key_cache;
  int           key_full;
} fdgpu_debug_opts_t;

void
fdgpu_debug_set_opts( fdgpu_debug_opts_t const * opts );

unsigned long
fdgpu_debug_gather_pauses( unsigned long * out, unsigned long n, int reset );

char const *
fdgpu_last_error( void );

#ifdef __cplusplus
}
#endif

#endif
```

Measured before the change: 307.8 million sigs/s.

## Add wide-window fixed-base tables for cached keys to cut point additions

Adds a second, wider precomputed table per cached public key that uses 11-bit signed windows over spans of the A scalar. Warps whose keys all have wide tables then do 40 additions instead of the existing full-table count. Extra wbase and wtab build kernels populate these tables for the first FD_FB_WCAP cache slots, and new counters report how often the path is taken. The cost is much more table-build work and memory per key, plus larger random table fetches. The benchmark uses 1M synthetic transactions, likely with mostly unique keys, so the wide path may rarely run and the extra kernel launches and grid items could add overhead.

```diff
diff --git a/firedancer_amd/csrc/fd_ed25519_gpu.hip b/firedancer_amd/csrc/fd_ed25519_gpu.hip
--- a/firedancer_amd/csrc/fd_ed25519_gpu.hip
+++ b/firedancer_amd/csrc/fd_ed25519_gpu.hip
@@ -144,6 +144,8 @@
 #define FD_KC_FFS   13
 #define FD_KC_PINK  14
 #define FD_KC_PINS  15
+#define FD_KC_FWK   16
+#define FD_KC_FWS   17
 
 
 __global__ void __launch_bounds__( FD_WG )
@@ -236,7 +238,8 @@
                   u32 const *              __restrict__ fidx,
                   u32 const *              __restrict__ birth,
                   u32                                   batch,
-                  u32 const *              __restrict__ full ) {
+                  u32 const *              __restrict__ full,
+                  u32                                   wcap ) {
   u32 s, is_r;
   unsigned char * st;
   if( ulist ) {
@@ -253,6 +256,7 @@
       if( fidx && kcnt[s] >= fb_min ) {
         u32 slot = fidx[s];
         if( slot != FD_FB_NONE && full[slot] ) atomicAdd( ucnt + 3 + FD_KC_FFK, 1u );
+        if( slot < wcap && full[slot] ) atomicAdd( ucnt + 3 + FD_KC_FWK, 1u );
         if( slot != FD_FB_NONE && birth[slot] != batch ) return;
       }
     } else if( order ) {
@@ -660,16 +664,32 @@
 }
 
 template<int FM = FD_CARRY_FOLD>
-FD_DEV void fbase_chain( uint4 * __restrict__ fbase, u32 fi, u32 j, ge_p3 & A, int nd ) {
+FD_DEV void chain_store( uint4 * __restrict__ b, ge_p3 & A, int nd ) {
 #pragma unroll 1
   for( int i=0; i<nd; i++ ) ge_p3_dbl<FM>( A, A );
   ge_cached c;
   ge_p3_to_cached<FM>( c, A );
-  uint4 * b = fbase + ( (size_t)fi * FD_FB_NT + j ) * 8;
   fe_store_packed( b + 0, c.YpX );
   fe_store_packed( b + 2, c.YmX );
   fe_store_packed( b + 4, c.Z   );
   fe_store_packed( b + 6, c.T2d );
+}
+template<int FM = FD_CARRY_FOLD>
+FD_DEV void fbase_chain( uint4 * __restrict__ fbase, u32 fi, u32 j, ge_p3 & A, int nd ) {
+  chain_store<FM>( fbase + ( (size_t)fi * FD_FB_NT + j ) * 8, A, nd );
+}
+FD_DEV void cached_to_dbl_input( ge_p3 & A, uint4 const * __restrict__ e ) {
+  fe ypx, ymx;
+  fe_from_quads( ypx, e[0], e[1] ); fe_from_quads( ymx, e[2], e[3] ); fe_from_quads( A.Z, e[4], e[5] );
+  fe_sub( A.X, ypx, ymx ); fe_wcarry( A.X, A.X );
+  fe_add( A.Y, ypx, ymx ); fe_wcarry( A.Y, A.Y );
+  fe_add( A.Z, A.Z, A.Z ); fe_wcarry( A.Z, A.Z ); A.T = fe_zero();
+}
+FD_DEV void wbase_chain( uint4 * __restrict__ wbase, uint4 const * __restrict__ fbase, u32 fi, u32 q ) {
+  u32 t = q >> 1, r = ( q & 1u ) + 1u;
+  ge_p3 A;
+  cached_to_dbl_input( A, fbase + ( (size_t)fi * FD_FB_NT + 4u*t ) * 8 );
+  chain_store( wbase + ( (size_t)fi * 16u + q ) * 8, A, 11*(int)r );
 }
 template<int FM = FD_CARRY_FOLD>
 FD_DEV void fbase_build( uint4 * __restrict__ fbase, u32 fi, u32 j, uint4 const * __restrict__ Axy, u32 rep ) {
@@ -685,9 +705,14 @@
 
 __device__ __attribute__(( aligned( 16 ) )) unsigned const fd_ptab_ident_w[ 24 ] = {
   1u,0u,0u,0u, 0u,0u,0u,0u,  1u,0u,0u,0u, 0u,0u,0u,0u,  0u,0u,0u,0u, 0u,0u,0u,0u };
+static unsigned const fd_ptab_ident_host[ 24 ] = {
+  1u,0u,0u,0u, 0u,0u,0u,0u,  1u,0u,0u,0u, 0u,0u,0u,0u,  0u,0u,0u,0u, 0u,0u,0u,0u };
 
 FD_DEV size_t ftab_at( u32 fi, u32 j, u32 e ) {
   return ( ( (size_t)fi * FD_FB_NT + j ) * FD_FB_E + ( e - 1u ) ) * 6;
+}
+FD_DEV size_t wtab_at( u32 fi, u32 t, u32 r, u32 e ) {
+  return ( ( (size_t)fi * 8u * FD_FB_WE + (size_t)fd_fb_wide_off( (int)t, (int)r ) ) + e ) * 6;
 }
 
 template<int I>
@@ -720,30 +745,52 @@
 __global__ void __launch_bounds__( FD_WG, 2 )
 fd_ftab_kernel( u32 const * __restrict__ kscnt, u32 const * __restrict__ flist,
                 unsigned char const * __restrict__ astat, uint4 const * __restrict__ fbase, uint4 * __restrict__ ftab,
-                u32 cg, u32 const * __restrict__ plist, u32 pmax ) {
+                u32 cg, u32 const * __restrict__ plist, u32 pmax,
+                uint4 const * __restrict__ wbase, uint4 * __restrict__ wtab, u32 wcap, u32 wnow ) {
   u32 nk = kscnt[FD_KC_BUILD] * cg;
   u32 np = kscnt[FD_KC_PTIX]; np = np < pmax ? np : pmax;
+  u32 nb = nk + 3u*np;
+  u32 nkw = wcap && wnow ? kscnt[FD_KC_BUILD] * 24u : 0u, nw = wcap ? nkw + 24u*np : 0u;
   u32 bi = blockIdx.x * 2u + ( threadIdx.x >> 7 );
-  if( blockIdx.x * 2u >= nk + 3u*np ) return;
-  if( bi >= nk + 3u*np ) return;
-  u32 fi, grp;
-  if( bi < nk ) {
-    if( astat[ flist[ 2u*( bi / cg ) + 1u ] ] & 7u ) return;
-    fi = flist[ 2u*( bi / cg ) ]; grp = bi % cg;
-  } else { fi = plist[ ( bi - nk ) / 3u ]; grp = ( bi - nk ) % 3u + 1u; }
-  u32 t = 4u*( ( threadIdx.x >> 4 ) & 7u ) + grp, g = threadIdx.x & 15u;
+  if( blockIdx.x * 2u >= nb + nw ) return;
+  if( bi >= nb + nw ) return;
+  u32 fi, grp, t, g;
+  int top = 3;
+  uint4 const * bp; uint4 * ent;
+  if( bi < nb ) {
+    if( bi < nk ) {
+      if( astat[ flist[ 2u*( bi / cg ) + 1u ] ] & 7u ) return;
+      fi = flist[ 2u*( bi / cg ) ]; grp = bi % cg;
+    } else { fi = plist[ ( bi - nk ) / 3u ]; grp = ( bi - nk ) % 3u + 1u; }
+    t = 4u*( ( threadIdx.x >> 4 ) & 7u ) + grp; g = threadIdx.x & 15u;
+    bp = fbase + ( (size_t)fi * FD_FB_NT + t ) * 8;
+    ent = ftab + ftab_at( fi, t, 8u*g + 1u );
+  } else {
+    u32 wi = bi - nb, q;
+    if( wi < nkw ) {
+      if( astat[ flist[ 2u*( wi / 24u ) + 1u ] ] & 7u ) return;
+      fi = flist[ 2u*( wi / 24u ) ]; q = wi % 24u;
+    } else { fi = plist[ ( wi - nkw ) / 24u ]; q = ( wi - nkw ) % 24u; }
+    if( fi >= wcap ) return;
+    t = q / 3u; u32 r = q % 3u;
+    g = threadIdx.x & 127u;
+    u32 gl = (u32)fd_fb_wide_entries( (int)r ) / 8u - 1u; g = g < gl ? g : gl;
+    top = 6;
+    bp = r ? wbase + ( (size_t)fi * 16u + 2u*t + r - 1u ) * 8 : fbase + ( (size_t)fi * FD_FB_NT + 4u*t ) * 8;
+    ent = wtab + wtab_at( fi, t, r, 8u*g + 1u );
+  }
   int lane = (int)( threadIdx.x & 63u );
   ge_cached pc;
   {
-    atab_raw r; uint4 const * b = fbase + ( (size_t)fi * FD_FB_NT + t ) * 8;
-#pragma unroll
-    for( int i=0; i<8; i++ ) r.q[i] = b[i];
+    atab_raw r;
+#pragma unroll
+    for( int i=0; i<8; i++ ) r.q[i] = bp[i];
     atab_unpack( pc, r );
   }
   ge_p3 Q; ge_p3_identity( Q );
   ge_p1p1 tt;
 #pragma unroll 1
-  for( int b=3; b>=0; b-- ) {
+  for( int b=top; b>=0; b-- ) {
     ge_p3_dbl( Q, Q );
     ge_add_cached( tt, Q, pc );
     ge_p3 Qa; ge_p1p1_to_p3( Qa, tt );
@@ -753,7 +800,6 @@
 #pragma unroll 1
   for( int b=0; b<3; b++ ) ge_p3_dbl( Q, Q );
   fe pf[ 8 ];
-  uint4 * ent = ftab + ftab_at( fi, t, 8u*g + 1u );
   ftab_pass1<0>( Q, pc, ent, pf );
   fe one = fe_one(), pre = pf[7], suf = pf[7], u;
 #pragma unroll 1
@@ -1171,6 +1217,38 @@
   fe_store_planar( Pbuf + 20*n + col, n, P.Z );
 }
 
+FD_DEV void wide_fetch( uint4 r[ 6 ], int & d, int i, size_t n, u32 fi, uint4 const * __restrict__ wtab,
+                        uint4 const * __restrict__ btabf, i8 const * __restrict__ dA, short const * __restrict__ dB ) {
+  if( !fd_fb_wide_is_base( i ) ) {
+    int t = fd_fb_wide_span( i ), q = fd_fb_wide_digit( i );
+    i8 const * p = dA + (size_t)( 4*t )*n;
+    d = fd_fb_wide_split( p[0], p[n], p[2*n], p[3*n], q );
+    ptab_fetch( r, wtab + ( d ? wtab_at( fi, (u32)t, (u32)q, (u32)fd_fb_entry( d ) ) : (size_t)0 ) );
+  } else {
+    d = dB[ (size_t)fd_fb_wide_digit( i )*n ];
+    ptab_fetch( r, btabf + ( (size_t)fd_fb_wide_table( i ) * FD_BTAB_ENTRIES + (size_t)fd_fb_entry( d ) ) * 6 );
+  }
+}
+template<int FM>
+FD_DEV void dsmf_wide( u32 col, size_t n, u32 fi, uint4 const * __restrict__ wtab, uint4 const * __restrict__ btabf,
+                       i8 const * __restrict__ digA, short const * __restrict__ digB, u32 * __restrict__ Pbuf ) {
+  ge_p3 P; ge_p3_identity( P );
+  i8 const * dA = digA + col; short const * dB = digB + col;
+  uint4 ra[ 6 ], rb[ 6 ];
+  int da, db;
+  wide_fetch( ra, da, 0, n, fi, wtab, btabf, dA, dB );
+#pragma unroll 1
+  for( int i=0; i<FD_FB_WIDE_ADDS; i+=2 ) {
+    wide_fetch( rb, db, i + 1, n, fi, wtab, btabf, dA, dB );
+    full_add<FM>( P, ra, da );
+    if( i + 2 < FD_FB_WIDE_ADDS ) wide_fetch( ra, da, i + 2, n, fi, wtab, btabf, dA, dB );
+    full_add<FM>( P, rb, db );
+  }
+  fe_store_planar( Pbuf + col, n, P.X );
+  fe_store_planar( Pbuf + 10*n + col, n, P.Y );
+  fe_store_planar( Pbuf + 20*n + col, n, P.Z );
+}
+
 template<int FM, int KS = 0>
 __global__ void __launch_bounds__( FD_WG, FM ? FD_DSMH_MINW : 1 )
 fd_dsmh_kernel( u32                      nsig,
@@ -1201,7 +1279,9 @@
                 uint4 const * __restrict__ btabf,
                 u32 *         __restrict__ Pbuf,
                 u32 const *   __restrict__ full,
-                u32 *         __restrict__ ffcnt ) {
+                u32 *         __restrict__ ffcnt,
+                uint4 const * __restrict__ wtab,
+                u32                        wcap ) {
   size_t n = nsig;
   if( blockIdx.x < nslowblk ) {
     u32 i = blockIdx.x * FD_WG + threadIdx.x;
@@ -1221,10 +1301,15 @@
       u32 fi = walk ? fidx[ arep[s] ] : 0u;
       unsigned long long wm = __ballot( walk );
       int allfull = __all( walk ? full[fi] != 0u : 1 );
+      int allwide = allfull && __all( walk ? fi < wcap : 1 );
       if( !walk ) return;
       if( allfull ) {
-        if( (int)( threadIdx.x & 63u ) == __ffsll( (long long)wm ) - 1 ) atomicAdd( ffcnt, (u32)__popcll( wm ) );
-        dsmf_full<FM>( col, n, fi, ftab, btabf, (i8 const *)digA, digB, Pbuf );
+        if( (int)( threadIdx.x & 63u ) == __ffsll( (long long)wm ) - 1 ) {
+          atomicAdd( ffcnt, (u32)__popcll( wm ) );
+          if( allwide ) atomicAdd( ffcnt + ( FD_KC_FWS - FD_KC_FFS ), (u32)__popcll( wm ) );
+        }
+        if( allwide ) dsmf_wide<FM>( col, n, fi, wtab, btabf, (i8 const *)digA, digB, Pbuf );
+        else dsmf_full<FM>( col, n, fi, ftab, btabf, (i8 const *)digA, digB, Pbuf );
       }
       else dsmf_one<FM>( col, n, fi, ftab, btabf, (i8 const *)digA, digB, Pbuf );
       return;
@@ -2106,7 +2191,7 @@
     u32 * c = ucnt + 3;
     for( int k=0; k<5; k++ ) c[k] = 0u;
     for( int k=FD_KC_HIT; k<=FD_KC_BUILD; k++ ) c[k] = 0u;
-    for( int k=FD_KC_PTIX; k<=FD_KC_PINS; k++ ) c[k] = 0u;
+    for( int k=FD_KC_PTIX; k<=FD_KC_FWS; k++ ) c[k] = 0u;
     if( iblk ) { u32 h = c[FD_KC_HAND] % kc.fcap; c[FD_KC_HAND] = h; c[FD_KC_HAND0] = h; }
   }
   int bypass = ucnt[1] != 0u;
@@ -2261,19 +2346,25 @@
 fd_keyclaim_kernel( u32 const * __restrict__ mlist, u32 * __restrict__ cnt, u32 * __restrict__ fidx,
                     u32 * __restrict__ flist, unsigned char const * __restrict__ payload,
                     fdgpu_txn_desc_t const * __restrict__ desc, u32 const * __restrict__ map, fd_kcache kc,
-                    u32 cblk, uint4 * __restrict__ fbase ) {
+                    u32 cblk, uint4 * __restrict__ fbase,
+                    u32 pblk, uint4 * __restrict__ wbase, u32 wcap ) {
+  if( blockIdx.x >= cblk + pblk ) {
+    u32 i = ( blockIdx.x - cblk - pblk ) * FD_WG + threadIdx.x;
+    u32 np = cnt[FD_KC_PTIX]; np = np < kc.pmax ? np : kc.pmax;
+    if( ( i >> 4 ) >= np ) return;
+    u32 slot = kc.plist[ i >> 4 ];
+    if( slot >= wcap ) return;
+    wbase_chain( wbase, fbase, slot, i & 15u );
+    return;
+  }
   if( blockIdx.x >= cblk ) {
     u32 i = ( blockIdx.x - cblk ) * FD_WG + threadIdx.x;
     u32 np = cnt[FD_KC_PTIX]; np = np < kc.pmax ? np : kc.pmax;
     u32 p = i / 24u, q = i % 24u;
     if( p >= np ) return;
     u32 slot = kc.plist[p], t = q / 3u, r = q % 3u + 1u;
-    uint4 const * e = fbase + ( (size_t)slot * FD_FB_NT + 4u*t ) * 8;
-    fe ypx, ymx; ge_p3 A;
-    fe_from_quads( ypx, e[0], e[1] ); fe_from_quads( ymx, e[2], e[3] ); fe_from_quads( A.Z, e[4], e[5] );
-    fe_sub( A.X, ypx, ymx ); fe_wcarry( A.X, A.X );
-    fe_add( A.Y, ypx, ymx ); fe_wcarry( A.Y, A.Y );
-    fe_add( A.Z, A.Z, A.Z ); fe_wcarry( A.Z, A.Z ); A.T = fe_zero();
+    ge_p3 A;
+    cached_to_dbl_input( A, fbase + ( (size_t)slot * FD_FB_NT + 4u*t ) * 8 );
     fbase_chain( fbase, slot, 4u*t + r, A, 8*(int)r );
     return;
   }
@@ -2324,6 +2415,16 @@
   fe_neg( A.X, A.X ); fe_wcarry( A.X, A.X );
   fe_mul( A.T, A.X, A.Y );
   fbase_chain( fbase, slot, j, A, 8*(int)j );
+}
+
+__global__ void __launch_bounds__( FD_WG )
+fd_wbase_kernel( u32 const * __restrict__ cnt, u32 const * __restrict__ flist, unsigned char const * __restrict__ stat,
+                 uint4 const * __restrict__ fbase, uint4 * __restrict__ wbase, u32 wcap ) {
+  u32 i = blockIdx.x * FD_WG + threadIdx.x;
+  if( ( i >> 4 ) >= cnt[FD_KC_BUILD] ) return;
+  u32 slot = flist[ 2u*( i >> 4 ) ];
+  if( slot >= wcap || ( stat[ flist[ 2u*( i >> 4 ) + 1u ] ] & 7u ) ) return;
+  wbase_chain( wbase, fbase, slot, i & 15u );
 }
 
 struct fd_seeds { u64 seed[ 16 ]; u32 nseed; };
@@ -2632,6 +2733,9 @@
   u32 *   d_orderh;
   uint4 * d_fbase;
   uint4 * d_ftab;
+  u32     wcap;
+  uint4 * d_wbase;
+  uint4 * d_wtab;
   uint4 * d_btabf;
   u32 *   d_fslow;
   hipEvent_t ev[5];
@@ -2805,7 +2909,7 @@
   FD_SW_HOT      = 4,
   FD_SW_FBSLOW   = 9,
   FD_SW_KCACHE   = 10,
-  FD_SW_CNT      = 20 };
+  FD_SW_CNT      = 24 };
 static u32 * slow_word( fdgpu_ed25519_ctx_t const * ctx, int w ) { return ctx->d_slow + ctx->max_sig + w; }
 
 struct fd_batch {
@@ -2850,7 +2954,7 @@
                         ctx->d_pstat, ctx->d_htop, 1, ctx->semantics, (u32 const *)NULL, (u32 const *)NULL,
                         (u32 const *)NULL, (u32 const *)NULL, (uint4 const *)NULL, (uint4 const *)NULL,
                         (u32 const *)NULL, (uint4 const *)NULL, (uint4 const *)NULL, (u32 *)NULL, (u32 const *)NULL,
-                        (u32 *)NULL );
+                        (u32 *)NULL, (uint4 const *)NULL, 0u );
   else
     hipLaunchKernelGGL( ( nsig <= ctx->nofold_max ? fd_dsm_kernel<0> : fd_dsm_kernel<1> ), dim3(sg), dim3(FD_WG), 0, st,
                         nsig, ctx->d_tab, ctx->d_Rxy, ctx->d_digA, ctx->d_digB, ctx->d_btab, code, ctx->d_P, 0 );
@@ -2898,9 +3002,10 @@
                           b.d_payload, b.d_desc, (u32 const *)ctx->d_map, seed, ctx->d_astat, kc );
       if( fkeys ) {
         unsigned cblk = (unsigned)( ( fkeys + FD_WG - 1UL ) / FD_WG ), pbk = (unsigned)( ( 24UL * ctx->pmax + FD_WG - 1 ) / FD_WG );
-        hipLaunchKernelGGL( fd_keyclaim_kernel, dim3( cblk + pbk ), dim3(FD_WG), 0, st,
+        unsigned wbk = ctx->wcap ? (unsigned)( ( 16UL * ctx->pmax + FD_WG - 1 ) / FD_WG ) : 0u;
+        hipLaunchKernelGGL( fd_keyclaim_kernel, dim3( cblk + pbk + wbk ), dim3(FD_WG), 0, st,
                             (u32 const *)ctx->d_mlist, slow_word( ctx, FD_SW_HOT ), ctx->d_fidx, ctx->d_flist, b.d_payload,
-                            b.d_desc, (u32 const *)ctx->d_map, kc, (u32)cblk, ctx->d_fbase );
+                            b.d_desc, (u32 const *)ctx->d_map, kc, (u32)cblk, ctx->d_fbase, (u32)pbk, ctx->d_wbase, ctx->wcap );
       }
     }
     if( ks )
@@ -2916,7 +3021,8 @@
                       kd ? ctx->d_astat : (unsigned char *)NULL, kd ? (u32)sg : 0u, kf ? order : (u32 const *)NULL,
                       (u32 const *)( kf ? ctx->d_orderh : NULL ), kf ? kscnt : (u32 const *)NULL,
                       (u32 const *)( kf ? ctx->d_kcnt : NULL ), kf ? fbm : 0u, (u32 const *)( kf ? ctx->d_fidx : NULL ),
-                      (u32 const *)( kf ? ctx->d_sbirth : NULL ), kc.batch, (u32 const *)( kf ? ctx->d_sfull : NULL ) );
+                      (u32 const *)( kf ? ctx->d_sbirth : NULL ), kc.batch, (u32 const *)( kf ? ctx->d_sfull : NULL ),
+                      kf ? ctx->wcap : 0u );
   if( ctx->timing ) hipEventRecord( b.ev[4], st );
   unsigned hb = ks ? (unsigned)( ( 2UL * ( nsig / ctx->hot_min ) + FD_WG - 1 ) / FD_WG ) : 0u;
   unsigned lpk = kf && ctx->kfull_mode == 2 ? 32u : 8u, cg = lpk / 8u;
@@ -2931,10 +3037,18 @@
                       ks ? ctx->d_htab : (uint4 *)NULL, (u32)hb, (u32 const *)( kf ? ctx->d_orderh : NULL ),
                       (u32 const *)( kf ? ctx->d_flist : NULL ), kf ? ctx->d_fbase : (uint4 *)NULL, (u32)fbk,
                       kf ? ctx->d_sstat : (unsigned char *)NULL, kf ? ctx->d_Rxy : (uint4 *)NULL, (u32)lpk );
-  if( fkeys )
-    hipLaunchKernelGGL( fd_ftab_kernel, dim3( (unsigned)( ( cg * fkeys + 3UL * pkeys + 1UL ) / 2UL ) ), dim3(FD_WG), 0, st, kscnt,
+  if( fkeys ) {
+    unsigned wnow = ctx->wcap && ctx->kfull_mode == 2;
+    unsigned long witems = ctx->wcap ? 24UL * ( ( wnow ? fkeys : 0UL ) + pkeys ) : 0UL;
+    if( wnow )
+      hipLaunchKernelGGL( fd_wbase_kernel, dim3( (unsigned)( ( 16UL * fkeys + FD_WG - 1 ) / FD_WG ) ), dim3(FD_WG), 0, st, kscnt,
+                          (u32 const *)ctx->d_flist, (unsigned char const *)ctx->d_astat, (uint4 const *)ctx->d_fbase,
+                          ctx->d_wbase, ctx->wcap );
+    hipLaunchKernelGGL( fd_ftab_kernel, dim3( (unsigned)( ( cg * fkeys + 3UL * pkeys + witems + 1UL ) / 2UL ) ), dim3(FD_WG), 0, st, kscnt,
                         (u32 const *)ctx->d_flist, (unsigned char const *)ctx->d_astat, (uint4 const *)ctx->d_fbase,
-                        ctx->d_ftab, (u32)cg, (u32 const *)ctx->d_plist, ctx->pmax );
+                        ctx->d_ftab, (u32)cg, (u32 const *)ctx->d_plist, ctx->pmax, (uint4 const *)ctx->d_wbase, ctx->d_wtab,
+                        ctx->wcap, (u32)wnow );
+  }
   if( ctx->timing ) hipEventRecord( b.ev[1], st );
   unsigned nsb = ( sg + 63u ) / 64u;
   int fold = nsig > ctx->nofold_max;
@@ -2946,7 +3060,8 @@
                       (uint4 const *)( ks ? ctx->d_htab : NULL ), (uint4 const *)( ks ? ctx->d_btabh : NULL ),
                       (u32 const *)( kf ? ctx->d_fidx : NULL ), (uint4 const *)( kf ? ctx->d_ftab : NULL ),
                       (uint4 const *)( kf ? ctx->d_btabf : NULL ), kf ? ctx->d_P : (u32 *)NULL,
-                      (u32 const *)( kf ? ctx->d_sfull : NULL ), kf ? slow_word( ctx, FD_SW_HOT ) + FD_KC_FFS : (u32 *)NULL );
+                      (u32 const *)( kf ? ctx->d_sfull : NULL ), kf ? slow_word( ctx, FD_SW_HOT ) + FD_KC_FFS : (u32 *)NULL,
+                      (uint4 const *)( kf ? ctx->d_wtab : NULL ), kf ? ctx->wcap : 0u );
   if( ctx->timing ) hipEventRecord( b.ev[2], st );
   if( fkeys || npin ) {
     u32 const * fcnt = kscnt + FD_KC_FB; u32 * fslow_cnt = slow_word( ctx, FD_SW_FBSLOW );
@@ -2970,7 +3085,7 @@
   hipLaunchKernelGGL( fd_decode_kernel, dim3(sg), dim3(FD_WG), 0, st, b.d_payload, b.d_desc, ctx->d_map, nsig, 0,
                       ctx->d_pstat, ctx->d_Rxy, ctx->d_Axy, (uint4 *)NULL, (uint4 *)NULL, (u32 const *)NULL,
                       (u32 *)NULL, (unsigned char *)NULL, 0u, (u32 const *)NULL, (u32 const *)NULL, (u32 const *)NULL,
-                      (u32 const *)NULL, 0u, (u32 const *)NULL, (u32 const *)NULL, 0u, (u32 const *)NULL );
+                      (u32 const *)NULL, 0u, (u32 const *)NULL, (u32 const *)NULL, 0u, (u32 const *)NULL, 0u );
   hipLaunchKernelGGL( fd_hash_kernel, dim3(sg), dim3(FD_WG), 0, st, b.d_payload, b.d_desc, ctx->d_map, nsig,
                       ctx->semantics, 1, ctx->d_pstat, code, ctx->d_digA, ctx->d_digB, ctx->d_Rxy,
                       (uint4 const *)ctx->d_khash );
@@ -3017,7 +3132,7 @@
 }
 
 static std::mutex g_dbg_mu;
-static fdgpu_debug_opts_t g_dbg = { -1, 0u, -1L, 0, -1L, 0, 0, 0, 0, 0, 0, 0, 0, 0, 0, 0 };
+static fdgpu_debug_opts_t g_dbg = { -1, 0u, -1L, 0, -1L, 0, 0, 0, 0, 0, 0, 0, 0, 0, 0, 0, 0 };
 static void debug_opts_get( fdgpu_debug_opts_t * o ) { std::lock_guard<std::mutex> lk( g_dbg_mu ); *o = g_dbg; }
 
 extern "C" void
@@ -3112,6 +3227,8 @@
         ctx->kc_iwords = iw; ctx->kc_iprobes = ctx->kc_mode == 2 ? 2u : FD_KD_PROBES;
         ctx->kfull_mode = dbg.key_full;
         ctx->pmax = ctx->kfull_mode == 1 ? 0u : ctx->fb_cap / 4u > 1u ? ctx->fb_cap / 4u : 1u;
+        ctx->wcap = dbg.key_wide == 1 ? 0u : dbg.key_wide == 2 ? ctx->fb_cap / 2u
+                  : ctx->fb_cap < (u32)FD_FB_WCAP ? ctx->fb_cap : (u32)FD_FB_WCAP;
       }
       HIPCHK( ctx_dev_alloc( ctx, &ctx->d_kidx, ( (size_t)ctx->kc_iwords + slots ) * sizeof(u32) ), -1 );
       ctx->d_ktab = ctx->d_kidx + ctx->kc_iwords;
@@ -3143,6 +3260,11 @@
           HIPCHK( ctx_dev_alloc( ctx, &ctx->d_orderh, ns * sizeof(u32) ), -1 );
           HIPCHK( ctx_dev_alloc( ctx, &ctx->d_fbase, fcn * FD_FB_NT * 8 * sizeof(uint4) ), -1 );
           HIPCHK( ctx_dev_alloc( ctx, &ctx->d_ftab, fcn * FD_FB_NT * FD_FB_E * 6 * sizeof(uint4) ), -1 );
+          if( ctx->wcap ) {
+            HIPCHK( ctx_dev_alloc( ctx, &ctx->d_wbase, (size_t)ctx->wcap * 16 * 8 * sizeof(uint4) ), -1 );
+            HIPCHK( ctx_dev_alloc( ctx, &ctx->d_wtab, ( (size_t)ctx->wcap * 8 * FD_FB_WE + 1 ) * 6 * sizeof(uint4) ), -1 );
+            HIPCHK( hipMemcpyAsync( ctx->d_wtab, fd_ptab_ident_host, sizeof(fd_ptab_ident_host), hipMemcpyHostToDevice, ctx->stream ), -1 );
+          }
           HIPCHK( ctx_dev_alloc( ctx, &ctx->d_btabf, (size_t)FD_FB_NB * FD_BTAB_ENTRIES * 6 * sizeof(uint4) ), -1 );
           HIPCHK( ctx_dev_alloc( ctx, &ctx->d_fslow, ns * sizeof(u32) ), -1 );
         }
@@ -4530,6 +4652,19 @@
 }
 
 extern "C" int
+fdgpu_ed25519_fwide_count( fdgpu_ed25519_ctx_t * ctx, unsigned long * keys, unsigned long * sigs ) {
+  if( keys ) *keys = 0UL;
+  if( sigs ) *sigs = 0UL;
+  if( !ctx || !ctx->half || !ctx->key_fixed || ctx->last_path != FDGPU_PATH_THROUGHPUT ) return 0;
+  if( hipSetDevice( ctx->device ) != hipSuccess || hipStreamSynchronize( ctx->stream ) != hipSuccess ) return -1;
+  u32 cnt[ 2 ] = { 0u, 0u };
+  if( hipMemcpy( cnt, slow_word( ctx, FD_SW_HOT ) + FD_KC_FWK, sizeof(cnt), hipMemcpyDeviceToHost ) != hipSuccess ) return -1;
+  if( keys ) *keys = (unsigned long)cnt[0];
+  if( sigs ) *sigs = (unsigned long)cnt[1];
+  return 0;
+}
+
+extern "C" int
 fdgpu_ed25519_pinned_count( fdgpu_ed25519_ctx_t * ctx, unsigned long * keys, unsigned long * sigs ) {
   if( keys ) *keys = 0UL;
   if( sigs ) *sigs = 0UL;
@@ -4569,9 +4704,14 @@
     HIPCHK( hipMemcpy( ctx->d_skey, uniq.data(), 32UL*m, hipMemcpyHostToDevice ), -3 );
     hipLaunchKernelGGL( fd_keypin_kernel, dim3( (unsigned)( ( (unsigned long)FD_FB_NT * m + FD_WG - 1UL ) / FD_WG ) ), dim3(FD_WG), 0, s,
                         (u32)m, (u32 const *)ctx->d_skey, ctx->d_sstat, ctx->d_fbase, ctx->d_flist, pcnt );
-    hipLaunchKernelGGL( fd_ftab_kernel, dim3( (unsigned)( ( 4UL * m + 1UL ) / 2UL ) ), dim3(FD_WG), 0, s, (u32 const *)pcnt,
-                        (u32 const *)ctx->d_flist, (unsigned char const *)ctx->d_sstat, (uint4 const *)ctx->d_fbase,
-                        ctx->d_ftab, 4u, (u32 const *)ctx->d_plist, 0u );
+    if( ctx->wcap )
+      hipLaunchKernelGGL( fd_wbase_kernel, dim3( (unsigned)( ( 16UL * m + FD_WG - 1UL ) / FD_WG ) ), dim3(FD_WG), 0, s, (u32 const *)pcnt,
+                          (u32 const *)ctx->d_flist, (unsigned char const *)ctx->d_sstat, (uint4 const *)ctx->d_fbase,
+                          ctx->d_wbase, ctx->wcap );
+    hipLaunchKernelGGL( fd_ftab_kernel, dim3( (unsigned)( ( ( ctx->wcap ? 28UL : 4UL ) * m + 1UL ) / 2UL ) ), dim3(FD_WG), 0, s,
+                        (u32 const *)pcnt, (u32 const *)ctx->d_flist, (unsigned char const *)ctx->d_sstat,
+                        (uint4 const *)ctx->d_fbase, ctx->d_ftab, 4u, (u32 const *)ctx->d_plist, 0u,
+                        (uint4 const *)ctx->d_wbase, ctx->d_wtab, ctx->wcap, 1u );
     HIPCHK( hipGetLastError(), -3 );
     HIPCHK( hipStreamSynchronize( s ), -3 );
     HIPCHK( hipMemcpy( st.data(), ctx->d_sstat, m, hipMemcpyDeviceToHost ), -3 );
diff --git a/firedancer_amd/csrc/fd_gpu_lattice.h b/firedancer_amd/csrc/fd_gpu_lattice.h
--- a/firedancer_amd/csrc/fd_gpu_lattice.h
+++ b/firedancer_amd/csrc/fd_gpu_lattice.h
@@ -318,3 +318,24 @@
 FD_LAT_FN int fd_fb_full_is_base( int i ) { return ( i % 3 ) == 2; }
 FD_LAT_FN int fd_fb_full_digit( int i ) { return ( i % 3 ) == 2 ? i / 3 : 2*( i / 3 ) + ( i % 3 ); }
 FD_LAT_FN int fd_fb_full_table( int i ) { return fd_fb_full_digit( i ); }
+
+#define FD_FB_WIDE_ADDS 40
+#define FD_FB_W0        1024
+#define FD_FB_W2        520
+#define FD_FB_WE        ( 2*FD_FB_W0 + FD_FB_W2 )
+#define FD_FB_WCAP      1024
+FD_LAT_FN int fd_fb_wide_split( int a0, int a1, int a2, int a3, int r ) {
+  int w  = a0 + 256*a1;
+  int d0 = ( ( w + 1024 ) & 2047 ) - 1024;
+  int v1 = ( ( w - d0 ) >> 11 ) + 32*a2 + 8192*a3;
+  int d1 = ( ( v1 + 1024 ) & 2047 ) - 1024;
+  int d2 = ( v1 - d1 ) >> 11;
+  return r==0 ? d0 : r==1 ? d1 : d2;
+}
+FD_LAT_FN int fd_fb_wide_entries( int r ) { return r < 2 ? FD_FB_W0 : FD_FB_W2; }
+FD_LAT_FN int fd_fb_wide_off( int t, int r ) { return t*FD_FB_WE + r*FD_FB_W0; }
+FD_LAT_FN int fd_fb_wide_is_base( int i ) { return ( i % 5 ) >= 3; }
+FD_LAT_FN int fd_fb_wide_span( int i ) { return i / 5; }
+FD_LAT_FN int fd_fb_wide_digit( int i ) { return ( i % 5 ) >= 3 ? 2*( i / 5 ) + ( i % 5 ) - 3 : i % 5; }
+FD_LAT_FN int fd_fb_wide_table( int i ) { return ( i % 5 ) >= 3 ? 2*( i / 5 ) + ( i % 5 ) - 3 : 3*( i / 5 ) + ( i % 5 ); }
+FD_LAT_FN int fd_fb_wave_adds( int all_wide ) { return all_wide ? FD_FB_WIDE_ADDS : FD_FB_FULL_ADDS; }
diff --git a/firedancer_amd/csrc/fd_lat_host.c b/firedancer_amd/csrc/fd_lat_host.c
--- a/firedancer_amd/csrc/fd_lat_host.c
+++ b/firedancer_amd/csrc/fd_lat_host.c
@@ -42,3 +42,26 @@
 
 int
 fd_fb_tables_host( int * nt, int * nb ) { *nt = FD_FB_NT; *nb = FD_FB_NB; return 0; }
+
+int
+fd_fb_wide_sched_host( int * out ) {
+  for( int i=0; i<FD_FB_WIDE_ADDS; i++ ) {
+    out[4*i] = fd_fb_wide_is_base( i ); out[4*i+1] = fd_fb_wide_span( i ); out[4*i+2] = fd_fb_wide_digit( i ); out[4*i+3] = fd_fb_wide_table( i );
+  }
+  return FD_FB_WIDE_ADDS;
+}
+
+int
+fd_fb_wave_adds_host( int all_wide ) { return fd_fb_wave_adds( all_wide ); }
+
+int
+fd_fb_wide_split_host( int a0, int a1, int a2, int a3, int r ) { return fd_fb_wide_split( a0, a1, a2, a3, r ); }
+
+int
+fd_fb_wide_geom_host( int * w0, int * w2, int * we, int * wcap ) { *w0 = FD_FB_W0; *w2 = FD_FB_W2; *we = FD_FB_WE; *wcap = FD_FB_WCAP; return 0; }
+
+int
+fd_fb_wide_entries_host( int r ) { return fd_fb_wide_entries( r ); }
+
+int
+fd_fb_wide_off_host( int t, int r ) { return fd_fb_wide_off( t, r ); }
diff --git a/firedancer_amd/engine.py b/firedancer_amd/engine.py
--- a/firedancer_amd/engine.py
+++ b/firedancer_amd/engine.py
@@ -38,7 +38,7 @@
            "fdgpu_ed25519_reserve_gather_cus", "fdgpu_ed25519_reserve_cus", "fdgpu_ed25519_set_cu_exclusive", "fdgpu_ed25519_get_cu_exclusive", "fdgpu_ed25519_set_lat_share", "fdgpu_ed25519_gather_stats", "fdgpu_ed25519_phase_stats", "fdgpu_ed25519_prepare", "fdgpu_ed25519_submit_raw_gather_dev", "fdgpu_host_region",
            "fdgpu_ed25519_dropin_init", "fdgpu_debug_set_opts", "fdgpu_debug_gather_pauses",
            "fdgpu_ed25519_pipeline_state", "fdgpu_ed25519_verify_many_host", "fdgpu_sha512_batch_device", "fdgpu_sha512_batch_host", "fdgpu_ed25519_set_timing", "fdgpu_ed25519_set_small_batch_max", "fdgpu_ed25519_kernel_ms", "fdgpu_mad_peak_per_s",
-           "fdgpu_ed25519_faulted", "fdgpu_ed25519_debug_fault", "fdgpu_ed25519_slow_count", "fdgpu_ed25519_key_count", "fdgpu_ed25519_hot_count", "fdgpu_ed25519_fixed_count", "fdgpu_ed25519_fcache_count", "fdgpu_ed25519_ffull_count", "fdgpu_ed25519_set_pinned_keys", "fdgpu_ed25519_pin_cap", "fdgpu_ed25519_pinned_count", "fdgpu_ed25519_set_dedup",
+           "fdgpu_ed25519_faulted", "fdgpu_ed25519_debug_fault", "fdgpu_ed25519_slow_count", "fdgpu_ed25519_key_count", "fdgpu_ed25519_hot_count", "fdgpu_ed25519_fixed_count", "fdgpu_ed25519_fcache_count", "fdgpu_ed25519_ffull_count", "fdgpu_ed25519_fwide_count", "fdgpu_ed25519_set_pinned_keys", "fdgpu_ed25519_pin_cap", "fdgpu_ed25519_pinned_count", "fdgpu_ed25519_set_dedup",
            "fdgpu_ed25519_set_record_fp_off", "fdgpu_ed25519_batch_stats", "fdgpu_ed25519_launch_stats", "fdgpu_ed25519_front_remaining", "fdgpu_ed25519_front_batch", "fdgpu_ed25519_verify_txn_ptrs",
            "fdgpu_ed25519_submit_raw_gather_dev_f", "fdgpu_launcher_new", "fdgpu_launcher_delete", "fdgpu_launcher_stats", "fdgpu_ed25519_set_launcher",
            "fdgpu_ed25519_submit_raw_gather_to", "fdgpu_ed25519_set_dedup_seeds", "fdgpu_ed25519_debug_fail_launch",
@@ -141,6 +141,8 @@
         L.fdgpu_ed25519_fcache_count.argtypes = [ctypes.c_void_p, ctypes.c_void_p, ctypes.c_void_p]
         L.fdgpu_ed25519_ffull_count.restype = ctypes.c_int
         L.fdgpu_ed25519_ffull_count.argtypes = [ctypes.c_void_p, ctypes.c_void_p, ctypes.c_void_p]
+        L.fdgpu_ed25519_fwide_count.restype = ctypes.c_int
+        L.fdgpu_ed25519_fwide_count.argtypes = [ctypes.c_void_p, ctypes.c_void_p, ctypes.c_void_p]
         L.fdgpu_ed25519_set_pinned_keys.restype = ctypes.c_int
         L.fdgpu_ed25519_set_pinned_keys.argtypes = [ctypes.c_void_p, ctypes.c_void_p, ctypes.c_ulong, ctypes.c_void_p]
         L.fdgpu_ed25519_pin_cap.restype = ctypes.c_ulong
@@ -188,19 +190,20 @@
                 ("poll_prefetch", ctypes.c_int), ("gather_rpb", ctypes.c_int), ("gather_cu_spread", ctypes.c_int),
                 ("cu_exclusive", ctypes.c_int), ("quad_sha", ctypes.c_int), ("key_dedup", ctypes.c_int),
                 ("key_split", ctypes.c_int), ("key_fixed", ctypes.c_int), ("key_cache", ctypes.c_int),
-                ("key_full", ctypes.c_int)]
+                ("key_full", ctypes.c_int), ("key_wide", ctypes.c_int)]
 
 
 def debug_set_opts(half: int = -1, half_force_slow: int = 0, small_batch_max: int = -1, dsm_lanes: int = 0,
                    nofold_max: int = -1, gather_no_writeback: int = 0, poll_prefetch: int = 0,
                    gather_rpb: int = 0, gather_cu_spread: int = 0, cu_exclusive: int = 0, quad_sha: int = 0,
                    key_dedup: int = 0, key_split: int = 0, key_fixed: int = 0, key_cache: int = 0,
-                   key_full: int = 0) -> None:
+                   key_full: int = 0, key_wide: int = 0) -> None:
     o = DebugOpts(half=half, half_force_slow=half_force_slow,
                   small_batch_max=min(small_batch_max, 2**63 - 1), dsm_lanes=dsm_lanes, nofold_max=nofold_max,
                   gather_no_writeback=gather_no_writeback, poll_prefetch=poll_prefetch, gather_rpb=gather_rpb,
                   gather_cu_spread=gather_cu_spread, cu_exclusive=cu_exclusive, quad_sha=quad_sha, key_dedup=key_dedup,
-                  key_split=key_split, key_fixed=key_fixed, key_cache=key_cache, key_full=key_full)
+                  key_split=key_split, key_fixed=key_fixed, key_cache=key_cache, key_full=key_full,
+                  key_wide=key_wide)
     load_library().fdgpu_debug_set_opts(ctypes.byref(o))
 
 
@@ -476,6 +479,12 @@
             raise RuntimeError("fdgpu_ed25519_ffull_count: " + last_error())
         return int(k.value), int(s.value)
 
+    def fwide_count(self) -> tuple[int, int]:
+        k, s = ctypes.c_ulong(), ctypes.c_ulong()
+        if self.L.fdgpu_ed25519_fwide_count(self.ctx, ctypes.byref(k), ctypes.byref(s)):
+            raise RuntimeError("fdgpu_ed25519_fwide_count: " + last_error())
+        return int(k.value), int(s.value)
+
     def set_pinned_keys(self, keys) -> np.ndarray:
         keys = [bytes(k) for k in keys]
         if any(len(k) != 32 for k in keys):
diff --git a/include/fd_ed25519_gpu.h b/include/fd_ed25519_gpu.h
--- a/include/fd_ed25519_gpu.h
+++ b/include/fd_ed25519_gpu.h
@@ -223,6 +223,9 @@
 
 int
 fdgpu_ed25519_ffull_count( fdgpu_ed25519_ctx_t * ctx, unsigned long * keys, unsigned long * sigs );
+
+int
+fdgpu_ed25519_fwide_count( fdgpu_ed25519_ctx_t * ctx, unsigned long * keys, unsigned long * sigs );
 
 int
 fdgpu_ed25519_set_pinned_keys( fdgpu_ed25519_ctx_t * ctx, unsigned char const * keys, unsigned long n,
@@ -388,6 +391,7 @@
   int           key_fixed;
   int           key_cache;
   int           key_full;
+  int           key_wide;
 } fdgpu_debug_opts_t;
 
 void
```

New measurement: 328.9 million sigs/s, median of 6. 1.07x the previous value.
